# johncai117/Meta-Fine-Tuning

Measured on AMD Instinct MI355X. Metric: episodes/sec at 5-way N-shot (ResNet10+GNN) per GPU and 1/2/4/8-GPU node, higher is better.
Workload: dtype f32

## Files before the change

### include/mft_hip.h

```cpp
#ifndef MFT_HIP_H
#define MFT_HIP_H

#ifdef __cplusplus
extern "C" {
#endif

#define MFT_EINVAL (-22)

enum { MFT_ACT_NONE = 0, MFT_ACT_RELU = 1, MFT_ACT_LRELU = 2 };
enum { MFT_BN_AFFINE_FMA = 0x100 };

int mft_version(void);
int mft_device_info(int* cu_count, int* gcn_arch_is_gfx950);

int mft_stream_create_cumask(const unsigned* mask_words, int n_words, void** stream_out);
int mft_stream_create_priority(int priority, void** stream_out, int* range_out);
int mft_stream_destroy(void* stream);
int mft_stream_probe(float* w, float* m, float* v, long long n, void* stream);
int mft_event_create(void** event_out);
int mft_event_record(void* event, void* stream);
int mft_event_elapsed_ms(void* start, void* stop, float* ms_out);
int mft_event_destroy(void* event);
int mft_probe_placement(unsigned* out, int n_blocks, int spin_cycles, void* stream);

int mft_augment_views(const unsigned char* src, int n_img, int Hs, int Ws, const float* params, int n_views, float* out,
                      long long view_stride, long long img_stride, int size, const float* mean3, const float* std3,
                      void* stream);

int mft_nchw_to_nhwc(const float* src, float* dst, int n_img, int C, int H, int W, void* stream);

long long mft_conv2d_wgrad_adam_dgrad_ws_floats(int n_img, int H, int W, int Cin);
int mft_conv2d_wgrad_adam_dgrad_nhwc(const float* x, int ldx, const float* dy, int ldy, float* w, float* m, float* v,
                                     float* dx_partials, int n_img, int H, int W, int Cin, int Cout, int imgs_per_group,
                                     long long group_stride, int step, float lr, float beta1, float beta2, float eps, void* stream);
int mft_conv2d_wgrad_adam_dgrad_nhwc_dev(const float* x, int ldx, const float* dy, int ldy, float* w, float* m, float* v,
                                         float* dx_partials, int n_img, int H, int W, int Cin, int Cout, int imgs_per_group,
                                         long long group_stride, const float* hyper, float beta1, float beta2, float eps,
                                         void* stream);
int mft_col2im_bn_backward_small(const float* dx_partials, const float* x_raw, const float* relu_out, float* dx, int n_img, int H,
                                 int W, int C, int imgs_per_group, const float* mean, const float* rstd, const float* gamma,
                                 long long gb_group_stride, float* dgamma, float* dbeta, void* stream);

int mft_ce_pool_bn_backward2(const float* feat, const int* labels, int imgs_per_group, int n_groups, int C, int hw,
                             const float* out, const float* xa, const float* xb, float* dxa, float* dxb, const float* mean_a,
                             const float* rstd_a, const float* gamma_a, const float* mean_b, const float* rstd_b,
                             const float* gamma_b, long long gb_group_stride, float* dgamma_a, float* dbeta_a, float* dgamma_b,
                             float* dbeta_b, float* loss, void* stream);

int mft_stem_cache_fill(const float* in, const float* w, int w_ld, int n_img, int H, int W, float* pmax, float* pmin,
                        float* mean_img, float* m2_img, void* stream);
int mft_pool_window_minmax(const float* x, float* ymax, float* ymin, long long n_img, int H, int W, int C, void* stream);
int mft_bn_relu_pooled_gather(const float* pmax, const float* pmin, const int* src_idx, float* y, int n_img, int OH, int OW, int C,
                              int imgs_per_group, const float* mean, const float* rstd, const float* gamma, const float* beta,
                              void* stream);

int mft_ingest_episode_views(const float* const* views, int n_views, int double_first, int n_way, int per_class, int n_support,
                             int C, int H, int W, float* support_store, float* all_store, void* stream);
int mft_pack_oihw(const float* w_oihw, float* w_pk, int Cout, int Cin, int KH, int KW, int k_pad, void* stream);
int mft_pack_oihw_multi(const void* jobs, int n_jobs, long long total_elements, void* stream);
int mft_unpack_oihw(const float* w_pk, float* w_oihw, int Cout, int Cin, int KH, int KW, int k_pad, void* stream);
int mft_pack_dgrad(const float* w_pk, float* wt_pk, int Cout, int Cin, int KH, int KW,
                   int groups, long long w_stride, long long wt_stride, void* stream);

int mft_conv2d_nhwc(const float* in, int ldi, const float* w, const float* bias, float* out, int ldo,
                    int n_img, int H, int W, int Cin, int Cout, int KH, int KW, int stride, int pad,
                    int imgs_per_group, long long w_group_stride, void* stream);

int mft_split_bf16x3(const float* w, unsigned short* planes, long long n, void* stream);
int mft_split_bf16x3_multi(const void* jobs, int n_jobs, long long total_elements, void* stream);
int mft_conv2d_nhwc_x3(const float* in, int ldi, const unsigned short* w3, long long plane_elems, float* out, int ldo,
                       int n_img, int H, int W, int Cin, int Cout, int KH, int KW, int stride, int pad, void* stream);
long long mft_conv2d_x3_stats_ws_floats(int n_img, int H, int W, int Cout, int KH, int KW, int stride, int pad);
int mft_conv2d_nhwc_x3_bnstats(const float* in, int ldi, const unsigned short* w3, long long plane_elems, float* out, int ldo,
                               int n_img, int H, int W, int Cin, int Cout, int KH, int KW, int stride, int pad,
                               int imgs_per_group, float eps, float* stats_ws, float* mean, float* rstd, void* stream);
int mft_conv2d_nhwc_x3_bnin_bnstats(const float* in, int ldi, const float* in_ws, const float* in_gamma, const float* in_beta,
                                    const unsigned short* w3, long long plane_elems, float* out, int ldo, int n_img, int H, int W,
                                    int Cin, int Cout, int imgs_per_group, float eps, float* stats_ws, float* mean, float* rstd,
                                    void* stream);
int mft_split_f16x2(const float* w, unsigned short* planes, long long n, void* stream);
int mft_conv2d_nhwc_h2(const float* in, int ldi, const unsigned short* w2, long long plane_elems, float* out, int ldo,
                       int n_img, int H, int W, int Cin, int Cout, int KH, int KW, int stride, int pad, void* stream);
int mft_conv2d_nhwc_h2_bnstats(const float* in, int ldi, const unsigned short* w2, long long plane_elems, float* out, int ldo,
                               int n_img, int H, int W, int Cin, int Cout, int KH, int KW, int stride, int pad,
                               int imgs_per_group, float eps, float* stats_ws, float* mean, float* rstd, void* stream);
int mft_conv2d_nhwc_h2_bnin_bnstats(const float* in, int ldi, const float* in_ws, const float* in_gamma, const float* in_beta,
                                    const unsigned short* w2, long long plane_elems, float* out, int ldo, int n_img, int H, int W,
                                    int Cin, int Cout, int imgs_per_group, float eps, float* stats_ws, float* mean, float* rstd,
                                    void* stream);
int mft_bn_apply_x3ws(const float* x, int ldx, float* y, int ldy, int C, int rows_per_group, int n_groups, const float* ws,
                      const float* gamma, const float* beta, const float* res, int ldr, const float* res_ws,
                      const float* res_gamma, const float* res_beta, int act, float slope, float eps, float* mean, float* rstd,
                      float* res_mean, float* res_rstd, void* stream);
int mft_bn_running_ema(const float* mean_a, const float* rstd_a, int rows_a, const float* mean_b, const float* rstd_b, int rows_b,
                       const int* order, int n_steps, int C, float eps, float momentum, float* running_mean, float* running_var,
                       void* stream);
int mft_bn_apply_x3ws_fits(int C, int rows_per_group, int with_res_bn);
int mft_bn_relu_pooled_gather_moments(const float* pmax, const float* pmin, const int* src_idx, float* y, int n_img, int OH, int OW,
                                      int C, int imgs_per_group, const float* mean_img, const float* m2_img, int rows_per_img,
                                      float eps, const float* gamma, const float* beta, float* mean, float* rstd, void* stream);

int mft_has_experiments(void);

int mft_conv2d_dgrad_nhwc(const float* dy, int ldy, const float* w, float* dx, int ldx,
                          int n_img, int H, int W, int Cin, int Cout, int KH, int KW, int stride, int pad,
                          int imgs_per_group, long long w_group_stride, void* stream);

long long mft_conv_ksplit_ws_floats(long long rows, int cols, int K);
long long mft_conv_ksplit_grouped_ws_floats(long long rows_per_group, int cols, int K, int groups);
int mft_conv2d_nhwc_ksplit_grouped(const float* in, int ldi, const float* w, float* out, int ldo, int n_img, int H, int W, int Cin,
                                   int Cout, int KH, int KW, int stride, int pad, int imgs_per_group, long long w_group_stride,
                                   float* ws, void* stream);
int mft_conv2d_dgrad_nhwc_ksplit_grouped(const float* dy, int ldy, const float* w, float* dx, int ldx, int n_img, int H, int W, int Cin,
                                         int Cout, int KH, int KW, int stride, int pad, int imgs_per_group, long long w_group_stride,
                                         float* ws, void* stream);
int mft_conv2d_nhwc_ksplit(const float* in, int ldi, const float* w, const float* bias, float* out, int ldo, int n_img, int H, int W,
                           int Cin, int Cout, int KH, int KW, int stride, int pad, float* ws, void* stream);
int mft_conv2d_dgrad_nhwc_ksplit(const float* dy, int ldy, const float* w, float* dx, int ldx, int n_img, int H, int W, int Cin,
                                 int Cout, int KH, int KW, int stride, int pad, float* ws, void* stream);
long long mft_conv2d_wgrad_ws_floats(int n_img, int H, int W, int Cin, int Cout, int KH, int KW, int stride, int pad,
                                     int imgs_per_group);
int mft_conv2d_wgrad_nhwc(const float* in, int ldi, const float* dy, int ldy, float* dw,
                          int n_img, int H, int W, int Cin, int Cout, int KH, int KW, int stride, int pad,
                          int imgs_per_group, long long dw_group_stride, float* ws, void* stream);

long long mft_conv2d_wgrad_oihw_ws_floats(int n_img, int H, int W, int Cin, int Cout, int KH, int KW, int stride, int pad);
int mft_conv2d_wgrad_oihw(const float* in, int ldi, const float* dy, int ldy, float* dw_oihw, int n_img, int H, int W, int Cin,
                          int Cout, int KH, int KW, int stride, int pad, int cin_valid, int cout_valid, float* ws, void* stream);

typedef struct MftWgradJob {
    const float* in; const float* dy; float* dw_oihw; float* ws;
    int ldi, ldy, n_img, H, W, Cin, Cout, KH, KW, stride, pad, cin_valid, cout_valid, reserved;
} MftWgradJob;
int mft_conv2d_wgrad_oihw_multi(const MftWgradJob* jobs, int n_jobs, void* stream);

int mft_conv2d_wgrad_adam_nhwc(const float* in, int ldi, const float* dy, int ldy, float* w, float* m, float* v,
                               float* dw_or_null, int n_img, int H, int W, int Cin, int Cout, int KH, int KW,
                               int stride, int pad, int imgs_per_group, long long group_stride,
                               int step, float lr, float beta1, float beta2, float eps, void* stream);

int mft_wgrad_adam_next_forward(const float* x, int ldx, const float* dy, int ldy, float* w, float* m, float* v,
                                float* dw_or_null, int n_img, int H, int W, int Cin, int Cout, int KH, int KW, int stride,
                                int pad, int imgs_per_group, long long group_stride, int step, const float* hyper, float lr,
                                float beta1, float beta2, float eps, const float* x_next, int mode, float* raw, float* act,
                                const float* gamma, const float* beta, long long gb_group_stride, float* mean, float* rstd,
                                const float* sc_raw, const float* gamma_s, const float* beta_s, float* mean_s, float* rstd_s,
                                float* pooled, float bn_eps, void* stream);


long long mft_bn_stats_ws_floats(int C, int rows_per_group, int n_groups);
int mft_bn_stats(const float* x, int ldx, int C, int rows_per_group, int n_groups, float eps,
                 float* mean, float* rstd, float* ws,
                 float* running_mean, float* running_var, float momentum, long long* num_batches_tracked, void* stream);
typedef struct MftBnStatsJob {
    const float* x; float* mean; float* rstd; float* ws; float* running_mean; float* running_var; long long* num_batches_tracked;
    int ldx, C, rows_per_group, n_groups; float eps, momentum;
} MftBnStatsJob;
int mft_bn_stats_multi(const MftBnStatsJob* jobs, int n_jobs, void* stream);
typedef struct MftBnFwdJob {
    const float* x; float* y; const float* gamma; const float* beta; float* mean; float* rstd;
    float* running_mean; float* running_var; long long* num_batches_tracked;
    const float* res; const float* res_gamma; const float* res_beta; float* res_mean; float* res_rstd;
    float* res_running_mean; float* res_running_var; long long* res_num_batches_tracked;
    int ldx, ldy, ldr, C, rows_per_group, n_groups, act; float eps, momentum, slope;
} MftBnFwdJob;
int mft_bn_forward_small(const MftBnFwdJob* job, void* stream);
int mft_bn_forward_small_max_rows(void);
typedef struct MftBnApplyJob {
    const float* x; float* y; const float* mean; const float* rstd; const float* gamma; const float* beta;
    int ldx, ldy, C, rows_per_group, n_groups, act; float slope; int reserved;
} MftBnApplyJob;
int mft_bn_apply_multi(const MftBnApplyJob* jobs, int n_jobs, void* stream);
int mft_bn_apply(const float* x, int ldx, float* y, int ldy, int C, int rows_per_group, int n_groups,
                 const float* mean, const float* rstd, const float* gamma, const float* beta,
                 long long gb_group_stride,
                 const float* res, int ldr, const float* res_mean, const float* res_rstd,
                 const float* res_gamma, const float* res_beta,
                 int act, float slope, void* stream);
int mft_var_to_rstd(const float* var, float* rstd, int n, float eps, void* stream);
int mft_bn_relu_maxpool(const float* x, float* y, int n_img, int H, int W, int C, int imgs_per_group,
                        const float* mean, const float* rstd, const float* gamma, const float* beta,
                        void* stream);

int mft_bn_image_moments(const float* x, int ldx, int C, int rows_per_img, long long n_img, float* mean_img, float* m2_img,
                         void* stream);
int mft_bn_combine_moments(const float* mean_img, const float* m2_img, const int* idx, int C, int rows_per_img,
                           int imgs_per_group, int n_groups, float eps, float* mean, float* rstd, void* stream);
int mft_bn_relu_maxpool_gather(const float* x, const int* src_idx, float* y, int n_img, int H, int W, int C,
                               int imgs_per_group, const float* mean, const float* rstd, const float* gamma,
                               const float* beta, void* stream);
int mft_global_avgpool(const float* x, float* y, int n_img, int HW, int C, void* stream);

int mft_bn_backward(const float* x, int ldx, const float* dy, int lddy, const float* relu_out, int ldro,
                    float* dx, int lddx, int C, int rows_per_group, int n_groups,
                    const float* mean, const float* rstd, const float* gamma, long long gb_group_stride,
                    float* dgamma, float* dbeta, void* stream);
int mft_bn_small_forward(const float* x1, int ld1, const float* x2, int ld2, const float* res, int ldr, float* y, int ldy, int C,
                         int rows_per_group, int n_groups, const float* gamma1, const float* beta1, const float* gamma2,
                         const float* beta2, long long gb_group_stride, float* mean1, float* rstd1, float* mean2, float* rstd2,
                         int act, float slope, float eps, float* pooled, int hw, void* stream);
int mft_bn_backward2(const float* xa, const float* xb, int ldx, const float* dy, int lddy, float* dxa, float* dxb, int lddx, int C,
                     int rows_per_group, int n_groups, const float* mean_a, const float* rstd_a, const float* gamma_a,
                     const float* mean_b, const float* rstd_b, const float* gamma_b, long long gb_group_stride, float* dgamma_a,
                     float* dbeta_a, float* dgamma_b, float* dbeta_b, void* stream);
int mft_ce_pool_backward(const float* feat, const int* labels, int rows_per_group, int n_groups, int C, int hw, const float* out,
                         float* d_out, float* loss, void* stream);

int mft_avgpool_relu_backward(const float* dfeat, const float* out, float* dout, int n_img, int HW, int C, void* stream);

int mft_cross_entropy(const float* logits, int ld, const int* labels, int C, int rows_per_group, int n_groups,
                      float* loss, float* dlogits, void* stream);
int mft_cross_entropy_mean(const float* logits, int ld, const void* labels, int labels_i64, int C, int rows, float* loss,
                           double* loss_sum, void* stream);
int mft_cross_entropy_mean_backward(const float* logits, int ld, const void* labels, int labels_i64, int C, int rows,
                                    const float* grad_loss, float* dlogits, int ldd, void* stream);
int mft_softmax_rows(const float* x, int ldx, float* y, int ldy, int C, int rows, void* stream);

int mft_proto_scores(const float* feats, int ld, int episodes, int n_way, int n_support, int n_query, int D, float* scores,
                     int softmax, void* stream);
int mft_proto_backward(const float* feats, int ld, int episodes, int n_way, int n_support, int n_query, int D,
                       const float* dscores, int ldg, float* dfeats, int ldd, void* stream);

int mft_mn_gemm(int transa, int transb, int M, int N, int batch, const float* a1, int lda1, long long a1_bs, const float* b1,
                const float* b1_alt, int ldb1, long long b1_bs, int K1, const float* a2, int lda2, long long a2_bs, const float* b2,
                int ldb2, long long b2_bs, int K2, const float* c_in, int ldci, long long ci_bs, const float* bias1,
                const float* bias2, float* c, int ldc, long long c_bs, void* stream);
int mft_lstm_step_forward(float* gates, int ld_g, long long bs_g, const float* c_prev, int ld_cp, long long bs_cp,
                          const float* f_add, int ld_f, float* c_out, float* h_out, int ld_o, long long bs_o, int rows, int D,
                          int batch, void* stream);
int mft_lstm_step_backward(float* gates, int ld_g, long long bs_g, const float* c_prev, int ld_cp, long long bs_cp,
                           const float* c_new, int ld_cn, long long bs_cn, const float* dh1, int ld_d1, long long bs_d1,
                           const float* dh2, int ld_d2, long long bs_d2, const float* dc_in, float* dc_out, int ld_dc,
                           long long bs_dc, float* dh_sum, float* dgate_sum, int accumulate, int rows, int D, int batch,
                           void* stream);
int mft_mn_gather(const float* feats, int ld, int episodes, int n_way, int n_support, int n_query, int D, float* zS, float* zQ,
                  float* h0, void* stream);
int mft_mn_scatter_backward(const float* dzS, const float* dq1, const float* dq2, int episodes, int n_way, int n_support,
                            int n_query, int D, float* dfeats, int ldd, void* stream);
int mft_mn_encode_combine(const float* zS, const float* hf, const float* hr, int episodes, int S, int D, float* G, float* gnorm,
                          void* stream);
int mft_mn_colsum(const float* x, int ldx, int C, long long rows, float* out, void* stream);
int mft_mn_attention_forward(const float* h, const float* G, int episodes, int Q, int S, int D, float* a, float* r, void* stream);
// ... 178 lines not shown
```

### meta-fine-tuning_amd/_lib.py

```python
import ctypes
import os

PKG = os.path.dirname(os.path.abspath(__file__))
LIB_PATH = os.path.join(PKG, "libmft_hip.so")

_P = ctypes.c_void_p
_I = ctypes.c_int
_L = ctypes.c_longlong
_F = ctypes.c_float

SIGNATURES = {
    "mft_version": [],
    "mft_device_info": [_P, _P],
    "mft_stream_create_cumask": [_P, _I, _P],
    "mft_stream_destroy": [_P],
    "mft_stream_probe": [_P, _P, _P, _L, _P],
    "mft_probe_placement": [_P, _I, _I, _P],
    "mft_event_create": [_P],
    "mft_event_record": [_P, _P],
    "mft_event_elapsed_ms": [_P, _P, _P],
    "mft_event_destroy": [_P],
    "mft_augment_views": [_P, _I, _I, _I, _P, _I, _P, _L, _L, _I, _P, _P, _P],
    "mft_nchw_to_nhwc": [_P, _P, _I, _I, _I, _I, _P],
    "mft_pack_oihw": [_P, _P, _I, _I, _I, _I, _I, _P],
    "mft_unpack_oihw": [_P, _P, _I, _I, _I, _I, _I, _P],
    "mft_pack_dgrad": [_P, _P, _I, _I, _I, _I, _I, _L, _L, _P],
    "mft_conv2d_nhwc": [_P, _I, _P, _P, _P, _I, _I, _I, _I, _I, _I, _I, _I, _I, _I, _I, _L, _P],
    "mft_has_experiments": [],
    "mft_split_bf16x3": [_P, _P, _L, _P],
    "mft_split_bf16x3_multi": [_P, _I, _L, _P],
    "mft_conv2d_nhwc_x3": [_P, _I, _P, _L, _P, _I, _I, _I, _I, _I, _I, _I, _I, _I, _I, _P],
    "mft_conv2d_x3_stats_ws_floats": [_I, _I, _I, _I, _I, _I, _I, _I],
    "mft_conv2d_nhwc_x3_bnstats": [_P, _I, _P, _L, _P, _I, _I, _I, _I, _I, _I, _I, _I, _I, _I, _I, _F, _P, _P, _P, _P],
    "mft_conv2d_dgrad_nhwc": [_P, _I, _P, _P, _I, _I, _I, _I, _I, _I, _I, _I, _I, _I, _I, _L, _P],
    "mft_conv_ksplit_ws_floats": [_L, _I, _I],
    "mft_conv_ksplit_grouped_ws_floats": [_L, _I, _I, _I],
    "mft_conv2d_nhwc_ksplit_grouped": [_P, _I, _P, _P, _I, _I, _I, _I, _I, _I, _I, _I, _I, _I, _I, _L, _P, _P],
    "mft_conv2d_dgrad_nhwc_ksplit_grouped": [_P, _I, _P, _P, _I, _I, _I, _I, _I, _I, _I, _I, _I, _I, _I, _L, _P, _P],
    "mft_conv2d_nhwc_ksplit": [_P, _I, _P, _P, _P, _I, _I, _I, _I, _I, _I, _I, _I, _I, _I, _P, _P],
    "mft_conv2d_dgrad_nhwc_ksplit": [_P, _I, _P, _P, _I, _I, _I, _I, _I, _I, _I, _I, _I, _I, _P, _P],
    "mft_conv2d_wgrad_oihw_ws_floats": [_I, _I, _I, _I, _I, _I, _I, _I, _I],
    "mft_conv2d_wgrad_oihw": [_P, _I, _P, _I, _P, _I, _I, _I, _I, _I, _I, _I, _I, _I, _I, _I, _P, _P],
    "mft_conv2d_wgrad_oihw_multi": [_P, _I, _P],
    "mft_conv2d_wgrad_ws_floats": [_I, _I, _I, _I, _I, _I, _I, _I, _I, _I],
    "mft_conv2d_wgrad_nhwc": [_P, _I, _P, _I, _P, _I, _I, _I, _I, _I, _I, _I, _I, _I, _I, _L, _P, _P],
    "mft_conv2d_wgrad_adam_nhwc": [_P, _I, _P, _I, _P, _P, _P, _P, _I, _I, _I, _I, _I, _I, _I, _I, _I, _I, _L, _I, _F, _F, _F,
                                   _F, _P],
    "mft_pair_softmax_ut_backward": [_P, _P, _P, _P, _P, _I, _I, _I, _P, _P],
    "mft_pair_bwd_stats_ws_floats": [_L, _I],
    "mft_pair_bn_act_backward": [_P, _I, _P, _I, _P, _P, _P, _P, _P, _P, _I, _L, _I, _L, _F, _P, _P, _P, _P, _P, _P],
    "mft_pair_absdiff_ut": [_P, _I, _P, _P, _I, _I, _I, _L, _L, _P],
    "mft_pair_dx_gather": [_P, _I, _P, _I, _P, _I, _I, _I, _I, _L, _L, _P],
    "mft_pack_oihw_multi": [_P, _I, _L, _P],
    "mft_wgrad_adam_next_forward": [_P, _I, _P, _I, _P, _P, _P, _P, _I, _I, _I, _I, _I, _I, _I, _I, _I, _I, _L, _I, _P, _F, _F, _F,
                                    _F, _P, _I, _P, _P, _P, _P, _L, _P, _P, _P, _P, _P, _P, _P, _P, _F, _P],
    "mft_bn_stats_ws_floats": [_I, _I, _I],
    "mft_bn_stats": [_P, _I, _I, _I, _I, _F, _P, _P, _P, _P, _P, _F, _P, _P],
    "mft_bn_apply": [_P, _I, _P, _I, _I, _I, _I, _P, _P, _P, _P, _L, _P, _I, _P, _P, _P, _P, _I, _F, _P],
    "mft_bn_apply_multi": [_P, _I, _P],
    "mft_bn_stats_multi": [_P, _I, _P],
    "mft_bn_relu_maxpool": [_P, _P, _I, _I, _I, _I, _I, _P, _P, _P, _P, _P],
    "mft_bn_relu_maxpool_gather": [_P, _P, _P, _I, _I, _I, _I, _I, _P, _P, _P, _P, _P],
    "mft_bn_image_moments": [_P, _I, _I, _I, _L, _P, _P, _P],
    "mft_bn_combine_moments": [_P, _P, _P, _I, _I, _I, _I, _F, _P, _P, _P],
    "mft_global_avgpool": [_P, _P, _I, _I, _I, _P],
    "mft_bn_small_forward": [_P, _I, _P, _I, _P, _I, _P, _I, _I, _I, _I, _P, _P, _P, _P, _L, _P, _P, _P, _P, _I, _F, _F, _P, _I, _P],
    "mft_bn_backward2": [_P, _P, _I, _P, _I, _P, _P, _I, _I, _I, _I, _P, _P, _P, _P, _P, _P, _L, _P, _P, _P, _P, _P],
    "mft_ce_pool_backward": [_P, _P, _I, _I, _I, _I, _P, _P, _P, _P],
    "mft_bn_backward": [_P, _I, _P, _I, _P, _I, _P, _I, _I, _I, _I, _P, _P, _P, _L, _P, _P, _P],
    "mft_avgpool_relu_backward": [_P, _P, _P, _I, _I, _I, _P],
    "mft_cross_entropy": [_P, _I, _P, _I, _I, _I, _P, _P, _P],
    "mft_softmax_rows": [_P, _I, _P, _I, _I, _I, _P],
    "mft_proto_scores": [_P, _I, _I, _I, _I, _I, _I, _P, _I, _P],
    "mft_proto_backward": [_P, _I, _I, _I, _I, _I, _I, _P, _I, _P, _I, _P],
    "mft_mn_gemm": [_I, _I, _I, _I, _I, _P, _I, _L, _P, _P, _I, _L, _I, _P, _I, _L, _P, _I, _L, _I, _P, _I, _L, _P, _P, _P, _I, _L, _P],
    "mft_lstm_step_forward": [_P, _I, _L, _P, _I, _L, _P, _I, _P, _P, _I, _L, _I, _I, _I, _P],
    "mft_lstm_step_backward": [_P, _I, _L, _P, _I, _L, _P, _I, _L, _P, _I, _L, _P, _I, _L, _P, _P, _I, _L, _P, _P, _I, _I, _I, _I, _P],
    "mft_mn_gather": [_P, _I, _I, _I, _I, _I, _I, _P, _P, _P, _P],
    "mft_mn_scatter_backward": [_P, _P, _P, _I, _I, _I, _I, _I, _P, _I, _P],
    "mft_mn_encode_combine": [_P, _P, _P, _I, _I, _I, _P, _P, _P],
    "mft_mn_colsum": [_P, _I, _I, _L, _P, _P],
    "mft_mn_attention_forward": [_P, _P, _I, _I, _I, _I, _P, _P, _P],
    "mft_mn_attention_backward": [_P, _P, _P, _P, _I, _I, _I, _I, _P, _P, _P],
    "mft_mn_readout_forward": [_P, _P, _P, _I, _I, _I, _I, _I, _P, _P, _P, _P, _P, _P],
    "mft_mn_readout_backward": [_P, _I, _P, _P, _P, _P, _P, _P, _P, _I, _I, _I, _I, _I, _P, _P, _P, _P],
    "mft_nll_mean": [_P, _I, _P, _I, _I, _I, _P, _P, _P],
    "mft_nll_mean_backward": [_P, _I, _I, _I, _P, _P, _I, _P],
    "mft_ridge_gram": [_P, _I, _I, _I, _I, _I, _I, _F, _P, _P],
    "mft_ridge_factor_solve": [_P, _I, _I, _I, _I, _I, _I, _P, _P, _P, _P],
    "mft_ridge_scores": [_P, _I, _I, _I, _I, _I, _I, _P, _P, _P, _I, _P],
    "mft_ridge_backward_query": [_P, _I, _I, _I, _I, _I, _I, _P, _P, _P, _I, _P, _I, _P, _P, _P],
    "mft_ridge_backward_support": [_P, _I, _I, _I, _I, _I, _I, _P, _P, _P, _P, _P, _P, _I, _P, _P],
    "mft_dist_linear_forward": [_P, _I, _I, _I, _P, _P, _I, _I, _F, _P, _I, _P],
    "mft_dist_linear_backward": [_P, _I, _I, _P, _P, _I, _I, _F, _P, _I, _P, _I, _P, _P, _P],
    "mft_dist_head_sgd_run": [_P, _P, _P, _I, _I, _I, _I, _I, _I, _P, _P, _F, _F, _F, _F, _F, _P],
    "mft_dist_head_step": [_P, _I, _P, _I, _I, _I, _I, _F, _P, _P, _P, _P, _P, _P, _P, _I, _P, _I, _F, _F, _F, _F, _F, _P],
    "mft_cross_entropy_mean": [_P, _I, _P, _I, _I, _I, _P, _P, _P],
    "mft_cross_entropy_mean_backward": [_P, _I, _P, _I, _I, _I, _P, _P, _I, _P],
    "mft_adam_step": [_P, _P, _P, _P, _L, _I, _F, _F, _F, _F, _F, _P],
    "mft_sgd_step": [_P, _P, _P, _L, _I, _F, _F, _F, _F, _P],
    "mft_maml_delta": [_P, _P, _P, _L, _P],
    "mft_conv2d_wgrad_adam_dgrad_ws_floats": [_I, _I, _I, _I],
    "mft_conv2d_wgrad_adam_dgrad_nhwc": [_P, _I, _P, _I, _P, _P, _P, _P, _I, _I, _I, _I, _I, _I, _L, _I, _F, _F, _F, _F, _P],
    "mft_conv2d_wgrad_adam_dgrad_nhwc_dev": [_P, _I, _P, _I, _P, _P, _P, _P, _I, _I, _I, _I, _I, _I, _L, _P, _F, _F, _F, _P],
    "mft_col2im_bn_backward_small": [_P, _P, _P, _P, _I, _I, _I, _I, _I, _P, _P, _P, _L, _P, _P, _P],
    "mft_stream_create_priority": [_I, _P, _P],
    "mft_ce_pool_bn_backward2": [_P, _P, _I, _I, _I, _I, _P, _P, _P, _P, _P, _P, _P, _P, _P, _P, _P, _L, _P, _P, _P, _P, _P, _P],
    "mft_pool_window_minmax": [_P, _P, _P, _L, _I, _I, _I, _P],
    "mft_stem_cache_fill": [_P, _P, _I, _I, _I, _I, _P, _P, _P, _P, _P],
    "mft_conv2d_nhwc_x3_bnin_bnstats": [_P, _I, _P, _P, _P, _P, _L, _P, _I, _I, _I, _I, _I, _I, _I, _F, _P, _P, _P, _P],
    "mft_split_f16x2": [_P, _P, _L, _P],
    "mft_conv2d_nhwc_h2": [_P, _I, _P, _L, _P, _I, _I, _I, _I, _I, _I, _I, _I, _I, _I, _P],
    "mft_conv2d_nhwc_h2_bnstats": [_P, _I, _P, _L, _P, _I, _I, _I, _I, _I, _I, _I, _I, _I, _I, _I, _F, _P, _P, _P, _P],
    "mft_conv2d_nhwc_h2_bnin_bnstats": [_P, _I, _P, _P, _P, _P, _L, _P, _I, _I, _I, _I, _I, _I, _I, _F, _P, _P, _P, _P],
    "mft_bn_apply_x3ws": [_P, _I, _P, _I, _I, _I, _I, _P, _P, _P, _P, _I, _P, _P, _P, _I, _F, _F, _P, _P, _P, _P, _P],
    "mft_bn_apply_x3ws_fits": [_I, _I, _I],
    "mft_bn_running_ema": [_P, _P, _I, _P, _P, _I, _P, _I, _I, _F, _F, _P, _P, _P],
    "mft_bn_relu_pooled_gather_moments": [_P, _P, _P, _P, _I, _I, _I, _I, _I, _P, _P, _I, _F, _P, _P, _P, _P, _P],
    "mft_bn_relu_pooled_gather": [_P, _P, _P, _P, _I, _I, _I, _I, _I, _P, _P, _P, _P, _P],
    "mft_ingest_episode_views": [_P, _I, _I, _I, _I, _I, _I, _I, _I, _P, _P, _P],
    "mft_block_entry_small_forward": [_P, _I, _P, _L, _P, _L, _P, _P, _P, _I, _I, _I, _I, _I, _I, _I, _P, _P, _L, _P, _P, _F, _P],
    "mft_block_exit_small_forward": [_P, _P, _L, _P, _P, _P, _P, _I, _I, _I, _I, _I, _P, _P, _P, _P, _L, _P, _P, _P, _P, _F, _P],
    "mft_conv2d_dgrad_bn_backward_small": [_P, _I, _P, _P, _I, _I, _I, _I, _I, _I, _I, _I, _I, _I, _L, _P, _P, _P, _P, _P, _L,
                                           _P, _P, _P],
    "mft_linear_head_sgd_run": [_P, _P, _P, _I, _I, _I, _I, _I, _I, _P, _P, _F, _F, _F, _F, _P],
    "mft_linear_head_adam_run": [_P, _P, _P, _I, _I, _I, _I, _I, _I, _P, _P, _F, _F, _F, _F, _F, _P],
    "mft_adam_multi": [_P, _I, _I, _F, _F, _F, _F, _F, _F, _P],
    "mft_adam_hyper_advance": [_P, _P, _F, _F, _F, _P],
    "mft_adam_step_dev": [_P, _P, _P, _P, _L, _P, _F, _F, _F, _F, _P],
    "mft_conv2d_wgrad_adam_nhwc_dev": [_P, _I, _P, _I, _P, _P, _P, _P, _I, _I, _I, _I, _I, _I, _I, _I, _I, _I, _L, _P, _F, _F,
                                       _F, _P],
    "mft_linear_head_step": [_P, _I, _P, _I, _I, _I, _I, _P, _P, _P, _P, _P, _P, _P, _I, _P, _I, _F, _F, _F, _F, _F, _P],
    "mft_linear_head_scores": [_P, _I, _I, _I, _I, _I, _P, _P, _P, _P],
    "mft_pair_absdiff": [_P, _I, _P, _I, _I, _I, _I, _P],
    "mft_masked_softmax": [_P, _I, _P, _I, _I, _P],
    "mft_pair_mlp_tiles_m": [_I, _I],
    "mft_pair_mlp_layer": [_P, _I, _I, _P, _P, _P, _P, _I, _I, _P, _P, _I, _I, _I, _I, _F, _P, _P, _P, _I, _P],
    "mft_bn_forward_small": [_P, _P],
    "mft_bn_forward_small_max_rows": [],
    "mft_gemm_rk": [_P, _I, _P, _I, _I, _P, _P, _I, _I, _I, _P],
    "mft_pair_mlp_tiles_m_rk": [_I, _I],
    "mft_pair_mlp_layer_rk": [_P, _I, _I, _P, _P, _P, _P, _I, _I, _P, _P, _I, _I, _I, _I, _F, _P, _P, _P, _P],
    "mft_pair_mlp_stats_finalize_rk": [_P, _P, _P, _I, _I, _I, _P, _P, _F, _P, _P, _P, _P, _P],
    "mft_pair_mlp_stats_finalize": [_P, _P, _P, _I, _I, _I, _P, _P, _F, _P, _P, _P, _P, _P],
    "mft_pair_mlp_score": [_P, _I, _P, _P, _P, _P, _F, _P, _I, _I, _I, _P],
    "mft_masked_softmax_ut": [_P, _P, _I, _I, _P],
    "mft_graph_aggregate": [_P, _P, _I, _P, _I, _I, _I, _I, _P],
    "mft_copy_cols": [_P, _I, _P, _I, _I, _I, _I, _I, _F, _P],
    "mft_build_graph_nodes": [_P, _I, _P, _I, _I, _I, _I, _I, _I, _P],
    "mft_gather_query_scores": [_P, _I, _P, _I, _I, _I, _I, _P],
    "mft_gather_rows": [_P, _P, _P, _I, _L, _P],
    "mft_var_to_rstd": [_P, _P, _I, _F, _P],
    "mft_bn_backward_ws_floats": [_I, _I, _I],
    "mft_bn_backward_act": [_P, _I, _P, _I, _P, _I, _P, _I, _I, _I, _I, _P, _P, _P, _L, _P, _P, _I, _F, _P, _P, _P, _P, _P],
    "mft_bn_backward_act_multi": [_P, _I, _P],
    "mft_act_backward": [_P, _I, _P, _I, _P, _I, _I, _L, _I, _F, _I, _P],
    "mft_colsum": [_P, _I, _I, _L, _P, _P, _P],
    "mft_bn_relu_maxpool_arg": [_P, _P, _P, _I, _I, _I, _I, _I, _P, _P, _P, _P, _P],
    "mft_maxpool_relu_backward": [_P, _P, _P, _P, _I, _I, _I, _I, _P],
    "mft_masked_softmax_backward": [_P, _P, _P, _I, _I, _I, _P],
    "mft_pair_absdiff_backward": [_P, _I, _P, _I, _P, _I, _I, _I, _I, _P],
    "mft_graph_aggregate_backward": [_P, _P, _I, _P, _I, _P, _I, _P, _I, _I, _I, _I, _P],
    "mft_build_graph_nodes_backward": [_P, _I, _P, _I, _I, _I, _I, _I, _I, _P],
    "mft_gather_query_scores_backward": [_P, _P, _I, _I, _I, _I, _I, _P, _P],
    "mft_fwt_draw_fold": [_P, _I, _I, _I, ctypes.c_ulonglong, _P, _P, _P, _P, _P],
    "mft_fwt_unfold": [_P, _I, _I, _I, _P, _P],
}
TESTING_SIGNATURES = {
    "mft_debug_set_conv_tile": [_I],
    "mft_debug_set_x3_tile": [_I],
    "mft_debug_reset": [],
    "mft_wgrad_fwd_set_exact": [_I],
    "mft_wgrad_fwd_set_xcd": [_I],
}
_RESTYPE = {"mft_conv2d_x3_stats_ws_floats": _L, "mft_bn_stats_ws_floats": _L, "mft_conv2d_wgrad_ws_floats": _L, "mft_bn_backward_ws_floats": _L,
            "mft_conv2d_wgrad_adam_dgrad_ws_floats": _L, "mft_pair_bwd_stats_ws_floats": _L, "mft_conv_ksplit_ws_floats": _L, "mft_conv2d_wgrad_oihw_ws_floats": _L, "mft_conv_ksplit_grouped_ws_floats": _L}

_lib = None


def lib():
    global _lib
    if _lib is None:
        if not os.path.exists(LIB_PATH):
            raise RuntimeError(
                "libmft_hip.so not found at %s -- build it with `python -c 'import __graft_entry__ as g; g.build()'`; "
                "this package has no CPU or PyTorch fallback" % LIB_PATH)
        import torch
        if torch.cuda.is_available():
            torch.cuda.init()
            torch.empty(1, device="cuda")
        h = ctypes.CDLL(LIB_PATH)
        for name, argtypes in list(SIGNATURES.items()) + list(TESTING_SIGNATURES.items()):
            fn = getattr(h, name)
            fn.argtypes = argtypes
            fn.restype = _RESTYPE.get(name, _I)
        _lib = h
    return _lib


MFT_EINVAL = -22


def check(rc, what):
    if rc != 0:
        raise RuntimeError("%s failed with code %d (hipError_t / MFT_EINVAL=-22)" % (what, rc))


class LaunchTimer:

    _SKIP = ("mft_event_", "mft_stream_", "mft_debug_", "mft_version", "mft_device_info", "mft_has_experiments",
             "mft_wgrad_fwd_set_", "mft_probe_placement")

    def __init__(self, only=None, keep_args=False):
        self.only = only
        self.keep_args = keep_args
        self._pairs = []
        self._free = []
        self._real = None

    def _event(self):
        if self._free:
            return self._free.pop()
        e = ctypes.c_void_p()
        check(self._real.mft_event_create(ctypes.byref(e)), "mft_event_create")
        return e

    def __getattr__(self, name):
        real = self.__dict__["_real"]
        fn = getattr(real, name)
        sig = SIGNATURES.get(name)
        if (sig is None or not sig or sig[-1] is not _P or name.endswith("_ws_floats") or name.startswith(self._SKIP)
                or (self.only is not None and not self.only(name))):
            return fn

        def timed(*args):
            stream = args[-1]
            a, b = self._event(), self._event()
            real.mft_event_record(a, stream)
            rc = fn(*args)
            if rc != 0:
                self._free += [a, b]
                return rc
            real.mft_event_record(b, stream)
            self._pairs.append((name, a, b, args if self.keep_args else None))
            return rc
        return timed

    def __enter__(self):
        global _lib
        self._real = lib()
        assert not isinstance(self._real, LaunchTimer), "LaunchTimer blocks do not nest"
        _lib = self
        return self

    def __exit__(self, *exc):
        global _lib
        _lib = self._real
        if exc and exc[0] is not None:
            for _, a, b, _ in self._pairs:
                self._free += [a, b]
            self._pairs = []
            self.close()
        return False

    def collect(self, calls=False):
        out, flat = {}, []
# ... 14 lines not shown
```

### meta-fine-tuning_amd/csrc/conv_x3.hip

```cpp
#include "mft_common.h"
#include "bn_fold.h"

namespace {

typedef __bf16 bf16x8 __attribute__((ext_vector_type(8)));
typedef __bf16 bf16x2 __attribute__((ext_vector_type(2)));
typedef _Float16 f16x8 __attribute__((ext_vector_type(8)));
typedef _Float16 f16x4 __attribute__((ext_vector_type(4)));
typedef float f32x2 __attribute__((ext_vector_type(2)));
typedef unsigned u32x2 __attribute__((ext_vector_type(2)));
typedef unsigned u32x4 __attribute__((ext_vector_type(4)));

struct X3Args {
    const float* in;
    const unsigned short* w3;
    long long plane;
    float* out;
    int ldi, ldo;
    int H, W, Cin, OH, OW, Cout, KH, KW, stride, pad;
    int Kpad;
    int M;
    int tiles_n;
    unsigned in_bytes, w_bytes;
    int xcd_swizzle;
    int row_swz;
    float* stats_ws;
    int rows_per_group;
    int s1_rows;
    const float* bn_ws; const float* bn_gamma; const float* bn_beta;
    float bn_eps;
    int bn_max_tiles;
};

constexpr int X3_RS = 40;

__device__ __forceinline__ unsigned pk_bf16(float a, float b) {
    f32x2 v = {a, b};
    return __builtin_bit_cast(unsigned, __builtin_convertvector(v, bf16x2));
}

__device__ __forceinline__ void split4(const f32x4 x, u32x2& p1, u32x2& p2, u32x2& p3) {
    f32x4 r;
    p1[0] = pk_bf16(x[0], x[1]);
    p1[1] = pk_bf16(x[2], x[3]);
    r[0] = x[0] - __builtin_bit_cast(float, p1[0] << 16);
    r[1] = x[1] - __builtin_bit_cast(float, p1[0] & 0xffff0000u);
    r[2] = x[2] - __builtin_bit_cast(float, p1[1] << 16);
    r[3] = x[3] - __builtin_bit_cast(float, p1[1] & 0xffff0000u);
    p2[0] = pk_bf16(r[0], r[1]);
    p2[1] = pk_bf16(r[2], r[3]);
    r[0] -= __builtin_bit_cast(float, p2[0] << 16);
    r[1] -= __builtin_bit_cast(float, p2[0] & 0xffff0000u);
    r[2] -= __builtin_bit_cast(float, p2[1] << 16);
    r[3] -= __builtin_bit_cast(float, p2[1] & 0xffff0000u);
    p3[0] = pk_bf16(r[0], r[1]);
    p3[1] = pk_bf16(r[2], r[3]);
}

__device__ __forceinline__ void split4_h2(const f32x4 x, u32x2& p1, u32x2& p2) {
    const f16x4 hi = __builtin_convertvector(x, f16x4);
    const f32x4 r = (x - __builtin_convertvector(hi, f32x4)) * 2048.f;
    const f16x4 lo = __builtin_convertvector(r, f16x4);
    p1 = __builtin_bit_cast(u32x2, hi);
    p2 = __builtin_bit_cast(u32x2, lo);
}
constexpr float X3_H2_LO_SCALE = 1.0f / 2048.f;

template <int BM, int BN, bool DB, int HOIST = 0, int DBG = 0, bool XS = false, int NP = 3>
__global__ __launch_bounds__(256) __attribute__((amdgpu_waves_per_eu(NP == 2 ? 3 : 1))) void conv_x3_kernel(X3Args p) {
    static_assert(NP == 3 || (NP == 2 && !DB && HOIST == 0 && DBG == 0 && !XS), "f16x2: the plain single-buffer form only");
    constexpr int NACC = NP == 3 ? 1 : 2;
    constexpr int TM = BM / 64;
    constexpr int TN = BN / 64;
    constexpr int PA = BM / 32;
    constexpr int PB = BN / 64;
    constexpr int RS = XS ? 32 : X3_RS;
    constexpr int A_PLANE = BM * RS;
    constexpr int B_PLANE = BN * RS;
    auto lo = [](int row, int c) -> int {
        if constexpr (XS) return row * 32 + ((((c >> 3) ^ (row >> 2)) & 3) << 3) + (c & 7);
        else return row * X3_RS + c;
    };
    extern __shared__ __attribute__((aligned(16))) unsigned short smem[];
    unsigned short* As = smem;
    unsigned short* Bs = smem + NP * A_PLANE;
    constexpr int BUF = NP * (A_PLANE + B_PLANE);

    const int tid = threadIdx.x;
    const int lane = tid & 63, wave = tid >> 6;
    const int wm = wave >> 1, wn = wave & 1;
    const int r = lane & 31, h = lane >> 5;
    const bool g_swz = !XS && p.row_swz != 0;
    int tile_id = blockIdx.x;
    if (p.xcd_swizzle) {
        const int nwg = gridDim.x, q = nwg >> 3, rmd = nwg & 7;
        const int xcd = tile_id & 7, slot = tile_id >> 3;
        tile_id = xcd * q + (xcd < rmd ? xcd : rmd) + slot;
    }
    const int nt = tile_id % p.tiles_n;
    const int mt = tile_id / p.tiles_n;
    const int m0 = mt * BM, n0 = nt * BN;

    const int g_id = tid >> 5;
    const int g_rr = (tid >> 3) & 3;
    const int lrow = g_swz ? g_rr * 4 + (g_id & 3) + 16 * (g_id >> 2) : tid >> 3;
    const int c4 = (tid & 7) * 4;
    const int ohw = p.OH * p.OW;
    const __amdgpu_buffer_rsrc_t rA = __builtin_amdgcn_make_buffer_rsrc((void*)p.in, 0, p.in_bytes, 0x00020000);
    const __amdgpu_buffer_rsrc_t rB = __builtin_amdgcn_make_buffer_rsrc((void*)p.w3, 0, p.w_bytes, 0x00020000);
    int a_off[PA];
    int a_ih0[PA], a_iw0[PA];
    bool a_ok[PA];
#pragma unroll
    for (int j = 0; j < PA; ++j) {
        const int m = m0 + lrow + 32 * j;
        a_ok[j] = m < p.M;
        const int mm = a_ok[j] ? m : 0;
        const int img = mm / ohw;
        const int rem = mm - img * ohw;
        const int oh = rem / p.OW, ow = rem - oh * p.OW;
        a_ih0[j] = oh * p.stride - p.pad;
        a_iw0[j] = ow * p.stride - p.pad;
        a_off[j] = (((img * p.H + a_ih0[j]) * p.W + a_iw0[j]) * p.ldi + c4) * 4;
    }
    const int bseg = tid & 3;
    const int brow = g_swz ? ((tid >> 2) & 3) * 4 + ((tid >> 4) & 3) + 16 * (tid >> 6) : tid >> 2;
    int b_off[PB];
#pragma unroll
    for (int j = 0; j < PB; ++j) b_off[j] = ((n0 + brow + 64 * j) * p.Kpad + bseg * 8) * 2;
    const int plane_bytes = (int)(p.plane * 2);

    f32x16 accs[NACC][TM][TN];
#pragma unroll
    for (int q = 0; q < NACC; ++q)
#pragma unroll
        for (int i = 0; i < TM; ++i)
#pragma unroll
            for (int j = 0; j < TN; ++j)
#pragma unroll
                for (int e = 0; e < 16; ++e) accs[q][i][j][e] = 0.f;
    auto& acc = accs[0];
    auto val = [&](int i, int j, int e) -> float {
        if constexpr (NP == 3) return accs[0][i][j][e];
        else return __builtin_fmaf(accs[NACC - 1][i][j][e], X3_H2_LO_SCALE, accs[0][i][j][e]);
    };

    struct Stage {
        f32x4 ra[PA];
        u32x4 rb[PB][NP];
    };
    Stage st0;
    const int nk = p.Kpad / 32;

    int t_kt = 0, t_ci0 = 0, t_kh = 0, t_kw = 0;
    auto load_tile = [&](int kt, Stage& S) {
        const int k0 = kt * 32;
        while (t_kt < kt) {
            ++t_kt;
            t_ci0 += 32;
            if (t_ci0 == p.Cin) { t_ci0 = 0; if (++t_kw == p.KW) { t_kw = 0; ++t_kh; } }
        }
        const int ci0 = t_ci0, kh = t_kh, kw = t_kw;
        const int tap_off = ((kh * p.W + kw) * p.ldi + ci0) * 4;
#pragma unroll
        for (int j = 0; j < PA; ++j) {
            const bool ok = a_ok[j] && (unsigned)(a_ih0[j] + kh) < (unsigned)p.H && (unsigned)(a_iw0[j] + kw) < (unsigned)p.W;
            const unsigned voff = ok ? (unsigned)(a_off[j] + tap_off) : 0x80000000u;
            S.ra[j] = __builtin_bit_cast(f32x4, __builtin_amdgcn_raw_buffer_load_b128(rA, voff, 0, 0));
        }
#pragma unroll
        for (int j = 0; j < PB; ++j)
#pragma unroll
            for (int pl = 0; pl < NP; ++pl)
                S.rb[j][pl] = __builtin_amdgcn_raw_buffer_load_b128(rB, b_off[j] + pl * plane_bytes, k0 * 2, 0);
    };
    auto store_tile = [&](const Stage& S, int buf) {
        unsigned short* As = smem + buf * BUF;
        unsigned short* Bs = As + NP * A_PLANE;
#pragma unroll
        for (int j = 0; j < PA; ++j) {
            const int off = lo(lrow + 32 * j, c4);
            if constexpr (NP == 2) {
                u32x2 p1, p2;
                split4_h2(S.ra[j], p1, p2);
                *(u32x2*)(As + off) = p1;
                *(u32x2*)(As + A_PLANE + off) = p2;
            } else {
                u32x2 p1, p2, p3;
                if constexpr (DBG & 1) {
                    const u32x4 raw = __builtin_bit_cast(u32x4, S.ra[j]);
                    p1[0] = raw[0]; p1[1] = raw[1]; p2[0] = raw[2]; p2[1] = raw[3]; p3 = p1;
                } else {
                    split4(S.ra[j], p1, p2, p3);
                }
                *(u32x2*)(As + off) = p1;
                *(u32x2*)(As + A_PLANE + off) = p2;
                *(u32x2*)(As + 2 * A_PLANE + off) = p3;
            }
        }
#pragma unroll
        for (int j = 0; j < PB; ++j)
#pragma unroll
            for (int pl = 0; pl < NP; ++pl)
                *(u32x4*)(Bs + pl * B_PLANE + lo(brow + 64 * j, bseg * 8)) = S.rb[j][pl];
    };

    auto compute = [&](int buf) {
        const unsigned short* As = smem + buf * BUF;
        const unsigned short* Bs = As + NP * A_PLANE;
        if constexpr (NP == 2) {
#pragma unroll
            for (int kk = 0; kk < 2; ++kk) {
                f16x8 a[TM][2], b[TN][2];
#pragma unroll
                for (int i = 0; i < TM; ++i)
#pragma unroll
                    for (int pl = 0; pl < 2; ++pl)
                        a[i][pl] = *(const f16x8*)(As + pl * A_PLANE + lo(wm * (BM / 2) + i * 32 + r, kk * 16 + h * 8));
#pragma unroll
                for (int j = 0; j < TN; ++j)
#pragma unroll
                    for (int pl = 0; pl < 2; ++pl)
                        b[j][pl] = *(const f16x8*)(Bs + pl * B_PLANE + lo(wn * (BN / 2) + j * 32 + r, kk * 16 + h * 8));
                constexpr int TA[3] = {0, 1, 0};
                constexpr int TB[3] = {1, 0, 0};
                constexpr int TQ[3] = {1, 1, 0};
#pragma unroll
                for (int t = 0; t < 3; ++t)
#pragma unroll
                    for (int i = 0; i < TM; ++i)
#pragma unroll
                        for (int j = 0; j < TN; ++j)
                            accs[TQ[t] ? NACC - 1 : 0][i][j] =
                                __builtin_amdgcn_mfma_f32_32x32x16_f16(a[i][TA[t]], b[j][TB[t]], accs[TQ[t] ? NACC - 1 : 0][i][j], 0, 0, 0);
            }
            return;
        }
        if constexpr (HOIST == 0) {
#pragma unroll
            for (int kk = 0; kk < 2; ++kk) {
                bf16x8 a[TM][3], b[TN][3];
#pragma unroll
                for (int i = 0; i < TM; ++i)
#pragma unroll
                    for (int pl = 0; pl < 3; ++pl)
                        a[i][pl] = *(const bf16x8*)(As + pl * A_PLANE + lo(wm * (BM / 2) + i * 32 + r, kk * 16 + h * 8));
#pragma unroll
                for (int j = 0; j < TN; ++j)
// ... 14 lines not shown
#pragma unroll
                    for (int t = 0; t < 6; ++t)
#pragma unroll
                        for (int i = 0; i < TM; ++i)
#pragma unroll
                            for (int j = 0; j < TN; ++j)
                                acc[i][j] = __builtin_amdgcn_mfma_f32_32x32x16_bf16(a[i][TA[t]], b[j][TB[t]], acc[i][j], 0, 0, 0);
                }
            }
            return;
        }
        bf16x8 a[2][TM][3], b[2][TN][3];
        if constexpr (HOIST == 1) {
#pragma unroll
            for (int kk = 0; kk < 2; ++kk) {
#pragma unroll
                for (int pl = 0; pl < 3; ++pl) {
#pragma unroll
                    for (int i = 0; i < TM; ++i)
                        a[kk][i][pl] = *(const bf16x8*)(As + pl * A_PLANE + lo(wm * (BM / 2) + i * 32 + r, kk * 16 + h * 8));
#pragma unroll
                    for (int j = 0; j < TN; ++j)
                        b[kk][j][pl] = *(const bf16x8*)(Bs + pl * B_PLANE + lo(wn * (BN / 2) + j * 32 + r, kk * 16 + h * 8));
                }
            }
            __builtin_amdgcn_sched_barrier(0);
            constexpr int TA[6] = {0, 0, 1, 1, 0, 2};
            constexpr int TB[6] = {0, 1, 0, 1, 2, 0};
#pragma unroll
            for (int kk = 0; kk < 2; ++kk)
#pragma unroll
                for (int t = 0; t < 6; ++t)
#pragma unroll
                    for (int i = 0; i < TM; ++i)
#pragma unroll
                        for (int j = 0; j < TN; ++j)
                            acc[i][j] = __builtin_amdgcn_mfma_f32_32x32x16_bf16(a[kk][i][TA[t]], b[kk][j][TB[t]], acc[i][j], 0, 0, 0);
            __builtin_amdgcn_sched_barrier(0);
        } else {
            auto rd = [&](int kk) {
#pragma unroll
                for (int pl = 0; pl < 3; ++pl) {
#pragma unroll
                    for (int i = 0; i < TM; ++i)
                        a[kk][i][pl] = *(const bf16x8*)(As + pl * A_PLANE + lo(wm * (BM / 2) + i * 32 + r, kk * 16 + h * 8));
#pragma unroll
                    for (int j = 0; j < TN; ++j)
                        b[kk][j][pl] = *(const bf16x8*)(Bs + pl * B_PLANE + lo(wn * (BN / 2) + j * 32 + r, kk * 16 + h * 8));
                }
            };
            constexpr int TA[6] = {0, 0, 1, 1, 0, 2};
            constexpr int TB[6] = {0, 1, 0, 1, 2, 0};
            auto mm = [&](int kk) {
#pragma unroll
                for (int t = 0; t < 6; ++t)
#pragma unroll
                    for (int i = 0; i < TM; ++i)
#pragma unroll
                        for (int j = 0; j < TN; ++j)
                            acc[i][j] = __builtin_amdgcn_mfma_f32_32x32x16_bf16(a[kk][i][TA[t]], b[kk][j][TB[t]], acc[i][j], 0, 0, 0);
            };
            rd(0);
            __builtin_amdgcn_sched_barrier(0);
            rd(1);
            mm(0);
            for (int q = 0; q < 6 * TM * TN; ++q) {
                __builtin_amdgcn_sched_group_barrier(0x8, 1, 0);
                __builtin_amdgcn_sched_group_barrier(0x100, (3 * (TM + TN) + 6 * TM * TN - 1) / (6 * TM * TN), 0);
            }
            __builtin_amdgcn_sched_barrier(0);
            mm(1);
            __builtin_amdgcn_sched_barrier(0);
        }
    };
    if constexpr (DB) {
        load_tile(0, st0);
        store_tile(st0, 0);
        __syncthreads();
        load_tile(nk > 1 ? 1 : 0, st0);
        for (int kt = 0; kt + 1 < nk; ++kt) {
            compute(kt & 1);
            store_tile(st0, (kt + 1) & 1);
            load_tile(kt + 2 < nk ? kt + 2 : nk - 1, st0);
            __syncthreads();
        }
        compute((nk - 1) & 1);
    } else {
        load_tile(0, st0);
        store_tile(st0, 0);
        __syncthreads();
        for (int kt = 0; kt < nk; ++kt) {
            if constexpr (!(DBG & 4)) { if (kt + 1 < nk) load_tile(kt + 1, st0); }
            if constexpr (!(DBG & 16)) compute(0);
            if constexpr (!(DBG & 32)) __syncthreads();
            if constexpr (!(DBG & 8)) { if (kt + 1 < nk) store_tile(st0, 0); }
            if constexpr (!(DBG & 32)) __syncthreads();
        }
    }

#pragma unroll
    for (int i = 0; i < TM; ++i)
#pragma unroll
        for (int j = 0; j < TN; ++j) {
            const int n = n0 + wn * (BN / 2) + j * 32 + r;
#pragma unroll
            for (int e = 0; e < 16; ++e) {
                const int row = (e & 3) + 8 * (e >> 2) + 4 * h;
                const int m = m0 + wm * (BM / 2) + i * 32 + row;
                if (m < p.M) p.out[(long long)m * p.ldo + n] = val(i, j, e);
            }
        }
    if (p.stats_ws != nullptr) {
        static_assert(TN == 1 || TN == 2, "stats epilogue");
        const int split = (m0 / p.rows_per_group + 1) * p.rows_per_group;
        float* sred = reinterpret_cast<float*>(smem);
        __syncthreads();
#pragma unroll
        for (int j = 0; j < TN; ++j) {
            float a1 = 0.f, a2 = 0.f, b1 = 0.f, b2 = 0.f;
#pragma unroll
            for (int i = 0; i < TM; ++i)
#pragma unroll
                for (int e = 0; e < 16; ++e) {
                    const int m = m0 + wm * (BM / 2) + i * 32 + (e & 3) + 8 * (e >> 2) + 4 * h;
                    const float v = val(i, j, e);
                    if (m < p.M) {
                        if (m < split) { a1 += v; a2 += v * v; }
                        else { b1 += v; b2 += v * v; }
                    }
                }
            a1 += __shfl_xor(a1, 32, 64); a2 += __shfl_xor(a2, 32, 64);
            b1 += __shfl_xor(b1, 32, 64); b2 += __shfl_xor(b2, 32, 64);
            if (h == 0) {
                float* o = sred + ((((wm * 2 + wn) * TN + j) * 32 + r) << 2);
                o[0] = a1; o[1] = a2; o[2] = b1; o[3] = b2;
            }
        }
        __syncthreads();
        if (wm == 0 && h == 0) {
#pragma unroll
            for (int j = 0; j < TN; ++j) {
                const float* o0 = sred + ((((0 * 2 + wn) * TN + j) * 32 + r) << 2);
                const float* o1 = sred + ((((1 * 2 + wn) * TN + j) * 32 + r) << 2);
                const int n = n0 + wn * (BN / 2) + j * 32 + r;
                float* w0 = p.stats_ws + (((long long)mt * 2 + 0) * p.Cout + n) * 2;
                float* w1 = p.stats_ws + (((long long)mt * 2 + 1) * p.Cout + n) * 2;
                w0[0] = o0[0] + o1[0]; w0[1] = o0[1] + o1[1];
                w1[0] = o0[2] + o1[2]; w1[1] = o0[3] + o1[3];
            }
        }
    }
}

#ifdef MFT_EXPERIMENTS
#include "../../tools/experiments/conv_x3_pingpong.inc"
#endif

template <int BM, int BN, bool BNIN, int NP = 3, bool BDB = true>
__device__ __forceinline__ void conv_x3_s1_body(const X3Args& p) {
    static_assert(NP == 3 || NP == 2, "3 bf16 pieces (six products) or 2 fp16 pieces (three products)");
    constexpr int NACC = NP == 3 ? 1 : 2;
    constexpr int TM = BM / 64, TN = BN / 64;
    constexpr int PA = BM / 32, PB = BN / 64;
    constexpr int RS = X3_RS;
    constexpr int B_PLANE = BN * RS;
    const int A_PLANE = p.s1_rows * RS;
    extern __shared__ __attribute__((aligned(16))) unsigned short smem[];
    constexpr int NBB = (NP == 2 && BDB) ? 2 : 1;
    unsigned short* As = smem;
    unsigned short* Bs = smem + NP * A_PLANE;
    float* bn_tab = reinterpret_cast<float*>(Bs + NBB * NP * B_PLANE);

    const int tid = threadIdx.x;
    const int lane = tid & 63, wave = tid >> 6;
    const int wm = wave >> 1, wn = wave & 1;
    const int r = lane & 31, h = lane >> 5;
    int tile_id = blockIdx.x;
    if (p.xcd_swizzle) {
        const int nwg = gridDim.x, q = nwg >> 3, rmd = nwg & 7;
        const int xcd = tile_id & 7, slot = tile_id >> 3;
        tile_id = xcd * q + (xcd < rmd ? xcd : rmd) + slot;
    }
    const int nt = tile_id % p.tiles_n;
    const int mt = tile_id / p.tiles_n;
    const int m0 = mt * BM, n0 = nt * BN;
    const int W = p.W, H = p.H;
    const int fr0 = m0 / W;
    const int g0 = BNIN ? m0 / p.rows_per_group : 0;
    const bool bn_two = BNIN && (m0 + (BM < p.M - m0 ? BM : p.M - m0) - 1) / p.rows_per_group > g0;
    if constexpr (BNIN) {
        char* stage = reinterpret_cast<char*>(smem);
        const size_t gstride = mft_x3_stage_bytes(p.bn_max_tiles, p.Cin);
        const bool two = bn_two;
        mft_x3_stats_stage(p.bn_ws, p.Cin, g0, p.M, p.rows_per_group, BM, p.bn_max_tiles, stage, tid, 256);
        if (two) mft_x3_stats_stage(p.bn_ws, p.Cin, g0 + 1, p.M, p.rows_per_group, BM, p.bn_max_tiles, stage + gstride, tid, 256);
        __syncthreads();
        for (int i = tid; i < 2 * p.Cin; i += 256) {
            const int gi = i >= p.Cin ? 1 : 0, c = i - gi * p.Cin;
            if (gi == 0 || two) {
                float mu, rs, sc, sh;
                mft_x3_stats_staged(stage + gi * gstride, p.bn_max_tiles, p.Cin, c, g0 + gi, p.M, p.rows_per_group, BM, p.bn_eps, mu, rs);
                mft_bn_fold(mu, rs, p.bn_gamma[c], p.bn_beta[c], sc, sh);
                bn_tab[(gi * 2 + 0) * p.Cin + c] = sc;
                bn_tab[(gi * 2 + 1) * p.Cin + c] = sh;
            }
        }
        __syncthreads();
    }
    const int g_id = tid >> 5, g_rr = (tid >> 3) & 3;
    const int lrow = p.row_swz ? g_rr * 4 + (g_id & 3) + 16 * (g_id >> 2) : tid >> 3;
    const int c4 = (tid & 7) * 4;
    const __amdgpu_buffer_rsrc_t rA = __builtin_amdgcn_make_buffer_rsrc((void*)p.in, 0, p.in_bytes, 0x00020000);
    const __amdgpu_buffer_rsrc_t rB = __builtin_amdgcn_make_buffer_rsrc((void*)p.w3, 0, p.w_bytes, 0x00020000);
    int a_off[PA], a_oh[PA], a_lds[PA], a_tab[PA];
    bool a_ok[PA];
#pragma unroll
    for (int j = 0; j < PA; ++j) {
        const int t = lrow + 32 * j, m = m0 + t;
        const int fr = m / W;
        a_ok[j] = m < p.M;
        a_oh[j] = fr - (fr / H) * H;
        a_off[j] = ((a_ok[j] ? m : 0) * p.ldi + c4) * 4;
        a_lds[j] = (t + 1) * RS + c4;
        a_tab[j] = BNIN ? ((a_ok[j] ? m / p.rows_per_group - g0 : 0) * 2 * p.Cin + c4) : 0;
    }
    const int hside = (tid >> 3) & 1;
    const int mh = hside ? m0 + BM : m0 - 1;
    const int frh = (mh > 0 ? mh : 0) / W;
    const bool h_ok = tid < 16 && (hside ? (mh < p.M && mh - frh * W != 0) : (m0 > 0 && m0 - fr0 * W != 0));
    const int h_oh = frh - (frh / H) * H;
    const int h_off = ((h_ok ? mh : 0) * p.ldi + c4) * 4;
    const int h_lds = (hside ? BM + 1 : 0) * RS + c4;
    const int h_tab = BNIN ? (((hside && h_ok) ? (m0 + BM - 1) / p.rows_per_group - g0 : 0) * 2 * p.Cin + c4) : 0;

    const int bseg = tid & 3;
    const int brow = p.row_swz ? ((tid >> 2) & 3) * 4 + ((tid >> 4) & 3) + 16 * (tid >> 6) : tid >> 2;
    int b_off[PB];
#pragma unroll
    for (int j = 0; j < PB; ++j) b_off[j] = ((n0 + brow + 64 * j) * p.Kpad + bseg * 8) * 2;
    const int plane_bytes = (int)(p.plane * 2);

    int fa[TM], fl[TM], fr_[TM];
    constexpr int Z0 = BM + 2;
#pragma unroll
    for (int i = 0; i < TM; ++i) {
        const int t = wm * (BM / 2) + i * 32 + r;
        const int ow = (m0 + t) - ((m0 + t) / W) * W;
        fa[i] = (t + 1) * RS;
        fl[i] = ow == 0 ? (Z0 + ((t - Z0) & 15)) * RS : fa[i] - RS;
        fr_[i] = ow == W - 1 ? (Z0 + ((t + 2 - Z0) & 15)) * RS : fa[i] + RS;
    }

    f32x16 acc[NACC][TM][TN];
#pragma unroll
    for (int q = 0; q < NACC; ++q)
#pragma unroll
        for (int i = 0; i < TM; ++i)
#pragma unroll
            for (int j = 0; j < TN; ++j)
#pragma unroll
                for (int e = 0; e < 16; ++e) acc[q][i][j][e] = 0.f;
    auto val = [&](int i, int j, int e) -> float {
        if constexpr (NP == 3) return acc[0][i][j][e];
        else return __builtin_fmaf(acc[1][i][j][e], X3_H2_LO_SCALE, acc[0][i][j][e]);
    };

    struct Stage {
        f32x4 ra[PA];
        f32x4 rh;
        u32x4 rb[PB][NP];
    };
    Stage st;
    const int n_ci = p.Cin / 32;
    const int n_ms = 3 * n_ci;
    auto load_a = [&](int ms, Stage& S) {
        const int kh = ms / n_ci, ci0 = (ms - kh * n_ci) * 32;
        const int shift = ((kh - 1) * W * p.ldi + ci0) * 4;
#pragma unroll
        for (int j = 0; j < PA; ++j) {
            const bool ok = a_ok[j] && (unsigned)(a_oh[j] + kh - 1) < (unsigned)H;
            S.ra[j] = __builtin_bit_cast(f32x4, __builtin_amdgcn_raw_buffer_load_b128(rA, ok ? (unsigned)(a_off[j] + shift) : 0x80000000u, 0, 0));
        }
        const bool okh = h_ok && (unsigned)(h_oh + kh - 1) < (unsigned)H;
        S.rh = __builtin_bit_cast(f32x4, __builtin_amdgcn_raw_buffer_load_b128(rA, okh ? (unsigned)(h_off + shift) : 0x80000000u, 0, 0));
    };
    auto load_b = [&](int ms, int kw, Stage& S) {
        const int kh = ms / n_ci, ci0 = (ms - kh * n_ci) * 32;
        const int k0 = (kh * 3 + kw) * p.Cin + ci0;
#pragma unroll
        for (int j = 0; j < PB; ++j)
#pragma unroll
            for (int pl = 0; pl < NP; ++pl)
                S.rb[j][pl] = __builtin_amdgcn_raw_buffer_load_b128(rB, b_off[j] + pl * plane_bytes, k0 * 2, 0);
    };
    auto put_a = [&](const f32x4 v, int off) {
        if constexpr (NP == 3) {
            u32x2 p1, p2, p3;
            split4(v, p1, p2, p3);
            *(u32x2*)(As + off) = p1;
            *(u32x2*)(As + A_PLANE + off) = p2;
            *(u32x2*)(As + 2 * A_PLANE + off) = p3;
        } else {
            u32x2 p1, p2;
            split4_h2(v, p1, p2);
            *(u32x2*)(As + off) = p1;
            *(u32x2*)(As + A_PLANE + off) = p2;
        }
    };
    auto bn_relu = [&](const f32x4 v, const f32x4 sc, const f32x4 sh, bool ok) {
        f32x4 o = mft_bn_affine4(v, sc, sh);
#pragma unroll
        for (int e = 0; e < 4; ++e) o[e] = ok ? fmaxf(o[e], 0.f) : 0.f;
        return o;
    };
    auto store_a = [&](const Stage& S, int ms) {
        if constexpr (BNIN) {
            const int kh = ms / n_ci, ci0 = (ms - kh * n_ci) * 32;
            const bool okh = h_ok && (unsigned)(h_oh + kh - 1) < (unsigned)H;
            if (!bn_two) {
                const f32x4 sc = *(const f32x4*)(bn_tab + ci0 + c4), sh = *(const f32x4*)(bn_tab + p.Cin + ci0 + c4);
#pragma unroll
                for (int j = 0; j < PA; ++j)
                    put_a(bn_relu(S.ra[j], sc, sh, a_ok[j] && (unsigned)(a_oh[j] + kh - 1) < (unsigned)H), a_lds[j]);
                if (tid < 16) put_a(bn_relu(S.rh, sc, sh, okh), h_lds);
            } else {
#pragma unroll
                for (int j = 0; j < PA; ++j)
                    put_a(bn_relu(S.ra[j], *(const f32x4*)(bn_tab + a_tab[j] + ci0), *(const f32x4*)(bn_tab + a_tab[j] + p.Cin + ci0),
                                  a_ok[j] && (unsigned)(a_oh[j] + kh - 1) < (unsigned)H), a_lds[j]);
                if (tid < 16)
                    put_a(bn_relu(S.rh, *(const f32x4*)(bn_tab + h_tab + ci0), *(const f32x4*)(bn_tab + h_tab + p.Cin + ci0), okh), h_lds);
            }
        } else {
#pragma unroll
            for (int j = 0; j < PA; ++j) put_a(S.ra[j], a_lds[j]);
            if (tid < 16) put_a(S.rh, h_lds);
        }
    };
    auto store_b = [&](const Stage& S, int bb = 0) {
#pragma unroll
        for (int j = 0; j < PB; ++j)
#pragma unroll
            for (int pl = 0; pl < NP; ++pl)
                *(u32x4*)(Bs + (bb * NP + pl) * B_PLANE + (brow + 64 * j) * RS + bseg * 8) = S.rb[j][pl];
    };
    auto compute = [&](int kw, int bb = 0) {
        const unsigned short* const Bc = Bs + bb * NP * B_PLANE;
#pragma unroll
        for (int kk = 0; kk < 2; ++kk) {
            if constexpr (NP == 3) {
                bf16x8 a[TM][3], b[TN][3];
#pragma unroll
                for (int i = 0; i < TM; ++i)
#pragma unroll
                    for (int pl = 0; pl < 3; ++pl)
                        a[i][pl] = *(const bf16x8*)(As + pl * A_PLANE + (kw == 0 ? fl[i] : (kw == 1 ? fa[i] : fr_[i])) + kk * 16 + h * 8);
#pragma unroll
                for (int j = 0; j < TN; ++j)
#pragma unroll
                    for (int pl = 0; pl < 3; ++pl)
                        b[j][pl] = *(const bf16x8*)(Bc + pl * B_PLANE + (wn * (BN / 2) + j * 32 + r) * RS + kk * 16 + h * 8);
                constexpr int TA[6] = {2, 0, 1, 1, 0, 0};
                constexpr int TB[6] = {0, 2, 1, 0, 1, 0};
#pragma unroll
                for (int t = 0; t < 6; ++t)
#pragma unroll
                    for (int i = 0; i < TM; ++i)
#pragma unroll
                        for (int j = 0; j < TN; ++j)
                            acc[0][i][j] = __builtin_amdgcn_mfma_f32_32x32x16_bf16(a[i][TA[t]], b[j][TB[t]], acc[0][i][j], 0, 0, 0);
            } else {
                f16x8 a[TM][2], b[TN][2];
#pragma unroll
                for (int i = 0; i < TM; ++i)
#pragma unroll
                    for (int pl = 0; pl < 2; ++pl)
                        a[i][pl] = *(const f16x8*)(As + pl * A_PLANE + (kw == 0 ? fl[i] : (kw == 1 ? fa[i] : fr_[i])) + kk * 16 + h * 8);
#pragma unroll
                for (int j = 0; j < TN; ++j)
#pragma unroll
                    for (int pl = 0; pl < 2; ++pl)
                        b[j][pl] = *(const f16x8*)(Bc + pl * B_PLANE + (wn * (BN / 2) + j * 32 + r) * RS + kk * 16 + h * 8);
                constexpr int TA[3] = {0, 1, 0};
                constexpr int TB[3] = {1, 0, 0};
                constexpr int TQ[3] = {1, 1, 0};
#pragma unroll
                for (int t = 0; t < 3; ++t)
#pragma unroll
                    for (int i = 0; i < TM; ++i)
#pragma unroll
                        for (int j = 0; j < TN; ++j)
                            acc[TQ[t]][i][j] = __builtin_amdgcn_mfma_f32_32x32x16_f16(a[i][TA[t]], b[j][TB[t]], acc[TQ[t]][i][j], 0, 0, 0);
            }
        }
    };

    for (int i = tid; i < NP * A_PLANE / 8; i += 256) ((u32x4*)As)[i] = (u32x4){0u, 0u, 0u, 0u};
    load_a(0, st);
    load_b(0, 0, st);
    __syncthreads();
    store_a(st, 0);
    store_b(st);
    __syncthreads();
    if constexpr (NBB == 2) {
        int cur = 0;
        for (int ms = 0; ms < n_ms; ++ms) {
            const int msn = ms + 1 < n_ms ? ms + 1 : ms;
            load_b(ms, 1, st);
            compute(0, cur);
            store_b(st, cur ^ 1);
            __syncthreads();
            load_b(ms, 2, st);
            compute(1, cur ^ 1);
            store_b(st, cur);
            __syncthreads();
            load_a(msn, st);
            load_b(msn, 0, st);
            compute(2, cur);
            store_b(st, cur ^ 1);
            __syncthreads();
            store_a(st, msn);
            __syncthreads();
            cur ^= 1;
        }
    } else {
        for (int ms = 0; ms < n_ms; ++ms) {
            const int msn = ms + 1 < n_ms ? ms + 1 : ms;
            load_b(ms, 1, st);
            compute(0);
            __syncthreads();
            store_b(st);
            __syncthreads();
            load_b(ms, 2, st);
            compute(1);
            __syncthreads();
            store_b(st);
            __syncthreads();
            load_a(msn, st);
            load_b(msn, 0, st);
            compute(2);
            __syncthreads();
            store_a(st, msn);
            store_b(st);
            __syncthreads();
        }
    }

#pragma unroll
    for (int i = 0; i < TM; ++i)
#pragma unroll
        for (int j = 0; j < TN; ++j) {
            const int n = n0 + wn * (BN / 2) + j * 32 + r;
#pragma unroll
            for (int e = 0; e < 16; ++e) {
                const int row = (e & 3) + 8 * (e >> 2) + 4 * h;
                const int m = m0 + wm * (BM / 2) + i * 32 + row;
                if (m < p.M) p.out[(long long)m * p.ldo + n] = val(i, j, e);
            }
        }
    if (p.stats_ws != nullptr) {
        static_assert(TN == 1 || TN == 2, "stats epilogue");
        const int split = (m0 / p.rows_per_group + 1) * p.rows_per_group;
        float* sred = reinterpret_cast<float*>(smem);
        __syncthreads();
#pragma unroll
        for (int j = 0; j < TN; ++j) {
            float a1 = 0.f, a2 = 0.f, b1 = 0.f, b2 = 0.f;
#pragma unroll
            for (int i = 0; i < TM; ++i)
#pragma unroll
                for (int e = 0; e < 16; ++e) {
                    const int m = m0 + wm * (BM / 2) + i * 32 + (e & 3) + 8 * (e >> 2) + 4 * h;
                    const float v = val(i, j, e);
                    if (m < p.M) {
                        if (m < split) { a1 += v; a2 += v * v; }
                        else { b1 += v; b2 += v * v; }
                    }
                }
            a1 += __shfl_xor(a1, 32, 64); a2 += __shfl_xor(a2, 32, 64);
            b1 += __shfl_xor(b1, 32, 64); b2 += __shfl_xor(b2, 32, 64);
            if (h == 0) {
                float* o = sred + ((((wm * 2 + wn) * TN + j) * 32 + r) << 2);
                o[0] = a1; o[1] = a2; o[2] = b1; o[3] = b2;
            }
        }
        __syncthreads();
        if (wm == 0 && h == 0) {
#pragma unroll
            for (int j = 0; j < TN; ++j) {
                const float* o0 = sred + ((((0 * 2 + wn) * TN + j) * 32 + r) << 2);
                const float* o1 = sred + ((((1 * 2 + wn) * TN + j) * 32 + r) << 2);
                const int n = n0 + wn * (BN / 2) + j * 32 + r;
                float* w0 = p.stats_ws + (((long long)mt * 2 + 0) * p.Cout + n) * 2;
                float* w1 = p.stats_ws + (((long long)mt * 2 + 1) * p.Cout + n) * 2;
                w0[0] = o0[0] + o1[0]; w0[1] = o0[1] + o1[1];
                w1[0] = o0[2] + o1[2]; w1[1] = o0[3] + o1[3];
            }
        }
    }
}

template <int BM, int BN, int NP = 3, bool BDB = true>
__global__ __launch_bounds__(256) __attribute__((amdgpu_waves_per_eu(NP == 2 ? 3 : 1))) void conv_x3_s1_kernel(X3Args p) {
    conv_x3_s1_body<BM, BN, false, NP, BDB>(p);
}

template <int BM, int BN, int NP = 3, bool BDB = true>
__global__ __launch_bounds__(256) __attribute__((amdgpu_waves_per_eu(3, 3))) void conv_x3_s1_bnin_kernel(X3Args p) {
    conv_x3_s1_body<BM, BN, true, NP, BDB>(p);
}

__global__ void x3_stats_finalize_kernel(const float* __restrict__ ws, int C, int M, int R, int BM, float eps,
                                         float* __restrict__ mean, float* __restrict__ rstd) {
    const int c = blockIdx.x * blockDim.x + threadIdx.x;
    const int g = blockIdx.y;
    if (c >= C) return;
    float mu, rs;
    mft_x3_stats_merge(ws, C, c, g, M, R, BM, eps, mu, rs);
    mean[(long long)g * C + c] = mu;
    rstd[(long long)g * C + c] = rs;
}

__global__ __launch_bounds__(256) void split_bf16x3_kernel(const float* __restrict__ w, unsigned short* __restrict__ out,
                                                           long long n) {
    for (long long i = (long long)blockIdx.x * blockDim.x + threadIdx.x; i < n; i += (long long)gridDim.x * blockDim.x) {
        const float x = w[i];
        const unsigned q1 = pk_bf16(x, 0.f) & 0xffffu;
        const float r1 = x - __builtin_bit_cast(float, q1 << 16);
        const unsigned q2 = pk_bf16(r1, 0.f) & 0xffffu;
        const float r2 = r1 - __builtin_bit_cast(float, q2 << 16);
        const unsigned q3 = pk_bf16(r2, 0.f) & 0xffffu;
        out[i] = (unsigned short)q1;
        out[n + i] = (unsigned short)q2;
        out[2 * n + i] = (unsigned short)q3;
    }
}

struct SplitJob { const float* src; unsigned short* dst; long long n, Cout, Cin, taps, transposed, start; };

__global__ __launch_bounds__(256) void split_bf16x3_multi_kernel(const SplitJob* __restrict__ jobs, int n_jobs, long long total) {
    for (long long i = (long long)blockIdx.x * blockDim.x + threadIdx.x; i < total; i += (long long)gridDim.x * blockDim.x) {
        int lo = 0, hi = n_jobs - 1;
        while (lo < hi) {
            const int mid = (lo + hi + 1) >> 1;
            if (jobs[mid].start <= i) lo = mid; else hi = mid - 1;
        }
        const SplitJob j = jobs[lo];
        const long long l = i - j.start;
        long long src = l;
        if (j.transposed) {
            const long long co = l % j.Cout, t = l / j.Cout;
            const long long tp = t % j.taps, ci = t / j.taps;
            src = (co * j.taps + (j.taps - 1 - tp)) * j.Cin + ci;
        }
        const float x = j.src[src];
        const unsigned q1 = pk_bf16(x, 0.f) & 0xffffu;
        const float r1 = x - __builtin_bit_cast(float, q1 << 16);
        const unsigned q2 = pk_bf16(r1, 0.f) & 0xffffu;
        const float r2 = r1 - __builtin_bit_cast(float, q2 << 16);
        const unsigned q3 = pk_bf16(r2, 0.f) & 0xffffu;
        j.dst[l] = (unsigned short)q1;
        j.dst[j.n + l] = (unsigned short)q2;
        j.dst[2 * j.n + l] = (unsigned short)q3;
    }
}

__global__ __launch_bounds__(256) void split_f16x2_kernel(const float* __restrict__ w, unsigned short* __restrict__ out, long long n) {
    for (long long i = (long long)blockIdx.x * blockDim.x + threadIdx.x; i < n; i += (long long)gridDim.x * blockDim.x) {
        const float x = w[i];
        const _Float16 hi = (_Float16)x;
        const _Float16 lo = (_Float16)((x - (float)hi) * 2048.f);
        out[i] = __builtin_bit_cast(unsigned short, hi);
        out[n + i] = __builtin_bit_cast(unsigned short, lo);
    }
}

int g_x3_db = 0;
int g_x3_dbg = 0;
int g_x3_hoist = 0;
int g_x3_row_swz = 1;
int g_x3_xcd = 1;
int g_x3_min_lds_kb = 0;

template <int BM, int BN, bool DB>
int launch_x3(X3Args p, hipStream_t s, int np = 3) {
    const int tiles_m = (p.M + BM - 1) / BM;
    p.tiles_n = p.Cout / BN;
    p.xcd_swizzle = g_x3_xcd;
    p.row_swz = g_x3_row_swz;
    if (np == 2) {
        if constexpr (!DB) {
            p.row_swz = g_x3_row_swz != 0;
            const size_t lds2 = (size_t)2 * (BM + BN) * X3_RS * sizeof(unsigned short);
            hipLaunchKernelGGL((conv_x3_kernel<BM, BN, false, 0, 0, false, 2>), dim3((unsigned)(tiles_m * p.tiles_n)), dim3(256), lds2, s, p);
            return mft_launch_status();
        }
        return MFT_EINVAL;
    }
#ifdef MFT_EXPERIMENTS
    const bool xs = g_x3_row_swz == 2 && !DB && g_x3_hoist == 0 && g_x3_dbg == 0;
#else
    constexpr bool xs = false;
#endif
    size_t lds = (size_t)(DB ? 2 : 1) * 3 * (BM + BN) * (xs ? 32 : X3_RS) * sizeof(unsigned short);
#ifdef MFT_EXPERIMENTS
    if ((size_t)g_x3_min_lds_kb * 1024 > lds) lds = (size_t)g_x3_min_lds_kb * 1024;
    if (xs) {
        if constexpr (!DB) {
            hipLaunchKernelGGL((conv_x3_kernel<BM, BN, false, 0, 0, true>), dim3((unsigned)(tiles_m * (p.Cout / BN))), dim3(256), lds, s,
                               ([&] { X3Args q = p; q.tiles_n = p.Cout / BN; q.xcd_swizzle = g_x3_xcd; q.row_swz = 0; return q; })());
            return mft_launch_status();
        }
    }
    auto kern = g_x3_hoist == 1 ? conv_x3_kernel<BM, BN, DB, 1> : (g_x3_hoist == 2 ? conv_x3_kernel<BM, BN, DB, 2> : conv_x3_kernel<BM, BN, DB, 0>);
    if (g_x3_dbg && !DB) {
        switch (g_x3_dbg) {
            case 1: kern = conv_x3_kernel<BM, BN, DB, 0, 1>; break;
            case 2: kern = conv_x3_kernel<BM, BN, DB, 0, 2>; break;
            case 4: kern = conv_x3_kernel<BM, BN, DB, 0, 4>; break;
            case 8: kern = conv_x3_kernel<BM, BN, DB, 0, 8>; break;
            case 12: kern = conv_x3_kernel<BM, BN, DB, 0, 12>; break;
            case 13: kern = conv_x3_kernel<BM, BN, DB, 0, 13>; break;
            case 16: kern = conv_x3_kernel<BM, BN, DB, 0, 16>; break;
            case 28: kern = conv_x3_kernel<BM, BN, DB, 0, 28>; break;
            case 32: kern = conv_x3_kernel<BM, BN, DB, 0, 32>; break;
            case 34: kern = conv_x3_kernel<BM, BN, DB, 0, 34>; break;
            case 36: kern = conv_x3_kernel<BM, BN, DB, 0, 36>; break;
            case 33: kern = conv_x3_kernel<BM, BN, DB, 0, 33>; break;
            default: break;
        }
    }
#else
    auto kern = conv_x3_kernel<BM, BN, DB, 0>;
#endif
    if (lds > 64 * 1024) {
        hipError_t e = hipFuncSetAttribute((const void*)kern, hipFuncAttributeMaxDynamicSharedMemorySize, 160 * 1024);
        if (e != hipSuccess) return (int)e;
    }
    hipLaunchKernelGGL(kern, dim3((unsigned)(tiles_m * p.tiles_n)), dim3(256), lds, s, p);
    return mft_launch_status();
}

int g_x3_s1 = 1;

constexpr size_t X3_S1_LDS_3PER_CU = 160 * 1024 / 3;

int g_x3_bdb = 1;

inline size_t x3_s1_lds(int BM, int BN, int W, int bn_cin, int np = 3) {
    (void)W;
    return (size_t)np * (BM + 18 + ((np == 2 && g_x3_bdb) ? 2 : 1) * BN) * X3_RS * sizeof(unsigned short) + (size_t)4 * bn_cin * sizeof(float);
}

template <int BM, int BN>
int launch_x3_s1(X3Args p, hipStream_t s, int np = 3) {
    const int tiles_m = (p.M + BM - 1) / BM;
    p.tiles_n = p.Cout / BN;
    p.xcd_swizzle = g_x3_xcd;
    p.row_swz = g_x3_row_swz != 0;
    p.s1_rows = BM + 18;
    const size_t lds = x3_s1_lds(BM, BN, p.W, p.bn_ws ? p.Cin : 0, np);
    const dim3 grid((unsigned)(tiles_m * p.tiles_n));
    if (np == 2 && g_x3_bdb) {
        if (p.bn_ws) hipLaunchKernelGGL((conv_x3_s1_bnin_kernel<BM, BN, 2, true>), grid, dim3(256), lds, s, p);
        else hipLaunchKernelGGL((conv_x3_s1_kernel<BM, BN, 2, true>), grid, dim3(256), lds, s, p);
    } else if (np == 2) {
        if (p.bn_ws) hipLaunchKernelGGL((conv_x3_s1_bnin_kernel<BM, BN, 2, false>), grid, dim3(256), lds, s, p);
        else hipLaunchKernelGGL((conv_x3_s1_kernel<BM, BN, 2, false>), grid, dim3(256), lds, s, p);
    } else if (p.bn_ws) {
        hipLaunchKernelGGL((conv_x3_s1_bnin_kernel<BM, BN>), grid, dim3(256), lds, s, p);
    } else {
        hipLaunchKernelGGL((conv_x3_s1_kernel<BM, BN>), grid, dim3(256), lds, s, p);
    }
    return mft_launch_status();
}

int g_x3_pp = 0;
#ifdef MFT_EXPERIMENTS

template <int BM, int BN>
int launch_x3_pp(X3Args p, hipStream_t s) {
    const int tiles_m = (p.M + BM - 1) / BM;
    p.tiles_n = p.Cout / BN;
    p.xcd_swizzle = g_x3_xcd;
    p.row_swz = 1;
    const size_t lds = (size_t)2 * 3 * (BM + BN) * X3_RS * sizeof(unsigned short);
    static MftPerDeviceOnce attr_once;
    if (attr_once.need()) {
        hipError_t e = hipFuncSetAttribute((const void*)conv_x3_pp_kernel<BM, BN>, hipFuncAttributeMaxDynamicSharedMemorySize, 160 * 1024);
        if (e != hipSuccess) return (int)e;
        attr_once.mark();
    }
    hipLaunchKernelGGL((conv_x3_pp_kernel<BM, BN>), dim3((unsigned)(tiles_m * p.tiles_n)), dim3(512), lds, s, p);
    return mft_launch_status();
}

#endif

#ifdef MFT_EXPERIMENTS
#include "../../tools/experiments/conv3x3_patch_x3.inc"
#endif
int g_x3_patch = 0;
int g_x3_tile = 0;

}

extern "C" int mft_split_bf16x3(const float* w, unsigned short* planes, long long n, void* stream) {
    if (n <= 0) return MFT_EINVAL;
    long long blocks = (n + 255) / 256;
    if (blocks > 4096) blocks = 4096;
    hipLaunchKernelGGL(split_bf16x3_kernel, dim3((unsigned)blocks), dim3(256), 0, (hipStream_t)stream, w, planes, n);
    return mft_launch_status();
}

extern "C" int mft_split_bf16x3_multi(const void* jobs, int n_jobs, long long total_elements, void* stream) {
    if (n_jobs < 1 || total_elements < 1) return MFT_EINVAL;
    long long blocks = (total_elements + 255) / 256;
    if (blocks > 4096) blocks = 4096;
    hipLaunchKernelGGL(split_bf16x3_multi_kernel, dim3((unsigned)blocks), dim3(256), 0, (hipStream_t)stream, (const SplitJob*)jobs, n_jobs,
                       total_elements);
    return mft_launch_status();
}

extern "C" int mft_debug_set_x3_tile(int t) {
#ifndef MFT_EXPERIMENTS
    const bool off = (t == 10 || t == 60 || t == 70 || t == 80 || t == 100 || t == 200);
    if (!off && ((t >= 10 && t < 20) || t == 42 || (t >= 60 && t < 90) || t >= 100)) return MFT_EINVAL;
#endif
    if (t >= 200) g_x3_dbg = t - 200;
    else if (t >= 100) g_x3_min_lds_kb = t - 100;
    else if (t >= 90) g_x3_s1 = t - 90;
    else if (t >= 80) g_x3_hoist = t - 80;
    else if (t >= 70) g_x3_pp = t - 70;
    else if (t >= 60) g_x3_db = t - 60;
    else if (t >= 40) g_x3_row_swz = t - 40;
    else if (t >= 30) g_x3_bdb = t - 30;
    else if (t >= 20) g_x3_xcd = t - 20;
    else if (t >= 10) g_x3_patch = t - 10;
    else g_x3_tile = t;
    return 0;
}

static int x3_dispatch(const float* in, int ldi, const unsigned short* w3, long long plane_elems, float* out, int ldo,
                       int n_img, int H, int W, int Cin, int Cout, int KH, int KW, int stride, int pad, float* stats_ws,
                       int rows_per_group, void* stream,
                       const float* bn_ws = nullptr, const float* bn_gamma = nullptr, const float* bn_beta = nullptr,
                       float bn_eps = 0.f, int np = 3) {
    if (n_img <= 0 || Cin % 32 != 0 || Cout % 64 != 0 || ldi % 4 != 0 || (np != 3 && np != 2)) return MFT_EINVAL;
    if (np == 2 && (g_x3_tile > 1 || g_x3_db || g_x3_pp || g_x3_dbg || g_x3_hoist || g_x3_row_swz == 2 || g_x3_min_lds_kb ||
                    g_x3_patch))
        return MFT_EINVAL;
    X3Args p;
    p.bn_ws = bn_ws; p.bn_gamma = bn_gamma; p.bn_beta = bn_beta; p.bn_eps = bn_eps;
    p.bn_max_tiles = bn_ws ? mft_x3_max_group_tiles(rows_per_group, 128) : 0;
    if (bn_ws != nullptr && (!bn_gamma || !bn_beta || rows_per_group < 128 || KH != 3 || KW != 3 || stride != 1 ||
                             pad != 1 || x3_s1_lds(128, 64, W, Cin, np) > X3_S1_LDS_3PER_CU ||
                             2 * mft_x3_stage_bytes_host(p.bn_max_tiles, Cin) >
                                 (size_t)np * (128 + 18) * X3_RS * sizeof(unsigned short)))
        return MFT_EINVAL;
    p.stats_ws = stats_ws;
    p.rows_per_group = rows_per_group;
    p.in = in; p.w3 = w3; p.plane = plane_elems; p.out = out; p.ldi = ldi; p.ldo = ldo;
    p.H = H; p.W = W; p.Cin = Cin; p.Cout = Cout; p.KH = KH; p.KW = KW; p.stride = stride; p.pad = pad;
    p.OH = (H + 2 * pad - KH) / stride + 1;
    p.OW = (W + 2 * pad - KW) / stride + 1;
    p.Kpad = KH * KW * Cin;
    const long long M = (long long)n_img * p.OH * p.OW;
    if (M > 0x7fffffffLL) return MFT_EINVAL;
    p.M = (int)M;
    p.tiles_n = 0;
    hipStream_t s = (hipStream_t)stream;
    int G = 0, R = 0;
    double eff = 0.0;
#ifdef MFT_EXPERIMENTS
    if (stats_ws == nullptr && g_x3_patch && KH == 3 && KW == 3 && stride == 1 && pad == 1 && ldi == Cin && ldo == Cout &&
        patch_geometry(H, W, &G, &R, &eff) && (g_x3_patch >= 2 || eff >= 0.9)) {
        P3Args q;
        q.in = in; q.w3 = w3; q.plane = plane_elems; q.out = out;
        q.n_img = n_img; q.H = H; q.W = W; q.Cin = Cin; q.Cout = Cout; q.G = G; q.R = R;
        q.row_blocks = (H + R - 1) / R;
        q.tiles_n = Cout / 64;
        const int img_groups = (n_img + G - 1) / G;
        const size_t lds = (size_t)3 * G * (R + 2) * (W + 2) * X3_RS * sizeof(unsigned short);
        static MftPerDeviceOnce attr_once;
        if (attr_once.need()) {
            hipError_t e = hipFuncSetAttribute((const void*)conv3x3_patch_x3_kernel, hipFuncAttributeMaxDynamicSharedMemorySize,
                                               64 * 1024);
            if (e != hipSuccess) return (int)e;
            attr_once.mark();
        }
        if (lds <= 64 * 1024) {
            hipLaunchKernelGGL(conv3x3_patch_x3_kernel, dim3((unsigned)(img_groups * q.row_blocks * q.tiles_n)), dim3(256), lds, s, q);
            return mft_launch_status();
        }
    }
#else
    (void)G; (void)R; (void)eff;
#endif
    int tile = g_x3_tile;
    if (tile == 0) tile = 1;
    p.w_bytes = (unsigned)(np * plane_elems * 2);
    const long long img_bytes = (long long)H * W * ldi * 4;
    const long long max_imgs = 0x7fff0000LL / img_bytes;
    if (max_imgs < 1 || 3 * plane_elems * 2 >= 0x7fff0000LL) return MFT_EINVAL;
    if ((stats_ws != nullptr || bn_ws != nullptr) && (max_imgs < n_img || rows_per_group < 128)) return MFT_EINVAL;
    if (stats_ws != nullptr && tile != 3) tile = 1;
    if (stats_ws != nullptr && tile == 3 && rows_per_group < 64) return MFT_EINVAL;
    for (long long i0 = 0; i0 < n_img; i0 += max_imgs) {
        const long long ni = (n_img - i0 < max_imgs) ? (n_img - i0) : max_imgs;
        X3Args q = p;
        q.in = in + i0 * H * W * ldi;
        q.out = out + i0 * p.OH * p.OW * ldo;
        q.M = (int)(ni * p.OH * p.OW);
        q.in_bytes = (unsigned)(ni * img_bytes);
        const bool s1 = g_x3_s1 && tile == 1 && KH == 3 && KW == 3 && stride == 1 && pad == 1 && !g_x3_db && !g_x3_pp && !g_x3_dbg &&
                        g_x3_hoist == 0 && g_x3_row_swz != 2 && g_x3_min_lds_kb == 0 &&
                        x3_s1_lds(128, 64, W, 0, np) <= 64 * 1024;
        if (bn_ws != nullptr && !s1) return MFT_EINVAL;
        const int rc = s1 ? launch_x3_s1<128, 64>(q, s, np)
                       : np == 2 ? launch_x3<128, 64, false>(q, s, 2)
                       : (tile == 2 && Cout % 128 == 0) ? launch_x3<128, 128, false>(q, s)
                       : (tile == 3)                  ? launch_x3<64, 64, false>(q, s)
#ifdef MFT_EXPERIMENTS
                       : g_x3_db                      ? launch_x3<128, 64, true>(q, s)
                       : (g_x3_pp && !g_x3_dbg)       ? launch_x3_pp<128, 64>(q, s)
#endif
                                                      : launch_x3<128, 64, false>(q, s);
        if (rc != 0) return rc;
    }
    return 0;
}

extern "C" int mft_conv2d_nhwc_x3(const float* in, int ldi, const unsigned short* w3, long long plane_elems, float* out,
                                  int ldo, int n_img, int H, int W, int Cin, int Cout, int KH, int KW, int stride,
                                  int pad, void* stream) {
    return x3_dispatch(in, ldi, w3, plane_elems, out, ldo, n_img, H, W, Cin, Cout, KH, KW, stride, pad, nullptr, 0, stream);
}

extern "C" int mft_split_f16x2(const float* w, unsigned short* planes, long long n, void* stream) {
    if (n <= 0) return MFT_EINVAL;
    long long blocks = (n + 255) / 256;
    if (blocks > 4096) blocks = 4096;
    hipLaunchKernelGGL(split_f16x2_kernel, dim3((unsigned)blocks), dim3(256), 0, (hipStream_t)stream, w, planes, n);
    return mft_launch_status();
}

extern "C" int mft_conv2d_nhwc_h2(const float* in, int ldi, const unsigned short* w2, long long plane_elems, float* out,
                                  int ldo, int n_img, int H, int W, int Cin, int Cout, int KH, int KW, int stride,
                                  int pad, void* stream) {
    return x3_dispatch(in, ldi, w2, plane_elems, out, ldo, n_img, H, W, Cin, Cout, KH, KW, stride, pad, nullptr, 0, stream,
                       nullptr, nullptr, nullptr, 0.f, 2);
}

extern "C" long long mft_conv2d_x3_stats_ws_floats(int n_img, int H, int W, int Cout, int KH, int KW, int stride, int pad) {
    const long long OH = (H + 2 * pad - KH) / stride + 1, OW = (W + 2 * pad - KW) / stride + 1;
    return ((long long)n_img * OH * OW + 63) / 64 * 2 * Cout * 2;
}

static int x3_bnstats(int np, const float* in, int ldi, const unsigned short* w3, long long plane_elems,
                      float* out, int ldo, int n_img, int H, int W, int Cin, int Cout, int KH, int KW,
                      int stride, int pad, int imgs_per_group, float eps, float* stats_ws,
                      float* mean, float* rstd, void* stream) {
    if (imgs_per_group <= 0 || n_img % imgs_per_group != 0 || stats_ws == nullptr) return MFT_EINVAL;
    const int OH = (H + 2 * pad - KH) / stride + 1, OW = (W + 2 * pad - KW) / stride + 1;
    const int R = imgs_per_group * OH * OW;
    const int rc = x3_dispatch(in, ldi, w3, plane_elems, out, ldo, n_img, H, W, Cin, Cout, KH, KW, stride, pad, stats_ws, R,
                               stream, nullptr, nullptr, nullptr, 0.f, np);
    if (rc != 0) return rc;
    if (mean == nullptr && rstd == nullptr) return g_x3_tile == 3 ? MFT_EINVAL : 0;
    const int groups = n_img / imgs_per_group;
    hipLaunchKernelGGL(x3_stats_finalize_kernel, dim3((Cout + 63) / 64, groups), dim3(64), 0, (hipStream_t)stream,
                       (const float*)stats_ws, Cout, n_img * OH * OW, R, g_x3_tile == 3 ? 64 : 128, eps, mean, rstd);
    return mft_launch_status();
}

extern "C" int mft_conv2d_nhwc_x3_bnstats(const float* in, int ldi, const unsigned short* w3, long long plane_elems,
                                          float* out, int ldo, int n_img, int H, int W, int Cin, int Cout, int KH, int KW,
                                          int stride, int pad, int imgs_per_group, float eps, float* stats_ws,
                                          float* mean, float* rstd, void* stream) {
    return x3_bnstats(3, in, ldi, w3, plane_elems, out, ldo, n_img, H, W, Cin, Cout, KH, KW, stride, pad, imgs_per_group, eps, stats_ws, mean,
                      rstd, stream);
}

extern "C" int mft_conv2d_nhwc_h2_bnstats(const float* in, int ldi, const unsigned short* w2, long long plane_elems,
                                          float* out, int ldo, int n_img, int H, int W, int Cin, int Cout, int KH, int KW,
                                          int stride, int pad, int imgs_per_group, float eps, float* stats_ws,
                                          float* mean, float* rstd, void* stream) {
    return x3_bnstats(2, in, ldi, w2, plane_elems, out, ldo, n_img, H, W, Cin, Cout, KH, KW, stride, pad, imgs_per_group, eps, stats_ws, mean,
                      rstd, stream);
}

static int x3_bnin_bnstats(int np, const float* in, int ldi, const float* in_ws, const float* in_gamma,
                           const float* in_beta, const unsigned short* w3, long long plane_elems, float* out,
                           int ldo, int n_img, int H, int W, int Cin, int Cout, int imgs_per_group, float eps,
                           float* stats_ws, float* mean, float* rstd, void* stream) {
    if (imgs_per_group <= 0 || n_img % imgs_per_group != 0 || stats_ws == nullptr || in_ws == nullptr ||
        (mean == nullptr) != (rstd == nullptr) || g_x3_tile == 3)
        return MFT_EINVAL;
    const int R = imgs_per_group * H * W;
    const int rc = x3_dispatch(in, ldi, w3, plane_elems, out, ldo, n_img, H, W, Cin, Cout, 3, 3, 1, 1, stats_ws, R, stream,
                               in_ws, in_gamma, in_beta, eps, np);
    if (rc != 0 || mean == nullptr) return rc;
    hipLaunchKernelGGL(x3_stats_finalize_kernel, dim3((Cout + 63) / 64, n_img / imgs_per_group), dim3(64), 0, (hipStream_t)stream,
                       (const float*)stats_ws, Cout, n_img * H * W, R, 128, eps, mean, rstd);
    return mft_launch_status();
}

extern "C" int mft_conv2d_nhwc_x3_bnin_bnstats(const float* in, int ldi, const float* in_ws, const float* in_gamma,
                                               const float* in_beta, const unsigned short* w3, long long plane_elems, float* out,
                                               int ldo, int n_img, int H, int W, int Cin, int Cout, int imgs_per_group, float eps,
                                               float* stats_ws, float* mean, float* rstd, void* stream) {
    return x3_bnin_bnstats(3, in, ldi, in_ws, in_gamma, in_beta, w3, plane_elems, out, ldo, n_img, H, W, Cin, Cout, imgs_per_group, eps,
                           stats_ws, mean, rstd, stream);
}

extern "C" int mft_conv2d_nhwc_h2_bnin_bnstats(const float* in, int ldi, const float* in_ws, const float* in_gamma,
                                               const float* in_beta, const unsigned short* w2, long long plane_elems, float* out,
                                               int ldo, int n_img, int H, int W, int Cin, int Cout, int imgs_per_group, float eps,
                                               float* stats_ws, float* mean, float* rstd, void* stream) {
    return x3_bnin_bnstats(2, in, ldi, in_ws, in_gamma, in_beta, w2, plane_elems, out, ldo, n_img, H, W, Cin, Cout, imgs_per_group, eps,
                           stats_ws, mean, rstd, stream);
}
```

### meta-fine-tuning_amd/functional.py

```python
import os

import numpy as np

import torch

from . import ops
from . import settings

FUSED_DGRAD = settings.current().fused_dgrad
FUSED_LAST_BLOCK = settings.current().fused_last_block
X3_FUSED_STATS = settings.current().x3_fused_stats
X3_FOLD_BN = settings.current().x3_fold_bn
TRUNK_F16X2 = settings.current().trunk_f16x2
TRAIN_X3 = settings.current().train_x3
TRAIN_X3_MIN_ROWS = settings.current().train_x3_min_rows
F16X2_BOUND = 3.0e4
F16X2_FLOOR = 2.0 ** -10
F16X2_MAX_ROWS = 1 << 20


def stem_rows_bound(ipg, image_size):
    oh = (image_size + 6 - 7) // 2 + 1
    ph = (oh + 2 - 3) // 2 + 1
    h6 = (ph + 2 - 3) // 2 + 1
    side = max(oh, 2 * ph, 4 * h6)
    return int(ipg) * side * side


def f16x2_safe(sd, prefix="", max_rows=None):
    import math
    max_rows = F16X2_MAX_ROWS if max_rows is None else int(max_rows)

    def arr(key):
        return np.abs(sd[prefix + key].detach().float().cpu().numpy())

    def g(name):
        w, b = arr(name + ".weight"), arr(name + ".bias")
        if not float(np.median(w)) >= F16X2_FLOOR:
            return float("inf")
        return float(w.max()) * math.sqrt(max_rows) + float(b.max())

    try:
        x_in = g("trunk.1")
        for idx, (cin, cout, _s) in STAGES.items():
            if idx == 7:
                break
            p = "trunk.%d" % idx
            for cname in (".C1", ".C2") + ((".shortcut",) if cin != cout else ()):
                w = arr(p + cname + ".weight")
                if not (float(w.max()) < F16X2_BOUND and float(np.sqrt(np.mean(np.square(w, dtype=np.float64)))) >= F16X2_FLOOR):
                    return False
            r1 = g(p + ".BN1")
            x_out = g(p + ".BN2") + (g(p + ".BNshortcut") if cin != cout else x_in)
            if not (x_in < F16X2_BOUND and r1 < F16X2_BOUND):
                return False
            x_in = x_out
        return True
    except KeyError:
        return False

STAGES = {4: (64, 64, 1), 5: (64, 128, 2), 6: (128, 256, 2), 7: (256, 512, 2)}

ADAPT_KEYS = [
    "trunk.7.C1.weight", "trunk.7.BN1.weight", "trunk.7.BN1.bias",
    "trunk.7.C2.weight", "trunk.7.BN2.weight", "trunk.7.BN2.bias",
    "trunk.7.shortcut.weight", "trunk.7.BNshortcut.weight", "trunk.7.BNshortcut.bias",
]
ADAPT_SHAPES = {
    "trunk.7.C1.weight": (512, 256, 3, 3), "trunk.7.C2.weight": (512, 512, 3, 3),
    "trunk.7.shortcut.weight": (512, 256, 1, 1),
    "trunk.7.BN1.weight": (512,), "trunk.7.BN1.bias": (512,), "trunk.7.BN2.weight": (512,),
    "trunk.7.BN2.bias": (512,), "trunk.7.BNshortcut.weight": (512,), "trunk.7.BNshortcut.bias": (512,),
}
ADAPT_NUMEL = sum(int(torch.Size(s).numel()) for s in ADAPT_SHAPES.values())


class Arena:

    def __init__(self, device):
        self.device = device
        self.bufs = {}

    def get(self, name, shape, dtype=torch.float32):
        key = (name, tuple(shape), dtype)
        t = self.bufs.get(key)
        if t is None:
            t = torch.empty(tuple(shape), device=self.device, dtype=dtype)
            self.bufs[key] = t
        return t

    def existing(self, name, shape, dtype=torch.float32):
        key = (name, tuple(shape), dtype)
        if key not in self.bufs:
            near = sorted(str(k) for k in self.bufs if k[0] == name)
            raise KeyError("arena has no buffer %r with shape %s%s" % (name, tuple(shape), "; same name, other shapes: " + ", ".join(near) if near else ""))
        return self.bufs[key]

    def nbytes(self):
        return sum(t.numel() * t.element_size() for t in self.bufs.values())


class ResNet10Weights:

    def __init__(self, sd, device, prefix="", x3=False, f16x2=None, max_rows=None):
        self.device = device
        self.conv = {}
        self.conv3 = {}
        self.f16x2_rows = F16X2_MAX_ROWS if max_rows is None else max(int(max_rows), 1)
        if f16x2 is None:
            f16x2 = bool(x3) and TRUNK_F16X2 and f16x2_safe(sd, prefix, self.f16x2_rows)
        self.f16x2 = bool(f16x2)
        split = ops.split_weight_h2 if self.f16x2 else ops.split_weight_x3
        self.bn = {}
        self.plan = ops.PackPlan()
        self.train3 = {}
        self.tplan = ops.SplitPlan()

        def dev(t):
            return t.detach().to(device=device, dtype=torch.float32).contiguous()

        def conv(name):
            src = sd[prefix + name + ".weight"]
            w = dev(src)
            self.conv[name] = ops.pack_conv_weight(w)
            if w.data_ptr() == src.data_ptr():
                self.plan.add(w, self.conv[name])
            if x3 and name.startswith(("trunk.4", "trunk.5", "trunk.6")):
                self.conv3[name] = split(self.conv[name])

        def bn(name):
            self.bn[name] = (dev(sd[prefix + name + ".weight"]), dev(sd[prefix + name + ".bias"]))

        conv("trunk.0")
        bn("trunk.1")
        for idx, (cin, cout, s) in STAGES.items():
            p = "trunk.%d" % idx
            conv(p + ".C1"); bn(p + ".BN1"); conv(p + ".C2"); bn(p + ".BN2")
            if cin != cout:
                conv(p + ".shortcut"); bn(p + ".BNshortcut")

    _STEM_SCALE = {"trunk.4": 2, "trunk.5": 2, "trunk.6": 4}

    def planes(self, p, ipg, H, fixed=None, running=None):
        if not self.conv3 or not self.f16x2:
            return self.conv3
        if fixed is not None or running is not None:
            return {}
        side = self._STEM_SCALE.get(p, 8) * H
        return self.conv3 if ipg * side * side <= self.f16x2_rows else {}

    def repack(self):
        assert self.can_repack()
        self.plan.run()
        self.tplan.run()

    def train_planes(self, name, cin, cout, k, stride, rows_out, transposed=False):
        if not TRAIN_X3 or k != 3 or rows_out < TRAIN_X3_MIN_ROWS:
            return None
        ci, co = (cout, cin) if transposed else (cin, cout)
        if ci % 32 != 0 or co % 64 != 0 or (transposed and stride != 1):
            return None
        key = (name, transposed)
        pl = self.train3.get(key)
        if pl is None:
            if not self.can_repack():
                return None
            pl = self.train3[key] = self.tplan.add(self.conv[name], cout, cin, k * k, transposed)
        return pl

    def can_repack(self):
        return len(self.plan.jobs) == len(self.conv) and not self.conv3


class LastBlockSlab:

    ORDER = [("c1w", 512 * 2304), ("c2w", 512 * 4608), ("scw", 512 * 256),
             ("bn1g", 512), ("bn1b", 512), ("bn2g", 512), ("bn2b", 512), ("bnsg", 512), ("bnsb", 512)]
    KEY = {"c1w": "trunk.7.C1.weight", "c2w": "trunk.7.C2.weight", "scw": "trunk.7.shortcut.weight",
           "bn1g": "trunk.7.BN1.weight", "bn1b": "trunk.7.BN1.bias", "bn2g": "trunk.7.BN2.weight",
           "bn2b": "trunk.7.BN2.bias", "bnsg": "trunk.7.BNshortcut.weight", "bnsb": "trunk.7.BNshortcut.bias"}

    def __init__(self, E, device, zero=True, flat=None):
        self.E = E
        total = E * ADAPT_NUMEL
        if flat is not None:
            assert flat.numel() == total and flat.dtype == torch.float32 and flat.is_contiguous()
            self.flat = flat.zero_() if zero else flat
        else:
            self.flat = torch.zeros(total, device=device) if zero else torch.empty(total, device=device)
        off = 0
        for name, n in self.ORDER:
            v = self.flat[off:off + E * n]
            if name.endswith("w"):
                cout = 512
                v = v.view(E, cout, n // cout)
            else:
                v = v.view(E, n)
            setattr(self, name, v)
            off += E * n
        assert off == total

    def load_shared(self, W):
        self.c1w.copy_(W.conv["trunk.7.C1"].unsqueeze(0).expand_as(self.c1w))
        self.c2w.copy_(W.conv["trunk.7.C2"].unsqueeze(0).expand_as(self.c2w))
        self.scw.copy_(W.conv["trunk.7.shortcut"].unsqueeze(0).expand_as(self.scw))
        for nm, bnname in (("bn1", "trunk.7.BN1"), ("bn2", "trunk.7.BN2"), ("bns", "trunk.7.BNshortcut")):
            g, b = W.bn[bnname]
            getattr(self, nm + "g").copy_(g.unsqueeze(0).expand(self.E, -1))
            getattr(self, nm + "b").copy_(b.unsqueeze(0).expand(self.E, -1))

    def export(self, e):
        out = {}
        for name, _ in self.ORDER:
            key = self.KEY[name]
            t = getattr(self, name)[e]
            if name.endswith("w"):
                out[key] = ops.unpack_conv_weight(t.contiguous(), ADAPT_SHAPES[key])
            else:
                out[key] = t.clone()
        return out


def _bn_stats4(arena, tag, x, ipg, groups, running=None, fixed=None):
    if fixed is not None:
        return fixed
    n, H, W, C = x.shape
    mean = arena.get(tag + ".mean", (groups, C))
    rstd = arena.get(tag + ".rstd", (groups, C))
    rows = ipg * H * W
    nws = max(int(ops._lib.lib().mft_bn_stats_ws_floats(C, rows, groups)), 1)
    ws = arena.get("bn.ws", (max(nws, 1 << 16),)) if nws <= (1 << 16) else arena.get(tag + ".ws", (nws,))
    rm = rv = nbt = None
    if running is not None:
        rm, rv, nbt = running if len(running) == 3 else (running + (None,))
    rc = ops._lib.lib().mft_bn_stats(ops._p(x), C, C, rows, groups, ops.BN_EPS, ops._p(mean), ops._p(rstd), ops._p(ws),
                                     ops._p(rm), ops._p(rv), 0.1, ops._p(nbt), ops._stream())
    ops._lib.check(rc, "mft_bn_stats")
    return mean, rstd


class StemCache:

# ... 113 lines not shown
    return a


def _bn_small(arena, tag, x1, g1, b1, rows, groups, C, gbs, out, x2=None, g2=None, b2=None, res=None, pooled=None, hw=0, stats=None,
              stats2=None):
    m1, s1 = stats if stats is not None else (arena.get(tag + ".mean", (groups, C)), arena.get(tag + ".rstd", (groups, C)))
    m2 = s2 = None
    if x2 is not None:
        m2, s2 = stats2 if stats2 is not None else (arena.get(tag + ".mean2", (groups, C)), arena.get(tag + ".rstd2", (groups, C)))
    rc = ops._lib.lib().mft_bn_small_forward(ops._p(x1), C, ops._p(x2), C, ops._p(res), C, ops._p(out), C, C, rows, groups,
                                             ops._p(g1), ops._p(b1), ops._p(g2), ops._p(b2), gbs, ops._p(m1), ops._p(s1),
                                             ops._p(m2), ops._p(s2), ops.ACT_RELU, 0.0, ops.BN_EPS, ops._p(pooled), hw,
                                             ops._stream())
    ops._lib.check(rc, "mft_bn_small_forward")
    return m1, s1, m2, s2


def simple_block(W, p, x, arena, ipg, cin, cout, stride, running=None, tag="b", slab=None, tape=None, pooled=None, fixed=None,
                 stats_out=None):
    n, H, Wd, _ = x.shape
    groups = n // ipg
    OH = (H + 2 - 3) // stride + 1

    def run(name):
        return None if running is None else running.get(name)

    def fix(name):
        return None if fixed is None else fixed[name]

    if slab is None:
        c1w, c2w = W.conv[p + ".C1"], W.conv[p + ".C2"]
        (g1, b1), (g2, b2) = W.bn[p + ".BN1"], W.bn[p + ".BN2"]
        scw = W.conv.get(p + ".shortcut")
        gs, bs = W.bn.get(p + ".BNshortcut", (None, None))
        gbs = 0
    else:
        c1w, c2w, scw = slab.c1w, slab.c2w, slab.scw
        g1, b1, g2, b2, gs, bs = slab.bn1g, slab.bn1b, slab.bn2g, slab.bn2b, slab.bnsg, slab.bnsb
        gbs = cout
    wipg = ipg if slab is not None else 0
    w3 = W.planes(p, ipg, H, fixed, running) if slab is None else {}

    def conv(name, inp, wpk, k, s, pd, out):
        if (p + name) in w3:
            return ops.conv2d_x3(inp, w3[p + name], cout, k, k, s, pd, out=out)
        return ops.conv2d(inp, wpk, cout, k, k, s, pd, imgs_per_group=wipg, out=out)

    rows = ipg * OH * OH
    if slab is not None and rows <= 64 and cout % 64 == 0 and cin != cout and running is None:
        so = stats_out or {}
        c1 = arena.get(tag + ".c1", (n, OH, OH, cout))
        r1 = arena.get(tag + ".r1", (n * OH * OH, cout))
        sc = arena.get(tag + ".sc", (n, OH, OH, cout))
        rc = ops._lib.MFT_EINVAL
        if FUSED_LAST_BLOCK and c1w.dim() == 3 and scw.dim() == 3 and groups > ops.SMALL_GROUPS and not so:
            m1 = arena.get(tag + ".bn1.mean", (groups, cout))
            s1 = arena.get(tag + ".bn1.rstd", (groups, cout))
            rc = ops._lib.lib().mft_block_entry_small_forward(
                ops._p(x), x.shape[-1], ops._p(c1w), c1w.shape[1] * c1w.shape[2], ops._p(scw), scw.shape[1] * scw.shape[2],
                ops._p(c1), ops._p(r1), ops._p(sc), n, H, Wd, cin, cout, stride, ipg, ops._p(g1), ops._p(b1), gbs, ops._p(m1),
                ops._p(s1), ops.BN_EPS, ops._stream())
            if rc != ops._lib.MFT_EINVAL:
                ops._lib.check(rc, "mft_block_entry_small_forward")
        if rc == ops._lib.MFT_EINVAL:
            conv(".C1", x, c1w, 3, stride, 1, c1)
            m1, s1, _, _ = _bn_small(arena, tag + ".bn1", c1, g1, b1, rows, groups, cout, gbs, r1, stats=so.get("bn1"))
            conv(".shortcut", x, scw, 1, stride, 0, sc)
        r1 = r1.view(n, OH, OH, cout)
        c2 = arena.get(tag + ".c2", (n, OH, OH, cout))
        out = arena.get(tag + ".out", (n * OH * OH, cout))
        rc = ops._lib.MFT_EINVAL
        if FUSED_LAST_BLOCK and pooled is not None and c2w.dim() == 3 and groups > ops.SMALL_GROUPS and not so:
            m2, s2, ms, ss = (arena.get(tag + ".bn2." + k, (groups, cout)) for k in ("mean", "rstd", "mean2", "rstd2"))
            rc = ops._lib.lib().mft_block_exit_small_forward(
                ops._p(r1), ops._p(c2w), c2w.shape[1] * c2w.shape[2], ops._p(sc), ops._p(c2), ops._p(out), ops._p(pooled), n, OH,
                OH, cout, ipg, ops._p(g2), ops._p(b2), ops._p(gs), ops._p(bs), gbs, ops._p(m2), ops._p(s2), ops._p(ms),
                ops._p(ss), ops.BN_EPS, ops._stream())
            if rc != ops._lib.MFT_EINVAL:
                ops._lib.check(rc, "mft_block_exit_small_forward")
        if rc == ops._lib.MFT_EINVAL:
            conv(".C2", r1, c2w, 3, 1, 1, c2)
            m2, s2, ms, ss = _bn_small(arena, tag + ".bn2", c2, g2, b2, rows, groups, cout, gbs, out, x2=sc, g2=gs, b2=bs,
                                       pooled=pooled, hw=OH * OH, stats=so.get("bn2"), stats2=so.get("bns"))
        out = out.view(n, OH, OH, cout)
        if tape is not None:
            tape.update(x=x, c1=c1, m1=m1, s1=s1, r1=r1, c2=c2, m2=m2, s2=s2, sc=sc, ms=ms, ss=ss, out=out,
                        pooled=pooled is not None)
        return out
    fuse_stats = (slab is None and running is None and fixed is None and rows >= 128 and X3_FUSED_STATS)

    def conv_bn(name, bnname, inp, wpk, k, s, pd, obuf, stag):
        if fuse_stats and (p + name) in w3:
            H_in = inp.shape[1]
            nws = int(ops._lib.lib().mft_conv2d_x3_stats_ws_floats(n, H_in, H_in, cout, k, k, s, pd))
            ws = arena.get("x3.statws", (max(nws, 1 << 20),)) if nws <= (1 << 20) else arena.get(stag + ".statws", (nws,))
            mean = arena.get(stag + ".mean", (groups, cout))
            rstd = arena.get(stag + ".rstd", (groups, cout))
            r = ops.conv2d_x3_bnstats(inp, w3[p + name], cout, k, k, s, pd, ipg, obuf, ws, mean, rstd)
            if r is not None:
                return r
        o = conv(name, inp, wpk, k, s, pd, obuf)
        mm, ss_ = _bn_stats4(arena, stag, o, ipg, groups, run(p + bnname), fix(p + bnname))
        return o, mm, ss_

    if (X3_FOLD_BN and fuse_stats and tape is None
            and all((p + nm) in w3 for nm in ((".C1", ".C2", ".shortcut") if cin != cout else (".C1", ".C2")))):
        r = _frozen_block_folded(W, p, x, arena, ipg, cin, cout, stride, tag)
        if r is not None:
            return r

    c1, m1, s1 = conv_bn(".C1", ".BN1", x, c1w, 3, stride, 1, arena.get(tag + ".c1", (n, OH, OH, cout)), tag + ".bn1")
    r1 = ops.bn_apply(c1.view(-1, cout), cout, rows, groups, m1, s1, g1, b1, act=ops.ACT_RELU, fma_affine=fuse_stats,
                      out=arena.get(tag + ".r1", (n * OH * OH, cout)), gb_group_stride=gbs).view(n, OH, OH, cout)
    c2, m2, s2 = conv_bn(".C2", ".BN2", r1, c2w, 3, 1, 1, arena.get(tag + ".c2", (n, OH, OH, cout)), tag + ".bn2")
    out = arena.get(tag + ".out", (n * OH * OH, cout))
    sc = ms = ss = None
    if cin != cout:
        sc, ms, ss = conv_bn(".shortcut", ".BNshortcut", x, scw, 1, stride, 0, arena.get(tag + ".sc", (n, OH, OH, cout)),
                             tag + ".bns")
        ops.bn_apply(c2.view(-1, cout), cout, rows, groups, m2, s2, g2, b2, act=ops.ACT_RELU, fma_affine=fuse_stats, res=sc.view(-1, cout),
                     res_bn=(ms, ss, gs, bs), out=out, gb_group_stride=gbs)
    else:
        ops.bn_apply(c2.view(-1, cout), cout, rows, groups, m2, s2, g2, b2, act=ops.ACT_RELU, fma_affine=fuse_stats, res=x.view(-1, cin),
                     out=out, gb_group_stride=gbs)
    out = out.view(n, OH, OH, cout)
    if tape is not None:
        tape.update(x=x, c1=c1, m1=m1, s1=s1, r1=r1, c2=c2, m2=m2, s2=s2, sc=sc, ms=ms, ss=ss, out=out)
    return out


_X3WS_FITS = {}


def _frozen_block_folded(W, p, x, arena, ipg, cin, cout, stride, tag):
    n, H, _, _ = x.shape
    groups = n // ipg
    OH = (H + 2 - 3) // stride + 1
    rows = ipg * OH * OH
    lib = ops._lib.lib()
    fits = _X3WS_FITS.get((cout, rows))
    if fits is None:
        fits = _X3WS_FITS[(cout, rows)] = bool(lib.mft_bn_apply_x3ws_fits(cout, rows, 1))
    if not fits:
        return None
    (g1, b1), (g2, b2) = W.bn[p + ".BN1"], W.bn[p + ".BN2"]
    w3 = W.conv3

    def partials(name, inp, k, s, pd, obuf, stag):
        ws = arena.get(stag + ".statws", (int(lib.mft_conv2d_x3_stats_ws_floats(n, inp.shape[1], inp.shape[1], cout, k, k, s, pd)),))
        r = ops.conv2d_x3_bnstats(inp, w3[p + name], cout, k, k, s, pd, ipg, obuf, ws, None, None)
        return None if r is None else ws

    c1 = arena.get(tag + ".c1", (n, OH, OH, cout))
    ws1 = partials(".C1", x, 3, stride, 1, c1, tag + ".bn1")
    if ws1 is None:
        return None
    c2 = arena.get(tag + ".c2", (n, OH, OH, cout))
    ws2 = arena.get(tag + ".bn2.statws", (int(lib.mft_conv2d_x3_stats_ws_floats(n, OH, OH, cout, 3, 3, 1, 1)),))
    if ops.conv2d_x3_bnin_bnstats(c1, ws1, g1, b1, w3[p + ".C2"], cout, ipg, c2, ws2) is None:
        r1 = ops.bn_apply_x3ws(c1.view(-1, cout), cout, rows, groups, ws1, g1, b1, arena.get(tag + ".r1", (n * OH * OH, cout)),
                               act=ops.ACT_RELU).view(n, OH, OH, cout)
        if ops.conv2d_x3_bnstats(r1, w3[p + ".C2"], cout, 3, 3, 1, 1, ipg, c2, ws2, None, None) is None:
            raise RuntimeError("frozen block %s: C2 outside the bf16x3 domain after C1 was inside it" % p)
    out = arena.get(tag + ".out", (n * OH * OH, cout))
    if cin != cout:
        gs, bs = W.bn[p + ".BNshortcut"]
        sc = arena.get(tag + ".sc", (n, OH, OH, cout))
        wss = partials(".shortcut", x, 1, stride, 0, sc, tag + ".bns")
        if wss is None:
            raise RuntimeError("frozen block %s: shortcut outside the bf16x3 domain after C1 was inside it" % p)
        ops.bn_apply_x3ws(c2.view(-1, cout), cout, rows, groups, ws2, g2, b2, out, act=ops.ACT_RELU, res=sc.view(-1, cout),
                          res_ws=wss, res_gamma=gs, res_beta=bs)
    else:
        ops.bn_apply_x3ws(c2.view(-1, cout), cout, rows, groups, ws2, g2, b2, out, act=ops.ACT_RELU, res=x.view(-1, cin))
    return out.view(n, OH, OH, cout)


def last_block_forward(W, a, arena, ipg, slab=None, tape=None, running=None, tag="f", fixed=None, stats_out=None):
    n = a.shape[0]
    feat = arena.get(tag + ".feat", (n, 512))
    info = tape if tape is not None else {}
    out = simple_block(W, "trunk.7", a, arena, ipg, 256, 512, 2, running, tag + ".trunk.7", slab=slab, tape=info, pooled=feat,
                       fixed=fixed, stats_out=stats_out)
    if not info.get("pooled", False):
        ops._lib.check(ops._lib.lib().mft_global_avgpool(ops._p(out), ops._p(feat), n, out.shape[1] * out.shape[2], 512,
                                                         ops._stream()), "mft_global_avgpool")
    return feat


def resnet10_forward(W, x, arena, ipg=0, slab=None, tape=None, running=None, tag="f", fixed=None):
    n = x.shape[0]
    if ipg <= 0 or fixed is not None:
        ipg = n
    a = resnet10_trunk(W, x, arena, ipg, upto=7, running=running, tag=tag, fixed=fixed)
    return last_block_forward(W, a, arena, ipg, slab=slab, tape=tape, running=running, tag=tag, fixed=fixed)


def _dgrad_c2_bn1(lib, tape, params, grads, arena, tag, dc2, c1, r1, n, oh, ow, C, ipg, bn_bwd):
    rc = ops._lib.MFT_EINVAL
    if FUSED_LAST_BLOCK and n // ipg > ops.SMALL_GROUPS:
        dc1 = arena.get(tag + ".dc1", tuple(c1.shape))
        w2 = params.c2w
        rc = lib.mft_conv2d_dgrad_bn_backward_small(ops._p(dc2), C, ops._p(w2), ops._p(dc1), C, n, oh, ow, C, C, 3, 3, 1, ipg,
                                                    w2.shape[1] * w2.shape[2], ops._p(c1), ops._p(r1), ops._p(tape["m1"]),
                                                    ops._p(tape["s1"]), ops._p(params.bn1g), C, ops._p(grads.bn1g),
                                                    ops._p(grads.bn1b), ops._stream())
        if rc != ops._lib.MFT_EINVAL:
            ops._lib.check(rc, "mft_conv2d_dgrad_bn_backward_small")
    if rc == ops._lib.MFT_EINVAL:
        dr1 = ops.conv2d_dgrad(dc2, params.c2w, 512, 3, 3, 1, imgs_per_group=ipg, out=arena.get(tag + ".dr1", (n, oh, ow, C)))
        dc1 = bn_bwd(c1, dr1, tape["m1"], tape["s1"], params.bn1g, grads.bn1g, grads.bn1b, r1, "dc1")
    return dc1


def next_step_tape(arena, tag, n, oh, ow, C, groups):
    rows = n * oh * ow
    t = {k: arena.get(tag + "." + k, (n, oh, ow, C)) for k in ("c1", "r1", "c2", "sc", "out")}
    for k in ("m1", "s1", "m2", "s2", "ms", "ss"):
        t[k] = arena.get(tag + "." + k, (groups, C))
    t["feat"] = arena.get(tag + ".feat", (n, C))
    t["pooled"] = True
    assert t["c1"].numel() == rows * C
    return t


def last_block_backward(tape, dfeat, params, grads, arena, ipg, tag="bw", adam=None, ce=None, nxt=None, before_next_read=None):
    x, c1, r1, c2, sc, out = tape["x"], tape["c1"], tape["r1"], tape["c2"], tape["sc"], tape["out"]
    n, oh, ow, C = out.shape
    groups = n // ipg
    rows = ipg * oh * ow
    lib = ops._lib.lib()
    fused_ce = FUSED_LAST_BLOCK and ce is not None and C % 64 == 0 and ipg <= 16
    d_out = None
    if fused_ce:
        pass
    elif ce is not None:
        d_out = arena.get(tag + ".dout", (n, oh, ow, C))
        feat, labels, loss = ce
        ops._lib.check(lib.mft_ce_pool_backward(ops._p(feat), ops._p(labels), ipg, groups, C, oh * ow, ops._p(out), ops._p(d_out),
                                                ops._p(loss), ops._stream()), "mft_ce_pool_backward")
    else:
        d_out = arena.get(tag + ".dout", (n, oh, ow, C))
        ops._lib.check(lib.mft_avgpool_relu_backward(ops._p(dfeat), ops._p(out), ops._p(d_out), n, oh * ow, C,
                                                     ops._stream()), "mft_avgpool_relu_backward")

    def bn_bwd(xraw, dy, mean, rstd, gamma, dgamma, dbeta, relu_out, name, need_dx=True):
        dx = arena.get(tag + "." + name, tuple(xraw.shape)) if need_dx else None
        rc = lib.mft_bn_backward(ops._p(xraw), C, ops._p(dy), C, ops._p(relu_out), C, ops._p(dx), C, C, rows, groups,
                                 ops._p(mean), ops._p(rstd), ops._p(gamma), C, ops._p(dgamma), ops._p(dbeta),
                                 ops._stream())
        ops._lib.check(rc, "mft_bn_backward")
        return dx

    def wgrad(xin, dy, name, k, stride, pad):
        if adam is None:
            ops.conv2d_wgrad(xin, dy, 512, k, k, stride, pad, imgs_per_group=ipg, out=getattr(grads, name))
        else:
            m, v, step, lr = adam
            hyper = step if torch.is_tensor(step) else None
            ops.conv2d_wgrad_adam(xin, dy, getattr(params, name), getattr(m, name), getattr(v, name), 512, k, k,
                                  stride, pad, 1 if hyper is not None else step, imgs_per_group=ipg, lr=lr, hyper=hyper)

    if fused_ce:
        feat, labels, loss = ce
        dc2 = arena.get(tag + ".dc2", tuple(c2.shape))
        dsc = arena.get(tag + ".dsc", tuple(sc.shape))
        rc = lib.mft_ce_pool_bn_backward2(ops._p(feat), ops._p(labels), ipg, groups, C, oh * ow, ops._p(out), ops._p(c2), ops._p(sc),
                                          ops._p(dc2), ops._p(dsc), ops._p(tape["m2"]), ops._p(tape["s2"]), ops._p(params.bn2g),
                                          ops._p(tape["ms"]), ops._p(tape["ss"]), ops._p(params.bnsg), C, ops._p(grads.bn2g),
                                          ops._p(grads.bn2b), ops._p(grads.bnsg), ops._p(grads.bnsb), ops._p(loss), ops._stream())
        ops._lib.check(rc, "mft_ce_pool_bn_backward2")
    elif C % 64 == 0:
        dc2 = arena.get(tag + ".dc2", tuple(c2.shape))
        dsc = arena.get(tag + ".dsc", tuple(sc.shape))
        rc = lib.mft_bn_backward2(ops._p(c2), ops._p(sc), C, ops._p(d_out), C, ops._p(dc2), ops._p(dsc), C, C, rows, groups,
                                  ops._p(tape["m2"]), ops._p(tape["s2"]), ops._p(params.bn2g), ops._p(tape["ms"]),
                                  ops._p(tape["ss"]), ops._p(params.bnsg), C, ops._p(grads.bn2g), ops._p(grads.bn2b),
                                  ops._p(grads.bnsg), ops._p(grads.bnsb), ops._stream())
        ops._lib.check(rc, "mft_bn_backward2")
    else:
        dc2 = bn_bwd(c2, d_out, tape["m2"], tape["s2"], params.bn2g, grads.bn2g, grads.bn2b, None, "dc2")
        dsc = bn_bwd(sc, d_out, tape["ms"], tape["ss"], params.bnsg, grads.bnsg, grads.bnsb, None, "dsc")
    done_c2 = False
    if FUSED_DGRAD and FUSED_LAST_BLOCK and adam is not None and rows <= 64 and C % 64 == 0:
        m_, v_, step, lr = adam
        hyper = step if torch.is_tensor(step) else None
        w2 = params.c2w
        dxp = arena.get(tag + ".dxp", (groups, 9, rows, C))
        dc1 = arena.get(tag + ".dc1", tuple(c1.shape))
        if ops.conv2d_wgrad_adam_dgrad(r1, dc2, w2, m_.c2w, v_.c2w, dxp, 1 if hyper is not None else step, ipg, lr=lr,
                                       hyper=hyper):
            ops._lib.check(lib.mft_col2im_bn_backward_small(ops._p(dxp), ops._p(c1), ops._p(r1), ops._p(dc1), n, oh, ow, C, ipg,
                                                            ops._p(tape["m1"]), ops._p(tape["s1"]), ops._p(params.bn1g), C,
                                                            ops._p(grads.bn1g), ops._p(grads.bn1b), ops._stream()),
                           "mft_col2im_bn_backward_small")
            done_c2 = True
    def adam_tail():
        m, v, step, lr = adam
        nb = params.E * 6 * 512
        hyper = step if torch.is_tensor(step) else None
        ops.adam_step(params.flat[-nb:], grads.flat[-nb:], m.flat[-nb:], v.flat[-nb:], 1 if hyper is not None else step,
                      lr=lr, hyper=hyper)

    if before_next_read is not None and (nxt is None or nxt[0] is None):
        raise RuntimeError("before_next_read given, but this call never reads x_next")
    if nxt is not None:
        assert adam is not None and not done_c2
        x_next, tn = nxt[0], nxt[1]
        waited = [before_next_read is None]

        def wait_next_once():
            if not waited[0]:
                before_next_read()
                waited[0] = True
        m_, v_, step, lr = adam
        hyper = step if torch.is_tensor(step) else None
        st = 1 if hyper is not None else step
        dc1 = _dgrad_c2_bn1(lib, tape, params, grads, arena, tag, dc2, c1, r1, n, oh, ow, C, ipg, bn_bwd)
        adam_tail()
        kw = dict(lr=lr, hyper=hyper)
        fw = x_next is not None
        if fw:
            wait_next_once()
        ok = ops.wgrad_adam_next_forward(x, dsc, params.scw, m_.scw, v_.scw, 1, 1, 2, 0, st, ipg, x_next=x_next, mode=ops.WF_RAW,
                                         raw=tn["sc"] if fw else None, **kw)
        ok = ok and ops.wgrad_adam_next_forward(x, dc1, params.c1w, m_.c1w, v_.c1w, 3, 3, 2, 1, st, ipg, x_next=x_next,
                                                mode=ops.WF_ENTRY, raw=tn["c1"] if fw else None, act=tn["r1"] if fw else None,
# ... 219 lines not shown
```

### meta-fine-tuning_amd/ops.py

```python
import ctypes
import os

import torch

from . import _lib
from . import settings

ACT_NONE, ACT_RELU, ACT_LRELU = 0, 1, 2
BN_EPS = 1e-5
LRELU_SLOPE = 0.01


import threading

_tls = threading.local()


def _stream(t=None):
    dev = getattr(_tls, "dev", None)
    _tls.dev = None
    if t is not None:
        dev = t.device.index if torch.is_tensor(t) else (t.index if isinstance(t, torch.device) else int(t))
    return ctypes.c_void_p(torch.cuda.current_stream(dev).cuda_stream)

# ... 78 lines not shown
        if self.table is None:
            import numpy as np
            self.table = torch.from_numpy(np.asarray(self.jobs, dtype=np.int64)).to(self.keep[0][1].device)
        _lib.check(_lib.lib().mft_pack_oihw_multi(_p(self.table), len(self.jobs), self.total, _stream()), "mft_pack_oihw_multi")


class SplitPlan:

    def __init__(self):
        self.jobs, self.total, self.table, self.keep = [], 0, None, []
        self.retired = []

    def add(self, pk, Cout, Cin, taps, transposed=False):
        assert pk.is_cuda and pk.dtype == torch.float32 and pk.is_contiguous() and pk.shape == (Cout, taps * Cin) and (taps * Cin) % 32 == 0
        if torch.cuda.is_current_stream_capturing():
            raise RuntimeError("SplitPlan.add() under stream capture: run one eager step first (the planes of every layer are "
                               "registered by the first forward)")
        n = pk.numel()
        planes = torch.empty((3, Cin, taps * Cout) if transposed else (3, Cout, taps * Cin), device=pk.device, dtype=torch.int16)
        self.jobs.append((pk.data_ptr(), planes.data_ptr(), n, Cout, Cin, taps, 1 if transposed else 0, self.total))
        self.total += n
        self.keep.append((pk, planes))
        if self.table is not None:
            self.retired.append(self.table)
        self.table = None
        self._launch(len(self.jobs) - 1)
        return planes

    def _launch(self, only=None):
        import numpy as np
        if only is not None:
            j = list(self.jobs[only])
            j[7] = 0
            tab = torch.from_numpy(np.asarray([j], dtype=np.int64)).to(self.keep[only][0].device)
            _lib.check(_lib.lib().mft_split_bf16x3_multi(_p(tab), 1, j[2], _stream()), "mft_split_bf16x3_multi")
            return
        if self.table is None:
            self.table = torch.from_numpy(np.asarray(self.jobs, dtype=np.int64)).to(self.keep[0][0].device)
        _lib.check(_lib.lib().mft_split_bf16x3_multi(_p(self.table), len(self.jobs), self.total, _stream()), "mft_split_bf16x3_multi")

    def run(self):
        if self.jobs:
            self._launch()


def unpack_conv_weight(pk, shape):
    Cout, Cin, KH, KW = shape
    w = torch.empty(shape, device=pk.device, dtype=torch.float32)
    _lib.check(_lib.lib().mft_unpack_oihw(_p(pk), _p(w), Cout, Cin, KH, KW, pk.shape[-1], _stream()), "mft_unpack_oihw")
    return w


def pack_dgrad_weight(w_pk, Cout, Cin, KH, KW, groups=1):
    w_pk = _f32c(w_pk)
    K = KH * KW * Cin
    wt = torch.empty((groups, Cin, KH * KW * Cout), device=w_pk.device, dtype=torch.float32)
    _lib.check(_lib.lib().mft_pack_dgrad(_p(w_pk), _p(wt), Cout, Cin, KH, KW, groups, Cout * K, Cin * KH * KW * Cout,
                                         _stream()), "mft_pack_dgrad")
    return wt



def conv2d(x, w_pk, Cout, KH, KW, stride, pad, imgs_per_group=0, bias=None, out=None):
    _f32c(x)
    n, H, W, Cin = x.shape
    OH = (H + 2 * pad - KH) // stride + 1
    OW = (W + 2 * pad - KW) // stride + 1
    if out is None:
        out = torch.empty((n, OH, OW, Cout), device=x.device, dtype=torch.float32)
    wgs = 0
    if w_pk.dim() == 3:
        wgs = w_pk.shape[1] * w_pk.shape[2]
        if imgs_per_group <= 0 or n // imgs_per_group != w_pk.shape[0]:
            raise RuntimeError("per-group weights need imgs_per_group with n/imgs_per_group == groups")
    if ((wgs == 0 and imgs_per_group <= 0) or (w_pk.dim() == 3 and w_pk.shape[0] == 1)) and Cin != 3:
        nws = _ksplit_ws(n * OH * OW, Cout, w_pk.shape[-1])
        if nws:
            ws = torch.empty((nws,), device=x.device, dtype=torch.float32)
            rc = _lib.lib().mft_conv2d_nhwc_ksplit(_p(x), Cin, _p(w_pk), _p(bias), _p(out), Cout, n, H, W, Cin, Cout, KH, KW,
                                                   stride, pad, _p(ws), _stream())
            _lib.check(rc, "mft_conv2d_nhwc_ksplit")
            return out
    if w_pk.dim() == 3 and 1 < w_pk.shape[0] <= SMALL_GROUPS and bias is None and Cin != 3:
        G = w_pk.shape[0]
        nws = _ksplit_ws(imgs_per_group * OH * OW, Cout, w_pk.shape[-1], G)
        if nws:
            ws = torch.empty((nws,), device=x.device, dtype=torch.float32)
            rc = _lib.lib().mft_conv2d_nhwc_ksplit_grouped(_p(x), Cin, _p(w_pk), _p(out), Cout, n, H, W, Cin, Cout, KH, KW, stride, pad,
                                                           imgs_per_group, wgs, _p(ws), _stream())
            _lib.check(rc, "mft_conv2d_nhwc_ksplit_grouped")
            return out
    rc = _lib.lib().mft_conv2d_nhwc(_p(x), Cin, _p(w_pk), _p(bias), _p(out), Cout, n, H, W, Cin, Cout, KH, KW,
                                    stride, pad, imgs_per_group, wgs, _stream())
    _lib.check(rc, "mft_conv2d_nhwc")
    return out


SMALL_GROUPS = settings.current().small_groups
_KSPLIT_WS = {}


def _ksplit_ws(rows, cols, K, groups=1):
    key = (rows, cols, K, groups)
    v = _KSPLIT_WS.get(key)
    if v is None:
        v = _KSPLIT_WS[key] = int(_lib.lib().mft_conv_ksplit_ws_floats(rows, cols, K) if groups == 1 else
                                  _lib.lib().mft_conv_ksplit_grouped_ws_floats(rows, cols, K, groups))
    return v


def split_weight_x3(w_pk):
    _f32c(w_pk)
    planes = torch.empty((3,) + tuple(w_pk.shape), device=w_pk.device, dtype=torch.int16)
    _lib.check(_lib.lib().mft_split_bf16x3(_p(w_pk), _p(planes), w_pk.numel(), _stream()), "mft_split_bf16x3")
    return planes


def split_weight_h2(w_pk):
    _f32c(w_pk)
    planes = torch.empty((2,) + tuple(w_pk.shape), device=w_pk.device, dtype=torch.int16)
    _lib.check(_lib.lib().mft_split_f16x2(_p(w_pk), _p(planes), w_pk.numel(), _stream()), "mft_split_f16x2")
    return planes


def _x3_fn(w3, stem):
    kind = {3: "x3", 2: "h2"}[int(w3.shape[0])]
    name = "mft_conv2d_nhwc_%s%s" % (kind, stem)
    return getattr(_lib.lib(), name), name


def conv2d_x3(x, w3, Cout, KH, KW, stride, pad, out=None):
    _f32c(x)
    n, H, W, Cin = x.shape
    OH = (H + 2 * pad - KH) // stride + 1
    OW = (W + 2 * pad - KW) // stride + 1
    if out is None:
        out = torch.empty((n, OH, OW, Cout), device=x.device, dtype=torch.float32)
    fn, name = _x3_fn(w3, "")
    rc = fn(_p(x), Cin, _p(w3), w3.shape[1] * w3.shape[2], _p(out), Cout, n, H, W, Cin, Cout, KH, KW, stride, pad, _stream())
    _lib.check(rc, name)
    return out


def conv2d_x3_bnstats(x, w3, Cout, KH, KW, stride, pad, imgs_per_group, out, ws, mean, rstd, eps=BN_EPS):
    _f32c(x)
    n, H, W, Cin = x.shape
    fn, name = _x3_fn(w3, "_bnstats")
    rc = fn(_p(x), Cin, _p(w3), w3.shape[1] * w3.shape[2], _p(out), Cout, n, H, W, Cin, Cout, KH, KW, stride, pad, imgs_per_group, eps,
            _p(ws), _p(mean), _p(rstd), _stream())
    if rc == _lib.MFT_EINVAL:
        return None
    _lib.check(rc, name)
    return out, mean, rstd


def conv2d_x3_bnin_bnstats(c_raw, in_ws, in_gamma, in_beta, w3, Cout, imgs_per_group, out, ws, mean=None, rstd=None, eps=BN_EPS):
    _f32c(c_raw)
    n, H, W, Cin = c_raw.shape
    fn, name = _x3_fn(w3, "_bnin_bnstats")
    rc = fn(_p(c_raw), Cin, _p(in_ws), _p(in_gamma), _p(in_beta), _p(w3), w3.shape[1] * w3.shape[2], _p(out), Cout, n, H, W, Cin, Cout,
            imgs_per_group, eps, _p(ws), _p(mean), _p(rstd), _stream())
    if rc == _lib.MFT_EINVAL:
        return None
    _lib.check(rc, name)
    return out


def bn_apply_x3ws(x2d, C, rows_per_group, n_groups, ws, gamma, beta, out, act=ACT_NONE, res=None, res_ws=None, res_gamma=None,
                  res_beta=None, slope=LRELU_SLOPE, eps=BN_EPS, stats=None, res_stats=None):
    _f32c(x2d)
    m, r = stats if stats is not None else (None, None)
    rm, rr = res_stats if res_stats is not None else (None, None)
    rc = _lib.lib().mft_bn_apply_x3ws(_p(x2d), x2d.shape[-1], _p(out), out.shape[-1], C, rows_per_group, n_groups, _p(ws), _p(gamma),
                                      _p(beta), _p(res), 0 if res is None else res.shape[-1], _p(res_ws), _p(res_gamma),
                                      _p(res_beta), act, slope, eps, _p(m), _p(r), _p(rm), _p(rr), _stream())
    _lib.check(rc, "mft_bn_apply_x3ws")
    return out


def gemm(a, K, w_pk, N, bias=None, out=None, ldo=None, rows_per_group=0):
    _f32c(a)
    M, lda = a.shape
    if out is None:
        ldo = N if ldo is None else ldo
        out = torch.empty((M, ldo), device=a.device, dtype=torch.float32)
    else:
        ldo = out.shape[1]
    wgs = 0
    if w_pk.dim() == 3:
        wgs = w_pk.shape[1] * w_pk.shape[2]
    rc = _lib.lib().mft_conv2d_nhwc(_p(a), lda, _p(w_pk), _p(bias), _p(out), ldo, M, 1, 1, K, N, 1, 1, 1, 0,
                                    rows_per_group, wgs, _stream())
    _lib.check(rc, "mft_conv2d_nhwc(gemm)")
    return out


def gemm_rk(a, K, w_pk, N, bias=None, out=None, ldo=None):
    _f32c(a)
    M, lda = a.shape
    assert w_pk.dim() == 2 and w_pk.shape[1] == K and w_pk.shape[0] >= N and K % 16 == 0 and K <= 512, (tuple(w_pk.shape), K, N)
    if out is None:
        ldo = N if ldo is None else ldo
        out = torch.empty((M, ldo), device=a.device, dtype=torch.float32)
    else:
        ldo = out.shape[1]
    _lib.check(_lib.lib().mft_gemm_rk(_p(a), lda, _p(w_pk), w_pk.shape[0], K, _p(bias), _p(out), ldo, M, N, _stream()), "mft_gemm_rk")
    return out


def conv2d_dgrad(dy, w_pk, Cin, KH, KW, pad, imgs_per_group=0, out=None, stride=1, in_hw=None):
    _f32c(dy)
    n, OH, OW, Cout = dy.shape
    H, W = (OH, OW) if in_hw is None else in_hw
    if out is None:
        out = torch.empty((n, H, W, Cin), device=dy.device, dtype=torch.float32)
    wgs = w_pk.shape[1] * w_pk.shape[2] if w_pk.dim() == 3 else 0
    if ((wgs == 0 and imgs_per_group <= 0) or (w_pk.dim() == 3 and w_pk.shape[0] == 1)) and Cin % 64 == 0:
        nws = _ksplit_ws(n * H * W, Cin, KH * KW * Cout)
        if nws:
            ws = torch.empty((nws,), device=dy.device, dtype=torch.float32)
            rc = _lib.lib().mft_conv2d_dgrad_nhwc_ksplit(_p(dy), Cout, _p(w_pk), _p(out), Cin, n, H, W, Cin, Cout, KH, KW, stride, pad,
                                                         _p(ws), _stream())
            _lib.check(rc, "mft_conv2d_dgrad_nhwc_ksplit")
            return out
    if w_pk.dim() == 3 and 1 < w_pk.shape[0] <= SMALL_GROUPS and Cin % 64 == 0 and stride == 1 and imgs_per_group > 0:
        nws = _ksplit_ws(imgs_per_group * H * W, Cin, KH * KW * Cout, w_pk.shape[0])
        if nws:
            ws = torch.empty((nws,), device=dy.device, dtype=torch.float32)
            rc = _lib.lib().mft_conv2d_dgrad_nhwc_ksplit_grouped(_p(dy), Cout, _p(w_pk), _p(out), Cin, n, H, W, Cin, Cout, KH, KW, stride,
                                                                 pad, imgs_per_group, wgs, _p(ws), _stream())
            _lib.check(rc, "mft_conv2d_dgrad_nhwc_ksplit_grouped")
            return out
    rc = _lib.lib().mft_conv2d_dgrad_nhwc(_p(dy), Cout, _p(w_pk), _p(out), Cin, n, H, W, Cin, Cout, KH, KW, stride, pad,
                                          imgs_per_group, wgs, _stream())
    _lib.check(rc, "mft_conv2d_dgrad_nhwc")
    return out


def conv2d_wgrad(x, dy, Cout, KH, KW, stride, pad, imgs_per_group=0, out=None, ldy=None):
    _f32c(x)
    _f32c(dy)
    n, H, W, Cin = x.shape
    groups = 1 if imgs_per_group <= 0 else n // imgs_per_group
    K = round_up(KH * KW * Cin, 32)
    if out is None:
        out = torch.empty((groups, Cout, K), device=x.device, dtype=torch.float32)
    nws = int(_lib.lib().mft_conv2d_wgrad_ws_floats(n, H, W, Cin, Cout, KH, KW, stride, pad, imgs_per_group))
    ws = torch.empty((nws,), device=x.device, dtype=torch.float32) if nws > 0 else None
    rc = _lib.lib().mft_conv2d_wgrad_nhwc(_p(x), Cin, _p(dy), dy.shape[-1] if ldy is None else ldy, _p(out), n, H, W,
                                          Cin, Cout, KH, KW, stride, pad, imgs_per_group, Cout * K, _p(ws), _stream())
    _lib.check(rc, "mft_conv2d_wgrad_nhwc")
    return out


def conv2d_wgrad_oihw(x, dy, Cout, KH, KW, stride, pad, cin_valid=0, cout_valid=0, out=None):
    _f32c(x)
    _f32c(dy)
    n, H, W, Cin = x.shape
    if out is None:
        out = torch.empty((cout_valid or Cout, cin_valid or Cin, KH, KW), device=x.device, dtype=torch.float32)
    ws = torch.empty((int(_lib.lib().mft_conv2d_wgrad_oihw_ws_floats(n, H, W, Cin, Cout, KH, KW, stride, pad)),), device=x.device,
                     dtype=torch.float32)
    rc = _lib.lib().mft_conv2d_wgrad_oihw(_p(x), Cin, _p(dy), dy.shape[-1], _p(out), n, H, W, Cin, Cout, KH, KW, stride, pad,
                                          cin_valid, cout_valid, _p(ws), _stream())
    _lib.check(rc, "mft_conv2d_wgrad_oihw")
    return out


class _WgradJob(ctypes.Structure):
    _fields_ = [("inp", ctypes.c_void_p), ("dy", ctypes.c_void_p), ("dw", ctypes.c_void_p), ("ws", ctypes.c_void_p)] + \
               [(n, ctypes.c_int) for n in ("ldi", "ldy", "n_img", "H", "W", "Cin", "Cout", "KH", "KW", "stride", "pad", "cin_valid",
                                            "cout_valid", "reserved")]


class WgradBatch:

    def __init__(self, enabled=True):
        self.enabled = enabled
        self.jobs, self.keep, self.after = [], [], []

    def add(self, x, dy, Cout, KH, KW, stride, pad, cin_valid=0, cout_valid=0):
        if not self.enabled:
            return conv2d_wgrad_oihw(x, dy, Cout, KH, KW, stride, pad, cin_valid, cout_valid)
        _f32c(x)
        _f32c(dy)
        n, H, W, Cin = x.shape
        out = torch.empty((cout_valid or Cout, cin_valid or Cin, KH, KW), device=x.device, dtype=torch.float32)
        ws = torch.empty((int(_lib.lib().mft_conv2d_wgrad_oihw_ws_floats(n, H, W, Cin, Cout, KH, KW, stride, pad)),), device=x.device,
                         dtype=torch.float32)
        self.jobs.append((x.data_ptr(), dy.data_ptr(), out.data_ptr(), ws.data_ptr(), Cin, dy.shape[-1], n, H, W, Cin, Cout, KH, KW, stride,
                          pad, cin_valid, cout_valid, 0))
        self.keep.append((x, dy, out, ws))
        return out

    def then(self, fn):
        if not self.enabled:
            fn()
        else:
            self.after.append(fn)

    def flush(self):
        if self.jobs:
            arr = (_WgradJob * len(self.jobs))(*[_WgradJob(*j) for j in self.jobs])
            dev = self.keep[0][0].device
            _lib.check(_lib.lib().mft_conv2d_wgrad_oihw_multi(arr, len(self.jobs), _stream(dev)), "mft_conv2d_wgrad_oihw_multi")
        for fn in self.after:
# ... 798 lines not shown
```

### meta-fine-tuning_amd/settings.py

```python
import dataclasses
import os


def _flag(v):
    lv = v.strip().lower()
    if lv in ("1", "true", "yes", "on"):
        return True
    if lv in ("0", "false", "no", "off"):
        return False
    raise ValueError("expected 0 / 1 (or true / false), got %r" % (v,))


def _opt_int(v):
    return None if v in ("", "none", "None") else int(v)


def _fuse(v):
    if v not in ("auto", "0", "1"):
        raise ValueError("expected auto, 0 or 1, got %r" % (v,))
    return v


KNOBS = (
    ("fuse_next", "MFT_FUSE_NEXT", _fuse, "auto", "fused weight-gradient + Adam + next-step forward launches: auto = engine.fuse_next_policy | 1 | 0"),
    ("wf_xcd", "MFT_WF_XCD", _flag, True, "fused launch: all workgroups of an episode on one XCD (A/B hook; read once per process)"),
    ("slab_candidates", "MFT_SLAB_CANDIDATES", _opt_int, None, "candidate buffers of the w/m/v placement scan (None: engine default 12; 0: off)"),
    ("slab_ballast_gb", "MFT_SLAB_BALLAST_GB", float, 12.0, "throw-away allocation between groups of placement candidates, GB"),
    ("slab_hints", "MFT_SLAB_HINTS", _flag, True, "re-use an earlier scan's placement when one probe confirms it"),
    ("trunk_chunk", "MFT_TRUNK_CHUNK", _opt_int, None, "inner steps per frozen-trunk launch set (None: 32 at E = 1, else 1)"),
    ("trunk_priority", "MFT_TRUNK_PRIORITY", int, 1, "HIP priority of the frozen-trunk stream (1 = the device's least)"),
    ("last_priority", "MFT_LAST_PRIORITY", int, -1, "torch priority of the last-block stream"),
    ("debug_skip_trunk", "MFT_DEBUG_SKIP_TRUNK", _flag, False, "measurement aid: reuse one cached trunk output (results are WRONG)"),
    ("adapt_graph", "MFT_ADAPT_GRAPH", _flag, True, "adapt_last_block: replay the meta-fine-tuning inner loop from one hipGraph"),
    ("adapt_batched_trunk", "MFT_ADAPT_BATCHED_TRUNK", _flag, True, "adapt_last_block: frozen trunk of all steps as two grouped passes"),
    ("fused_dgrad", "MFT_FUSED_DGRAD", _flag, False, "one-pass trunk.7.C2 weight gradient + Adam + data gradient (measured slower in the step)"),
    ("x3_fused_stats", "MFT_X3_FUSED_STATS", _flag, True, "BatchNorm statistics from the split-precision convolution epilogue"),
    ("x3_fold_bn", "MFT_X3_FOLD_BN", _flag, True, "frozen blocks without helper launches (per-tile partials merged by the consumers)"),
    ("trunk_f16x2", "MFT_TRUNK_F16X2", _flag, True, "frozen trunk.4-6 on two fp16 pieces per operand (0: three bf16 pieces)"),
    ("stem_pooled", "MFT_STEM_POOLED", _flag, True, "stem cache keeps per-window (max, min) instead of the full-resolution output"),
    ("stem_fused_fill", "MFT_STEM_FUSED_FILL", _flag, True, "stem cache filled by ONE launch (convolution + moments + window min/max; 0: three launches through a full-resolution buffer)"),
    ("stem_chunk", "MFT_STEM_CHUNK", _opt_int, None, "images per stem-cache fill launch (None: StemCache's default)"),
    ("fused_last_block", "MFT_FUSED_LAST_BLOCK", _flag, True, "conv + BatchNorm fusions of the adapted block (csrc/skinny.hip)"),
    ("small_groups", "MFT_SMALL_GROUPS", int, 12, "up to this many per-episode weight sets take the K-sliced GEMM route"),
    ("fused_pair_mlp", "MFT_FUSED_PAIR_MLP", _flag, True, "Wcompute on the fused upper-triangle pair-MLP kernels"),
    ("pair_mlp_gb", "MFT_PAIR_MLP_GB", float, 6.0, "memory budget of the fused pair-MLP's hidden activations per chunk, GB"),
    ("train_graph", "MFT_TRAIN_GRAPH", _flag, True, "MetaTemplate episode loop: loss + backward replayed from one hipGraph"),
    ("train_x3", "MFT_TRAIN_X3", _flag, True, "meta-training: 3x3 layers with >= 8192 output rows on the bf16x3 kernels, forward and stride-1 data gradient (0: fp32 MFMA everywhere)"),
    ("train_x3_min_rows", "MFT_TRAIN_X3_MIN_ROWS", int, 6000, "meta-training: output rows from which a 3x3 layer takes the bf16x3 kernels (below: fp32 MFMA with K slices; measured at 3,780 / 945 rows in profiles/r06_q_train_x3_min_rows.txt)"),
    ("wgrad_batch", "MFT_WGRAD_BATCH", _flag, True, "meta-training backward: every layer's weight gradient deferred to the end of the pass and run in one multi-problem launch pair per 16 layers (0: one launch pair per layer, as round 5; bit-identical)"),
    ("pair_f16x2", "MFT_PAIR_F16X2", _flag, False, "GNN pair-MLP layers (Wcompute) as f16x2 products on the fp16 matrix cores (fp32-accurate; 0: fp32 MFMA)"),
    ("gemm_rk_rows", "MFT_GEMM_RK_ROWS", int, 4096, "meta-training: head linear layers (fc, Gconv.fc) of at most this many rows take the skinny register-K GEMM (0: the tile kernel always)"),
    ("pair_rk_rows", "MFT_PAIR_RK_ROWS", int, 16384, "meta-training: Wcompute layers over at most this many pair rows (all episodes of the step) take the register-K small-problem kernel, 32-row tiles, no LDS staging (0: the 128-row tile kernel always)"),
    ("train_source", "MFT_TRAIN_SOURCE", str, "pool", "train.main --dataset miniImageNet: 'pool' = resident uint8 class pool, 'synthetic' = host fp32 episodes"),
    ("standin_weights", "MFT_STANDIN_WEIGHTS", _flag, False, "allow synthetic stand-in weights when no checkpoint is found (explicit opt-in)"),
    ("image_size", "MFT_IMAGE_SIZE", int, 84, "image side the CLI evaluates at (84 = BASELINE; 224 = the reference's)"),
    ("episodes", "MFT_EPISODES", _opt_int, None, "override of the CLI's episode count (None: 600)"),
    ("episodes_per_batch", "MFT_EPISODES_PER_BATCH", _opt_int, None, "override of the CLI's lockstep batch (None: 128 / 96 / 64 by n_shot)"),
    ("timings", "MFT_TIMINGS", _flag, False, "print the drivers' phase timings to stderr"),
    ("pool_per_class", "MFT_POOL_PER_CLASS", _opt_int, None, "images per class of the dataset-shaped resident pool (None: the dataset's)"),
    ("synth_on_host", "MFT_SYNTH_ON_HOST", _flag, False, "generate synthetic test episodes with numpy on the host instead of on the device"),
    ("balance_batches", "MFT_BALANCE_BATCHES", _flag, True, "equalise the lockstep batch sizes of an evaluation"),
    ("force_collectives", "MFT_FORCE_COLLECTIVES", _flag, False, "run the N-rank collectives even with one rank (1-GPU RCCL tests)"),
    ("one_device", "MFT_ONE_DEVICE", _flag, False, "test hook: W ranks share device 0, gloo for the gathers"),
)


@dataclasses.dataclass(frozen=True)
class Settings:
    fuse_next: str = "auto"
    wf_xcd: bool = True
    slab_candidates: "int | None" = None
    slab_ballast_gb: float = 12.0
    slab_hints: bool = True
    trunk_chunk: "int | None" = None
    trunk_priority: int = 1
    last_priority: int = -1
    debug_skip_trunk: bool = False
    adapt_graph: bool = True
    adapt_batched_trunk: bool = True
    fused_dgrad: bool = False
    x3_fused_stats: bool = True
    x3_fold_bn: bool = True
    trunk_f16x2: bool = True
    stem_pooled: bool = True
    stem_fused_fill: bool = True
    stem_chunk: "int | None" = None
    fused_last_block: bool = True
    small_groups: int = 12
    fused_pair_mlp: bool = True
    pair_mlp_gb: float = 6.0
    train_graph: bool = True
    train_x3: bool = True
    train_x3_min_rows: int = 6000
    wgrad_batch: bool = True
    pair_f16x2: bool = False
    gemm_rk_rows: int = 4096
    pair_rk_rows: int = 16384
    train_source: str = "pool"
    standin_weights: bool = False
    image_size: int = 84
    episodes: "int | None" = None
    episodes_per_batch: "int | None" = None
    timings: bool = False
    pool_per_class: "int | None" = None
    synth_on_host: bool = False
    balance_batches: bool = True
    force_collectives: bool = False
    one_device: bool = False

    @classmethod
    def from_env(cls, env=None):
        env = os.environ if env is None else env
        kw = {}
        for field, var, parse, default, _ in KNOBS:
            raw = env.get(var)
            if raw is None:
                kw[field] = default
                continue
            try:
                kw[field] = parse(raw)
            except (TypeError, ValueError) as e:
                raise ValueError("%s=%r: %s" % (var, raw, e)) from None
        s = cls(**kw)
        if s.train_source not in ("pool", "synthetic"):
            raise ValueError("MFT_TRAIN_SOURCE=%r: expected pool or synthetic" % (s.train_source,))
        if s.image_size < 32:
            raise ValueError("MFT_IMAGE_SIZE out of range")
        return s


assert tuple(f.name for f in dataclasses.fields(Settings)) == tuple(k[0] for k in KNOBS), "KNOBS and Settings fields must match"
_VARS = tuple(k[1] for k in KNOBS)
_cache = (None, None)


def current():
    global _cache
    key = tuple(os.environ.get(v) for v in _VARS)
    if _cache[0] != key:
        _cache = (key, Settings.from_env())
    return _cache[1]


IMPORT_TIME = frozenset((
    "debug_skip_trunk", "adapt_graph", "adapt_batched_trunk", "fused_dgrad", "fused_last_block", "x3_fused_stats",
    "x3_fold_bn", "trunk_f16x2", "train_x3", "train_x3_min_rows", "fused_pair_mlp", "pair_f16x2", "pair_rk_rows", "gemm_rk_rows", "pair_mlp_gb", "wgrad_batch",
    "train_graph", "small_groups", "wf_xcd",
))
assert IMPORT_TIME <= set(k[0] for k in KNOBS), IMPORT_TIME - set(k[0] for k in KNOBS)


def describe():
    return "\n".join("%-26s %-22s %-7s default %-8r %s" % (var, field, "import" if field in IMPORT_TIME else "live", default, doc)
                     for field, var, _, default, doc in KNOBS)
```

Before: 86.87.

## Fuse shortcut conv into C1 grid and finish block exit inside C2 launch

In frozen ResNet blocks, the 1x1 strided shortcut convolution now runs as extra workgroups inside C1's launch through a paired kernel. C2 gains an exit variant in which the last workgroup per (group, N tile), tracked by atomic counters, finalises the BN stats and applies BN, residual and ReLU itself. Exit counters are zeroed by the C1 launch. This removes two launches per block and a separate bn_apply pass, at the cost of atomic stores, a serial tail in the last workgroup and extra LDS needs.

Measured after the change: 87.58, median of 6. Within noise of the previous version (+0.8%).

```diff
diff --git a/include/mft_hip.h b/include/mft_hip.h
--- a/include/mft_hip.h
+++ b/include/mft_hip.h
@@ -88,6 +88,30 @@
                                     const unsigned short* w2, long long plane_elems, float* out, int ldo, int n_img, int H, int W,
                                     int Cin, int Cout, int imgs_per_group, float eps, float* stats_ws, float* mean, float* rstd,
                                     void* stream);
+int mft_conv2d_nhwc_x3_pair_bnstats(const float* in, int ldi, int n_img, int H, int W, int Cin, int Cout, int stride,
+                                    int imgs_per_group, const unsigned short* w_c1, long long plane_c1, float* out_c1, int ldo_c1,
+                                    float* ws_c1, const unsigned short* w_sc, long long plane_sc, float* out_sc, int ldo_sc,
+                                    float* ws_sc, int* zero_cnt, int n_zero, void* stream);
+int mft_conv2d_nhwc_h2_pair_bnstats(const float* in, int ldi, int n_img, int H, int W, int Cin, int Cout, int stride,
+                                    int imgs_per_group, const unsigned short* w_c1, long long plane_c1, float* out_c1, int ldo_c1,
+                                    float* ws_c1, const unsigned short* w_sc, long long plane_sc, float* out_sc, int ldo_sc,
+                                    float* ws_sc, int* zero_cnt, int n_zero, void* stream);
+int mft_conv2d_nhwc_x3_bnstats_zero(const float* in, int ldi, const unsigned short* w3, long long plane_elems, float* out, int ldo,
+                                    int n_img, int H, int W, int Cin, int Cout, int KH, int KW, int stride, int pad,
+                                    int imgs_per_group, float* stats_ws, int* zero_cnt, int n_zero, void* stream);
+int mft_conv2d_nhwc_h2_bnstats_zero(const float* in, int ldi, const unsigned short* w2, long long plane_elems, float* out, int ldo,
+                                    int n_img, int H, int W, int Cin, int Cout, int KH, int KW, int stride, int pad,
+                                    int imgs_per_group, float* stats_ws, int* zero_cnt, int n_zero, void* stream);
+int mft_conv2d_nhwc_x3_bnin_bnstats_exit(const float* in, int ldi, const float* in_ws, const float* in_gamma, const float* in_beta,
+                                         const unsigned short* w3, long long plane_elems, float* out, int ldo, int n_img, int H, int W,
+                                         int Cin, int Cout, int imgs_per_group, float eps, float* stats_ws, const float* gamma,
+                                         const float* beta, const float* res, int ldr, const float* res_ws, const float* res_gamma,
+                                         const float* res_beta, float* y, int ldy, int* cnt, void* stream);
+int mft_conv2d_nhwc_h2_bnin_bnstats_exit(const float* in, int ldi, const float* in_ws, const float* in_gamma, const float* in_beta,
+                                         const unsigned short* w2, long long plane_elems, float* out, int ldo, int n_img, int H, int W,
+                                         int Cin, int Cout, int imgs_per_group, float eps, float* stats_ws, const float* gamma,
+                                         const float* beta, const float* res, int ldr, const float* res_ws, const float* res_gamma,
+                                         const float* res_beta, float* y, int ldy, int* cnt, void* stream);
 int mft_bn_apply_x3ws(const float* x, int ldx, float* y, int ldy, int C, int rows_per_group, int n_groups, const float* ws,
                       const float* gamma, const float* beta, const float* res, int ldr, const float* res_ws,
                       const float* res_gamma, const float* res_beta, int act, float slope, float eps, float* mean, float* rstd,
diff --git a/meta-fine-tuning_amd/_lib.py b/meta-fine-tuning_amd/_lib.py
--- a/meta-fine-tuning_amd/_lib.py
+++ b/meta-fine-tuning_amd/_lib.py
@@ -113,6 +113,12 @@
     "mft_conv2d_nhwc_h2": [_P, _I, _P, _L, _P, _I, _I, _I, _I, _I, _I, _I, _I, _I, _I, _P],
     "mft_conv2d_nhwc_h2_bnstats": [_P, _I, _P, _L, _P, _I, _I, _I, _I, _I, _I, _I, _I, _I, _I, _I, _F, _P, _P, _P, _P],
     "mft_conv2d_nhwc_h2_bnin_bnstats": [_P, _I, _P, _P, _P, _P, _L, _P, _I, _I, _I, _I, _I, _I, _I, _F, _P, _P, _P, _P],
+    "mft_conv2d_nhwc_x3_pair_bnstats": [_P, _I, _I, _I, _I, _I, _I, _I, _I, _P, _L, _P, _I, _P, _P, _L, _P, _I, _P, _P, _I, _P],
+    "mft_conv2d_nhwc_x3_bnstats_zero": [_P, _I, _P, _L, _P, _I, _I, _I, _I, _I, _I, _I, _I, _I, _I, _I, _P, _P, _I, _P],
+    "mft_conv2d_nhwc_x3_bnin_bnstats_exit": [_P, _I, _P, _P, _P, _P, _L, _P, _I, _I, _I, _I, _I, _I, _I, _F, _P, _P, _P, _P, _I, _P, _P, _P, _P, _I, _P, _P],
+    "mft_conv2d_nhwc_h2_pair_bnstats": [_P, _I, _I, _I, _I, _I, _I, _I, _I, _P, _L, _P, _I, _P, _P, _L, _P, _I, _P, _P, _I, _P],
+    "mft_conv2d_nhwc_h2_bnstats_zero": [_P, _I, _P, _L, _P, _I, _I, _I, _I, _I, _I, _I, _I, _I, _I, _I, _P, _P, _I, _P],
+    "mft_conv2d_nhwc_h2_bnin_bnstats_exit": [_P, _I, _P, _P, _P, _P, _L, _P, _I, _I, _I, _I, _I, _I, _I, _F, _P, _P, _P, _P, _I, _P, _P, _P, _P, _I, _P, _P],
     "mft_bn_apply_x3ws": [_P, _I, _P, _I, _I, _I, _I, _P, _P, _P, _P, _I, _P, _P, _P, _I, _F, _F, _P, _P, _P, _P, _P],
     "mft_bn_apply_x3ws_fits": [_I, _I, _I],
     "mft_bn_running_ema": [_P, _P, _I, _P, _P, _I, _P, _I, _I, _F, _F, _P, _P, _P],
diff --git a/meta-fine-tuning_amd/csrc/conv_x3.hip b/meta-fine-tuning_amd/csrc/conv_x3.hip
--- a/meta-fine-tuning_amd/csrc/conv_x3.hip
+++ b/meta-fine-tuning_amd/csrc/conv_x3.hip
@@ -30,6 +30,12 @@
     const float* bn_ws; const float* bn_gamma; const float* bn_beta;
     float bn_eps;
     int bn_max_tiles;
+    int* exit_cnt;
+    float* exit_out; int exit_ldo;
+    const float* exit_gamma; const float* exit_beta;
+    const float* exit_res; int exit_ldr;
+    const float* exit_rws; const float* exit_rgamma; const float* exit_rbeta;
+    int* zero_cnt; int n_zero;
 };
 
 constexpr int X3_RS = 40;
@@ -67,7 +73,7 @@
 constexpr float X3_H2_LO_SCALE = 1.0f / 2048.f;
 
 template <int BM, int BN, bool DB, int HOIST = 0, int DBG = 0, bool XS = false, int NP = 3>
-__global__ __launch_bounds__(256) __attribute__((amdgpu_waves_per_eu(NP == 2 ? 3 : 1))) void conv_x3_kernel(X3Args p) {
+__device__ __forceinline__ void conv_x3_body(const X3Args& p, const int wg, const int nwg) {
     static_assert(NP == 3 || (NP == 2 && !DB && HOIST == 0 && DBG == 0 && !XS), "f16x2: the plain single-buffer form only");
     constexpr int NACC = NP == 3 ? 1 : 2;
     constexpr int TM = BM / 64;
@@ -91,9 +97,11 @@
     const int wm = wave >> 1, wn = wave & 1;
     const int r = lane & 31, h = lane >> 5;
     const bool g_swz = !XS && p.row_swz != 0;
-    int tile_id = blockIdx.x;
+    if (p.zero_cnt != nullptr && wg == 0)
+        for (int i = tid; i < p.n_zero; i += 256) p.zero_cnt[i] = 0;
+    int tile_id = wg;
     if (p.xcd_swizzle) {
-        const int nwg = gridDim.x, q = nwg >> 3, rmd = nwg & 7;
+        const int q = nwg >> 3, rmd = nwg & 7;
         const int xcd = tile_id & 7, slot = tile_id >> 3;
         tile_id = xcd * q + (xcd < rmd ? xcd : rmd) + slot;
     }
@@ -414,12 +422,28 @@
     }
 }
 
+template <int BM, int BN, bool DB, int HOIST = 0, int DBG = 0, bool XS = false, int NP = 3>
+__global__ __launch_bounds__(256) __attribute__((amdgpu_waves_per_eu(NP == 2 ? 3 : 1))) void conv_x3_kernel(X3Args p) {
+    conv_x3_body<BM, BN, DB, HOIST, DBG, XS, NP>(p, blockIdx.x, gridDim.x);
+}
+
+struct X3PairArgs { X3Args q[2]; int split; };
+
+template <int BM, int BN, int NP>
+__global__ __launch_bounds__(256) __attribute__((amdgpu_waves_per_eu(NP == 2 ? 3 : 1))) void conv_x3_pair_kernel(X3PairArgs a) {
+    const int second = (int)blockIdx.x >= a.split;
+    const X3Args& p = a.q[second];
+    conv_x3_body<BM, BN, false, 0, 0, false, NP>(p, second ? (int)blockIdx.x - a.split : (int)blockIdx.x,
+                                                 second ? (int)gridDim.x - a.split : a.split);
+}
+
 #ifdef MFT_EXPERIMENTS
 #include "../../tools/experiments/conv_x3_pingpong.inc"
 #endif
 
-template <int BM, int BN, bool BNIN, int NP = 3, bool BDB = true>
+template <int BM, int BN, bool BNIN, int NP = 3, bool BDB = true, bool EXIT = false>
 __device__ __forceinline__ void conv_x3_s1_body(const X3Args& p) {
+    static_assert(!EXIT || BNIN, "the exit belongs to C2");
     static_assert(NP == 3 || NP == 2, "3 bf16 pieces (six products) or 2 fp16 pieces (three products)");
     constexpr int NACC = NP == 3 ? 1 : 2;
     constexpr int TM = BM / 64, TN = BN / 64;
@@ -447,6 +471,8 @@
     const int mt = tile_id / p.tiles_n;
     const int m0 = mt * BM, n0 = nt * BN;
     const int W = p.W, H = p.H;
+    if (p.zero_cnt != nullptr && blockIdx.x == 0)
+        for (int i = tid; i < p.n_zero; i += 256) p.zero_cnt[i] = 0;
     const int fr0 = m0 / W;
     const int g0 = BNIN ? m0 / p.rows_per_group : 0;
     const bool bn_two = BNIN && (m0 + (BM < p.M - m0 ? BM : p.M - m0) - 1) / p.rows_per_group > g0;
@@ -708,6 +734,10 @@
         }
     }
 
+    auto put = [](float* dst, float v) {
+        if constexpr (EXIT) __hip_atomic_store(dst, v, __ATOMIC_RELAXED, __HIP_MEMORY_SCOPE_AGENT);
+        else *dst = v;
+    };
 #pragma unroll
     for (int i = 0; i < TM; ++i)
 #pragma unroll
@@ -717,7 +747,7 @@
             for (int e = 0; e < 16; ++e) {
                 const int row = (e & 3) + 8 * (e >> 2) + 4 * h;
                 const int m = m0 + wm * (BM / 2) + i * 32 + row;
-                if (m < p.M) p.out[(long long)m * p.ldo + n] = val(i, j, e);
+                if (m < p.M) put(p.out + (long long)m * p.ldo + n, val(i, j, e));
             }
         }
     if (p.stats_ws != nullptr) {
@@ -755,8 +785,105 @@
                 const int n = n0 + wn * (BN / 2) + j * 32 + r;
                 float* w0 = p.stats_ws + (((long long)mt * 2 + 0) * p.Cout + n) * 2;
                 float* w1 = p.stats_ws + (((long long)mt * 2 + 1) * p.Cout + n) * 2;
-                w0[0] = o0[0] + o1[0]; w0[1] = o0[1] + o1[1];
-                w1[0] = o0[2] + o1[2]; w1[1] = o0[3] + o1[3];
+                put(w0, o0[0] + o1[0]); put(w0 + 1, o0[1] + o1[1]);
+                put(w1, o0[2] + o1[2]); put(w1 + 1, o0[3] + o1[3]);
+            }
+        }
+    }
+    if constexpr (EXIT) {
+        static_assert(BN == 64, "exit tables");
+        asm volatile("s_waitcnt vmcnt(0)" ::: "memory");
+        __syncthreads();
+        int* last = reinterpret_cast<int*>(smem);
+        const int R = p.rows_per_group;
+        const int g_hi = (m0 + (BM < p.M - m0 ? BM : p.M - m0) - 1) / R;
+        if (tid == 0) {
+            bool any = false;
+#pragma unroll
+            for (int gi = 0; gi < 2; ++gi) {
+                const int g = m0 / R + gi;
+                int is_last = 0;
+                if (g <= g_hi) {
+                    const MftTileSpan sp = mft_x3_group_tiles(g, p.M, R, BM);
+                    const int old = __hip_atomic_fetch_add(p.exit_cnt + (long long)g * p.tiles_n + nt, 1, __ATOMIC_RELAXED, __HIP_MEMORY_SCOPE_AGENT);
+                    is_last = old == sp.t1 - sp.t0;
+                }
+                last[gi] = is_last;
+                any |= is_last != 0;
+            }
+            if (any) {
+                __builtin_amdgcn_fence(__ATOMIC_ACQUIRE, "agent");
+                asm volatile("s_waitcnt vmcnt(0)" ::: "memory");
+            }
+        }
+        __syncthreads();
+        const int last0 = last[0], last1 = last[1];
+        if (last0 | last1) {
+            const int mx = p.bn_max_tiles;
+            MftTileW* wt = reinterpret_cast<MftTileW*>(smem + 16);
+            mft_f32x2* part = reinterpret_cast<mft_f32x2*>(wt + mx);
+            mft_f32x2* rpart = part + mx * BN;
+            float* tab = reinterpret_cast<float*>(rpart + mx * BN);
+#pragma unroll 1
+            for (int gi = 0; gi < 2; ++gi) {
+                if (!(gi == 0 ? last0 : last1)) continue;
+                const int g = m0 / R + gi;
+                const MftTileSpan sp = mft_x3_group_tiles(g, p.M, R, BM);
+                const int ntl = sp.t1 - sp.t0 + 1;
+                __syncthreads();
+                for (int i = tid; i < ntl; i += 256) wt[i] = mft_x3_tile_weights(sp.t0 + i, g, p.M, R, BM);
+                for (int i = tid; i < ntl * BN; i += 256) {
+                    const int tt = i / BN, c = i - tt * BN, t = sp.t0 + tt;
+                    const long long o = (((long long)t * 2 + mft_x3_tile_seg(t, g, R, BM)) * p.Cout + n0 + c) * 2;
+                    part[i] = *(const mft_f32x2*)(p.stats_ws + o);
+                    if (p.exit_rws) rpart[i] = *(const mft_f32x2*)(p.exit_rws + o);
+                }
+                __syncthreads();
+                if (tid < BN) {
+                    const int c = tid;
+                    float mu, rs, sc, sh;
+                    mft_x3_stats_chain([&](int t, int) { return part[(t - sp.t0) * BN + c]; }, [&](int t) { return wt[t - sp.t0]; }, g, p.M, R,
+                                       BM, p.bn_eps, mu, rs);
+                    mft_bn_fold(mu, rs, p.exit_gamma[n0 + c], p.exit_beta[n0 + c], sc, sh);
+                    tab[c] = sc; tab[BN + c] = sh;
+                    if (p.exit_rws) {
+                        mft_x3_stats_chain([&](int t, int) { return rpart[(t - sp.t0) * BN + c]; }, [&](int t) { return wt[t - sp.t0]; }, g,
+                                           p.M, R, BM, p.bn_eps, mu, rs);
+                        mft_bn_fold(mu, rs, p.exit_rgamma[n0 + c], p.exit_rbeta[n0 + c], sc, sh);
+                        tab[2 * BN + c] = sc; tab[3 * BN + c] = sh;
+                    }
+                }
+                __syncthreads();
+                const int r0 = g * R, r1 = r0 + R < p.M ? r0 + R : p.M;
+                const int total = (r1 - r0) * (BN / 4);
+                constexpr int EXIT_U = 8;
+                for (int i0 = tid; i0 < total; i0 += 256 * EXIT_U) {
+                    f32x4 v[EXIT_U], rv[EXIT_U];
+#pragma unroll
+                    for (int u = 0; u < EXIT_U; ++u) {
+                        const int i = i0 + u * 256;
+                        const int ic = i < total ? i : total - 1;
+                        const int rr = ic / (BN / 4), c = (ic - rr * (BN / 4)) * 4;
+                        const long long row = (long long)r0 + rr;
+                        v[u] = *(const f32x4*)(p.out + row * p.ldo + n0 + c);
+                        rv[u] = *(const f32x4*)(p.exit_res + row * p.exit_ldr + n0 + c);
+                    }
+#pragma unroll
+                    for (int u = 0; u < EXIT_U; ++u) {
+                        const int i = i0 + u * 256;
+                        if (i < total) {
+                            const int rr = i / (BN / 4), c = (i - rr * (BN / 4)) * 4;
+                            const long long row = (long long)r0 + rr;
+                            f32x4 o = mft_bn_affine4(v[u], *(const f32x4*)(tab + c), *(const f32x4*)(tab + BN + c));
+                            f32x4 r_ = rv[u];
+                            if (p.exit_rws) r_ = mft_bn_affine4(r_, *(const f32x4*)(tab + 2 * BN + c), *(const f32x4*)(tab + 3 * BN + c));
+                            o += r_;
+#pragma unroll
+                            for (int e = 0; e < 4; ++e) o[e] = fmaxf(o[e], 0.f);
+                            *(f32x4*)(p.exit_out + row * p.exit_ldo + n0 + c) = o;
+                        }
+                    }
+                }
             }
         }
     }
@@ -770,6 +897,11 @@
 template <int BM, int BN, int NP = 3, bool BDB = true>
 __global__ __launch_bounds__(256) __attribute__((amdgpu_waves_per_eu(3, 3))) void conv_x3_s1_bnin_kernel(X3Args p) {
     conv_x3_s1_body<BM, BN, true, NP, BDB>(p);
+}
+
+template <int BM, int BN, int NP = 3>
+__global__ __launch_bounds__(256) __attribute__((amdgpu_waves_per_eu(3, 3))) void conv_x3_s1_bnin_exit_kernel(X3Args p) {
+    conv_x3_s1_body<BM, BN, true, NP, true, true>(p);
 }
 
 __global__ void x3_stats_finalize_kernel(const float* __restrict__ ws, int C, int M, int R, int BM, float eps,
@@ -923,6 +1055,13 @@
     p.s1_rows = BM + 18;
     const size_t lds = x3_s1_lds(BM, BN, p.W, p.bn_ws ? p.Cin : 0, np);
     const dim3 grid((unsigned)(tiles_m * p.tiles_n));
+    if (p.exit_cnt != nullptr) {
+        const size_t need = 32 + (size_t)p.bn_max_tiles * (16 + 2 * BN * 8) + 4 * BN * sizeof(float);
+        if (!p.bn_ws || (np == 2 && !g_x3_bdb) || need > lds) return MFT_EINVAL;
+        if (np == 2) hipLaunchKernelGGL((conv_x3_s1_bnin_exit_kernel<BM, BN, 2>), grid, dim3(256), lds, s, p);
+        else hipLaunchKernelGGL((conv_x3_s1_bnin_exit_kernel<BM, BN, 3>), grid, dim3(256), lds, s, p);
+        return mft_launch_status();
+    }
     if (np == 2 && g_x3_bdb) {
         if (p.bn_ws) hipLaunchKernelGGL((conv_x3_s1_bnin_kernel<BM, BN, 2, true>), grid, dim3(256), lds, s, p);
         else hipLaunchKernelGGL((conv_x3_s1_kernel<BM, BN, 2, true>), grid, dim3(256), lds, s, p);
@@ -1003,16 +1142,28 @@
     return 0;
 }
 
+static void x3_no_extras(X3Args& p) {
+    p.exit_cnt = nullptr; p.exit_out = nullptr; p.exit_ldo = 0; p.exit_gamma = nullptr; p.exit_beta = nullptr; p.exit_res = nullptr;
+    p.exit_ldr = 0; p.exit_rws = nullptr; p.exit_rgamma = nullptr; p.exit_rbeta = nullptr; p.zero_cnt = nullptr; p.n_zero = 0;
+}
+
 static int x3_dispatch(const float* in, int ldi, const unsigned short* w3, long long plane_elems, float* out, int ldo,
                        int n_img, int H, int W, int Cin, int Cout, int KH, int KW, int stride, int pad, float* stats_ws,
                        int rows_per_group, void* stream,
                        const float* bn_ws = nullptr, const float* bn_gamma = nullptr, const float* bn_beta = nullptr,
-                       float bn_eps = 0.f, int np = 3) {
+                       float bn_eps = 0.f, int np = 3, const X3Args* extra = nullptr) {
     if (n_img <= 0 || Cin % 32 != 0 || Cout % 64 != 0 || ldi % 4 != 0 || (np != 3 && np != 2)) return MFT_EINVAL;
     if (np == 2 && (g_x3_tile > 1 || g_x3_db || g_x3_pp || g_x3_dbg || g_x3_hoist || g_x3_row_swz == 2 || g_x3_min_lds_kb ||
                     g_x3_patch))
         return MFT_EINVAL;
     X3Args p;
+    x3_no_extras(p);
+    if (extra != nullptr) {
+        p.exit_cnt = extra->exit_cnt; p.exit_out = extra->exit_out; p.exit_ldo = extra->exit_ldo;
+        p.exit_gamma = extra->exit_gamma; p.exit_beta = extra->exit_beta; p.exit_res = extra->exit_res; p.exit_ldr = extra->exit_ldr;
+        p.exit_rws = extra->exit_rws; p.exit_rgamma = extra->exit_rgamma; p.exit_rbeta = extra->exit_rbeta;
+        p.zero_cnt = extra->zero_cnt; p.n_zero = extra->n_zero;
+    }
     p.bn_ws = bn_ws; p.bn_gamma = bn_gamma; p.bn_beta = bn_beta; p.bn_eps = bn_eps;
     p.bn_max_tiles = bn_ws ? mft_x3_max_group_tiles(rows_per_group, 128) : 0;
     if (bn_ws != nullptr && (!bn_gamma || !bn_beta || rows_per_group < 128 || KH != 3 || KW != 3 || stride != 1 ||
@@ -1078,7 +1229,7 @@
         const bool s1 = g_x3_s1 && tile == 1 && KH == 3 && KW == 3 && stride == 1 && pad == 1 && !g_x3_db && !g_x3_pp && !g_x3_dbg &&
                         g_x3_hoist == 0 && g_x3_row_swz != 2 && g_x3_min_lds_kb == 0 &&
                         x3_s1_lds(128, 64, W, 0, np) <= 64 * 1024;
-        if (bn_ws != nullptr && !s1) return MFT_EINVAL;
+        if ((bn_ws != nullptr || p.exit_cnt != nullptr) && !s1) return MFT_EINVAL;
         const int rc = s1 ? launch_x3_s1<128, 64>(q, s, np)
                        : np == 2 ? launch_x3<128, 64, false>(q, s, 2)
                        : (tile == 2 && Cout % 128 == 0) ? launch_x3<128, 128, false>(q, s)
@@ -1152,6 +1303,67 @@
                       rstd, stream);
 }
 
+static int x3_pair_bnstats(int np, const float* in, int ldi, int n_img, int H, int W, int Cin, int Cout, int stride, int imgs_per_group,
+                           const unsigned short* w_c1, long long plane_c1, float* out_c1, int ldo_c1, float* ws_c1,
+                           const unsigned short* w_sc, long long plane_sc, float* out_sc, int ldo_sc, float* ws_sc, int* zero_cnt,
+                           int n_zero, void* stream) {
+    if (n_img <= 0 || imgs_per_group <= 0 || n_img % imgs_per_group != 0 || Cin % 32 != 0 || Cout % 64 != 0 || ldi % 4 != 0 ||
+        (np != 3 && np != 2) || stride < 2 || ldi < Cin || ldo_c1 < Cout || ldo_sc < Cout || H < 1 || W < 1 || !in || !w_c1 || !w_sc || !out_c1 || !out_sc || !ws_c1 || !ws_sc)
+        return MFT_EINVAL;
+    if (g_x3_tile > 1 || g_x3_db || g_x3_pp || g_x3_dbg || g_x3_hoist || g_x3_row_swz == 2 || g_x3_min_lds_kb || g_x3_patch)
+        return MFT_EINVAL;
+    const int OH = (H + 2 - 3) / stride + 1, OW = (W + 2 - 3) / stride + 1;
+    if (OH != (H - 1) / stride + 1 || OW != (W - 1) / stride + 1) return MFT_EINVAL;
+    const long long M = (long long)n_img * OH * OW, R = (long long)imgs_per_group * OH * OW;
+    const long long img_bytes = (long long)H * W * ldi * 4;
+    if (M > 0x7fffffffLL || R < 128 || img_bytes * n_img > 0x7fff0000LL || 3 * plane_c1 * 2 >= 0x7fff0000LL ||
+        plane_c1 < (long long)Cout * 9 * Cin || plane_sc < (long long)Cout * Cin)
+        return MFT_EINVAL;
+    X3PairArgs a;
+    for (int i = 0; i < 2; ++i) {
+        X3Args& p = a.q[i];
+        const int k = i == 0 ? 3 : 1;
+        p.in = in; p.ldi = ldi; p.in_bytes = (unsigned)(n_img * img_bytes);
+        p.w3 = i == 0 ? w_c1 : w_sc; p.plane = i == 0 ? plane_c1 : plane_sc; p.w_bytes = (unsigned)(np * p.plane * 2);
+        p.out = i == 0 ? out_c1 : out_sc; p.ldo = i == 0 ? ldo_c1 : ldo_sc;
+        p.H = H; p.W = W; p.Cin = Cin; p.OH = OH; p.OW = OW; p.Cout = Cout; p.KH = k; p.KW = k; p.stride = stride; p.pad = i == 0 ? 1 : 0;
+        p.Kpad = k * k * Cin;
+        p.M = (int)M;
+        p.tiles_n = Cout / 64;
+        p.xcd_swizzle = g_x3_xcd;
+        p.row_swz = g_x3_row_swz != 0;
+        p.stats_ws = i == 0 ? ws_c1 : ws_sc;
+        p.rows_per_group = (int)R;
+        p.s1_rows = 0;
+        p.bn_ws = nullptr; p.bn_gamma = nullptr; p.bn_beta = nullptr; p.bn_eps = 0.f; p.bn_max_tiles = 0;
+        x3_no_extras(p);
+    }
+    if (n_zero < 0 || (n_zero > 0 && !zero_cnt)) return MFT_EINVAL;
+    a.q[0].zero_cnt = n_zero > 0 ? zero_cnt : nullptr; a.q[0].n_zero = n_zero;
+    const int tiles = (int)((M + 127) / 128) * (Cout / 64);
+    a.split = tiles;
+    const size_t lds = (size_t)np * (128 + 64) * X3_RS * sizeof(unsigned short);
+    if (np == 2) hipLaunchKernelGGL((conv_x3_pair_kernel<128, 64, 2>), dim3((unsigned)(2 * tiles)), dim3(256), lds, (hipStream_t)stream, a);
+    else hipLaunchKernelGGL((conv_x3_pair_kernel<128, 64, 3>), dim3((unsigned)(2 * tiles)), dim3(256), lds, (hipStream_t)stream, a);
+    return mft_launch_status();
+}
+
+extern "C" int mft_conv2d_nhwc_x3_pair_bnstats(const float* in, int ldi, int n_img, int H, int W, int Cin, int Cout, int stride,
+                                               int imgs_per_group, const unsigned short* w_c1, long long plane_c1, float* out_c1,
+                                               int ldo_c1, float* ws_c1, const unsigned short* w_sc, long long plane_sc,
+                                               float* out_sc, int ldo_sc, float* ws_sc, int* zero_cnt, int n_zero, void* stream) {
+    return x3_pair_bnstats(3, in, ldi, n_img, H, W, Cin, Cout, stride, imgs_per_group, w_c1, plane_c1, out_c1, ldo_c1, ws_c1, w_sc, plane_sc,
+                           out_sc, ldo_sc, ws_sc, zero_cnt, n_zero, stream);
+}
+
+extern "C" int mft_conv2d_nhwc_h2_pair_bnstats(const float* in, int ldi, int n_img, int H, int W, int Cin, int Cout, int stride,
+                                               int imgs_per_group, const unsigned short* w_c1, long long plane_c1, float* out_c1,
+                                               int ldo_c1, float* ws_c1, const unsigned short* w_sc, long long plane_sc,
+                                               float* out_sc, int ldo_sc, float* ws_sc, int* zero_cnt, int n_zero, void* stream) {
+    return x3_pair_bnstats(2, in, ldi, n_img, H, W, Cin, Cout, stride, imgs_per_group, w_c1, plane_c1, out_c1, ldo_c1, ws_c1, w_sc, plane_sc,
+                           out_sc, ldo_sc, ws_sc, zero_cnt, n_zero, stream);
+}
+
 static int x3_bnin_bnstats(int np, const float* in, int ldi, const float* in_ws, const float* in_gamma,
                            const float* in_beta, const unsigned short* w3, long long plane_elems, float* out,
                            int ldo, int n_img, int H, int W, int Cin, int Cout, int imgs_per_group, float eps,
@@ -1183,3 +1395,67 @@
     return x3_bnin_bnstats(2, in, ldi, in_ws, in_gamma, in_beta, w2, plane_elems, out, ldo, n_img, H, W, Cin, Cout, imgs_per_group, eps,
                            stats_ws, mean, rstd, stream);
 }
+
+static int x3_bnstats_zero(int np, const float* in, int ldi, const unsigned short* w3, long long plane_elems, float* out, int ldo, int n_img,
+                           int H, int W, int Cin, int Cout, int KH, int KW, int stride, int pad, int imgs_per_group, float* stats_ws,
+                           int* zero_cnt, int n_zero, void* stream) {
+    if (imgs_per_group <= 0 || n_img % imgs_per_group != 0 || stats_ws == nullptr || zero_cnt == nullptr || n_zero < 1 || g_x3_tile == 3)
+        return MFT_EINVAL;
+    const int OH = (H + 2 * pad - KH) / stride + 1, OW = (W + 2 * pad - KW) / stride + 1;
+    X3Args ex;
+    x3_no_extras(ex);
+    ex.zero_cnt = zero_cnt; ex.n_zero = n_zero;
+    return x3_dispatch(in, ldi, w3, plane_elems, out, ldo, n_img, H, W, Cin, Cout, KH, KW, stride, pad, stats_ws, imgs_per_group * OH * OW,
+                       stream, nullptr, nullptr, nullptr, 0.f, np, &ex);
+}
+
+extern "C" int mft_conv2d_nhwc_x3_bnstats_zero(const float* in, int ldi, const unsigned short* w3, long long plane_elems, float* out, int ldo,
+                                               int n_img, int H, int W, int Cin, int Cout, int KH, int KW, int stride, int pad,
+                                               int imgs_per_group, float* stats_ws, int* zero_cnt, int n_zero, void* stream) {
+    return x3_bnstats_zero(3, in, ldi, w3, plane_elems, out, ldo, n_img, H, W, Cin, Cout, KH, KW, stride, pad, imgs_per_group, stats_ws, zero_cnt,
+                           n_zero, stream);
+}
+
+extern "C" int mft_conv2d_nhwc_h2_bnstats_zero(const float* in, int ldi, const unsigned short* w2, long long plane_elems, float* out, int ldo,
+                                               int n_img, int H, int W, int Cin, int Cout, int KH, int KW, int stride, int pad,
+                                               int imgs_per_group, float* stats_ws, int* zero_cnt, int n_zero, void* stream) {
+    return x3_bnstats_zero(2, in, ldi, w2, plane_elems, out, ldo, n_img, H, W, Cin, Cout, KH, KW, stride, pad, imgs_per_group, stats_ws, zero_cnt,
+                           n_zero, stream);
+}
+
+static int x3_bnin_bnstats_exit(int np, const float* in, int ldi, const float* in_ws, const float* in_gamma, const float* in_beta,
+                                const unsigned short* w3, long long plane_elems, float* out, int ldo, int n_img, int H, int W, int Cin,
+                                int Cout, int imgs_per_group, float eps, float* stats_ws, const float* gamma, const float* beta,
+                                const float* res, int ldr, const float* res_ws, const float* res_gamma, const float* res_beta, float* y,
+                                int ldy, int* cnt, void* stream) {
+    if (imgs_per_group <= 0 || n_img % imgs_per_group != 0 || stats_ws == nullptr || in_ws == nullptr || g_x3_tile > 1 || !gamma || !beta ||
+        !res || !y || !cnt || ldr < Cout || ldy < Cout || ldo < Cout || ldr % 4 != 0 || ldy % 4 != 0 || ldo % 4 != 0 ||
+        (res_ws && (!res_gamma || !res_beta)) || y == out || y == res)
+        return MFT_EINVAL;
+    X3Args ex;
+    x3_no_extras(ex);
+    ex.exit_cnt = cnt; ex.exit_out = y; ex.exit_ldo = ldy; ex.exit_gamma = gamma; ex.exit_beta = beta; ex.exit_res = res; ex.exit_ldr = ldr;
+    ex.exit_rws = res_ws; ex.exit_rgamma = res_gamma; ex.exit_rbeta = res_beta;
+    return x3_dispatch(in, ldi, w3, plane_elems, out, ldo, n_img, H, W, Cin, Cout, 3, 3, 1, 1, stats_ws, imgs_per_group * H * W, stream, in_ws,
+                       in_gamma, in_beta, eps, np, &ex);
+}
+
+extern "C" int mft_conv2d_nhwc_x3_bnin_bnstats_exit(const float* in, int ldi, const float* in_ws, const float* in_gamma, const float* in_beta,
+                                                    const unsigned short* w3, long long plane_elems, float* out, int ldo, int n_img, int H,
+                                                    int W, int Cin, int Cout, int imgs_per_group, float eps, float* stats_ws,
+                                                    const float* gamma, const float* beta, const float* res, int ldr, const float* res_ws,
+                                                    const float* res_gamma, const float* res_beta, float* y, int ldy, int* cnt,
+                                                    void* stream) {
+    return x3_bnin_bnstats_exit(3, in, ldi, in_ws, in_gamma, in_beta, w3, plane_elems, out, ldo, n_img, H, W, Cin, Cout, imgs_per_group, eps,
+                                stats_ws, gamma, beta, res, ldr, res_ws, res_gamma, res_beta, y, ldy, cnt, stream);
+}
+
+extern "C" int mft_conv2d_nhwc_h2_bnin_bnstats_exit(const float* in, int ldi, const float* in_ws, const float* in_gamma, const float* in_beta,
+                                                    const unsigned short* w2, long long plane_elems, float* out, int ldo, int n_img, int H,
+                                                    int W, int Cin, int Cout, int imgs_per_group, float eps, float* stats_ws,
+                                                    const float* gamma, const float* beta, const float* res, int ldr, const float* res_ws,
+                                                    const float* res_gamma, const float* res_beta, float* y, int ldy, int* cnt,
+                                                    void* stream) {
+    return x3_bnin_bnstats_exit(2, in, ldi, in_ws, in_gamma, in_beta, w2, plane_elems, out, ldo, n_img, H, W, Cin, Cout, imgs_per_group, eps,
+                                stats_ws, gamma, beta, res, ldr, res_ws, res_gamma, res_beta, y, ldy, cnt, stream);
+}
diff --git a/meta-fine-tuning_amd/functional.py b/meta-fine-tuning_amd/functional.py
--- a/meta-fine-tuning_amd/functional.py
+++ b/meta-fine-tuning_amd/functional.py
@@ -11,6 +11,9 @@
 FUSED_LAST_BLOCK = settings.current().fused_last_block
 X3_FUSED_STATS = settings.current().x3_fused_stats
 X3_FOLD_BN = settings.current().x3_fold_bn
+X3_PAIR_ENTRY = settings.current().x3_pair_entry
+X3_EXIT_IN_C2 = settings.current().x3_exit_in_c2
+X3_EXIT_MAX_ROWS = 256
 TRUNK_F16X2 = settings.current().trunk_f16x2
 TRAIN_X3 = settings.current().train_x3
 TRAIN_X3_MIN_ROWS = settings.current().train_x3_min_rows
@@ -88,6 +91,12 @@
             t = torch.empty(tuple(shape), device=self.device, dtype=dtype)
             self.bufs[key] = t
         return t
+
+    def zeros(self, name, shape, dtype=torch.float32):
+        key = (name, tuple(shape), dtype)
+        if key not in self.bufs:
+            self.bufs[key] = torch.zeros(tuple(shape), device=self.device, dtype=dtype)
+        return self.bufs[key]
 
     def existing(self, name, shape, dtype=torch.float32):
         key = (name, tuple(shape), dtype)
@@ -507,27 +516,53 @@
         return None if r is None else ws
 
     c1 = arena.get(tag + ".c1", (n, OH, OH, cout))
-    ws1 = partials(".C1", x, 3, stride, 1, c1, tag + ".bn1")
+    cnt = arena.zeros(tag + ".exitcnt", (groups * (cout // 64),), torch.int32) if X3_EXIT_IN_C2 and cout % 64 == 0 and rows <= X3_EXIT_MAX_ROWS else None
+    zeroed = False
+    sc = wss = None
+    ws1 = None
+    if X3_PAIR_ENTRY and cin != cout and stride > 1:
+        sc = arena.get(tag + ".sc", (n, OH, OH, cout))
+        ws1 = arena.get(tag + ".bn1.statws", (int(lib.mft_conv2d_x3_stats_ws_floats(n, H, H, cout, 3, 3, stride, 1)),))
+        wss = arena.get(tag + ".bns.statws", (int(lib.mft_conv2d_x3_stats_ws_floats(n, H, H, cout, 1, 1, stride, 0)),))
+        if ops.conv2d_x3_pair_bnstats(x, w3[p + ".C1"], w3[p + ".shortcut"], cout, stride, ipg, c1, ws1, sc, wss, zero=cnt) is None:
+            ws1 = wss = None
+        else:
+            zeroed = cnt is not None
+    if ws1 is None and cnt is not None:
+        ws1 = arena.get(tag + ".bn1.statws", (int(lib.mft_conv2d_x3_stats_ws_floats(n, H, H, cout, 3, 3, stride, 1)),))
+        if ops.conv2d_x3_bnstats_zero(x, w3[p + ".C1"], cout, 3, 3, stride, 1, ipg, c1, ws1, cnt) is None:
+            ws1 = None
+        else:
+            zeroed = True
+    if ws1 is None:
+        ws1 = partials(".C1", x, 3, stride, 1, c1, tag + ".bn1")
     if ws1 is None:
         return None
     c2 = arena.get(tag + ".c2", (n, OH, OH, cout))
     ws2 = arena.get(tag + ".bn2.statws", (int(lib.mft_conv2d_x3_stats_ws_floats(n, OH, OH, cout, 3, 3, 1, 1)),))
+    out = arena.get(tag + ".out", (n * OH * OH, cout))
+    gs = bs = None
+    if cin != cout:
+        gs, bs = W.bn[p + ".BNshortcut"]
+        if wss is None:
+            sc = arena.get(tag + ".sc", (n, OH, OH, cout))
+            wss = partials(".shortcut", x, 1, stride, 0, sc, tag + ".bns")
+        if wss is None:
+            raise RuntimeError("frozen block %s: shortcut outside the bf16x3 domain after C1 was inside it" % p)
+    res = sc.view(-1, cout) if cin != cout else x.view(-1, cin)
+    if zeroed and ops.conv2d_x3_bnin_bnstats_exit(c1, ws1, g1, b1, w3[p + ".C2"], cout, ipg, c2, ws2, g2, b2, res, out, cnt,
+                                                  res_ws=wss, res_gamma=gs, res_beta=bs) is not None:
+        return out.view(n, OH, OH, cout)
     if ops.conv2d_x3_bnin_bnstats(c1, ws1, g1, b1, w3[p + ".C2"], cout, ipg, c2, ws2) is None:
         r1 = ops.bn_apply_x3ws(c1.view(-1, cout), cout, rows, groups, ws1, g1, b1, arena.get(tag + ".r1", (n * OH * OH, cout)),
                                act=ops.ACT_RELU).view(n, OH, OH, cout)
         if ops.conv2d_x3_bnstats(r1, w3[p + ".C2"], cout, 3, 3, 1, 1, ipg, c2, ws2, None, None) is None:
             raise RuntimeError("frozen block %s: C2 outside the bf16x3 domain after C1 was inside it" % p)
-    out = arena.get(tag + ".out", (n * OH * OH, cout))
     if cin != cout:
-        gs, bs = W.bn[p + ".BNshortcut"]
-        sc = arena.get(tag + ".sc", (n, OH, OH, cout))
-        wss = partials(".shortcut", x, 1, stride, 0, sc, tag + ".bns")
-        if wss is None:
-            raise RuntimeError("frozen block %s: shortcut outside the bf16x3 domain after C1 was inside it" % p)
-        ops.bn_apply_x3ws(c2.view(-1, cout), cout, rows, groups, ws2, g2, b2, out, act=ops.ACT_RELU, res=sc.view(-1, cout),
-                          res_ws=wss, res_gamma=gs, res_beta=bs)
+        ops.bn_apply_x3ws(c2.view(-1, cout), cout, rows, groups, ws2, g2, b2, out, act=ops.ACT_RELU, res=res, res_ws=wss, res_gamma=gs,
+                          res_beta=bs)
     else:
-        ops.bn_apply_x3ws(c2.view(-1, cout), cout, rows, groups, ws2, g2, b2, out, act=ops.ACT_RELU, res=x.view(-1, cin))
+        ops.bn_apply_x3ws(c2.view(-1, cout), cout, rows, groups, ws2, g2, b2, out, act=ops.ACT_RELU, res=res)
     return out.view(n, OH, OH, cout)
 
 
diff --git a/meta-fine-tuning_amd/ops.py b/meta-fine-tuning_amd/ops.py
--- a/meta-fine-tuning_amd/ops.py
+++ b/meta-fine-tuning_amd/ops.py
@@ -254,6 +254,49 @@
         return None
     _lib.check(rc, name)
     return out, mean, rstd
+
+
+def conv2d_x3_pair_bnstats(x, w3_c1, w3_sc, Cout, stride, imgs_per_group, out_c1, ws_c1, out_sc, ws_sc, zero=None):
+    _f32c(x)
+    if int(w3_c1.shape[0]) != int(w3_sc.shape[0]):
+        return None
+    n, H, W, Cin = x.shape
+    fn, name = _x3_fn(w3_c1, "_pair_bnstats")
+    rc = fn(_p(x), Cin, n, H, W, Cin, Cout, stride, imgs_per_group, _p(w3_c1), w3_c1.shape[1] * w3_c1.shape[2], _p(out_c1), Cout,
+            _p(ws_c1), _p(w3_sc), w3_sc.shape[1] * w3_sc.shape[2], _p(out_sc), Cout, _p(ws_sc), _p(zero),
+            0 if zero is None else zero.numel(), _stream())
+    if rc == _lib.MFT_EINVAL:
+        return None
+    _lib.check(rc, name)
+    return out_c1, out_sc
+
+
+def conv2d_x3_bnstats_zero(x, w3, Cout, KH, KW, stride, pad, imgs_per_group, out, ws, zero):
+    _f32c(x)
+    assert zero.dtype == torch.int32 and zero.is_contiguous()
+    n, H, W, Cin = x.shape
+    fn, name = _x3_fn(w3, "_bnstats_zero")
+    rc = fn(_p(x), Cin, _p(w3), w3.shape[1] * w3.shape[2], _p(out), Cout, n, H, W, Cin, Cout, KH, KW, stride, pad, imgs_per_group, _p(ws),
+            _p(zero), zero.numel(), _stream())
+    if rc == _lib.MFT_EINVAL:
+        return None
+    _lib.check(rc, name)
+    return out
+
+
+def conv2d_x3_bnin_bnstats_exit(c_raw, in_ws, in_gamma, in_beta, w3, Cout, imgs_per_group, out, ws, gamma, beta, res, y, cnt,
+                                res_ws=None, res_gamma=None, res_beta=None, eps=BN_EPS):
+    _f32c(c_raw)
+    n, H, W, Cin = c_raw.shape
+    assert cnt.dtype == torch.int32 and cnt.numel() >= (n // imgs_per_group) * (Cout // 64)
+    fn, name = _x3_fn(w3, "_bnin_bnstats_exit")
+    rc = fn(_p(c_raw), Cin, _p(in_ws), _p(in_gamma), _p(in_beta), _p(w3), w3.shape[1] * w3.shape[2], _p(out), Cout, n, H, W, Cin, Cout,
+            imgs_per_group, eps, _p(ws), _p(gamma), _p(beta), _p(res), res.shape[-1], _p(res_ws), _p(res_gamma), _p(res_beta), _p(y),
+            y.shape[-1], _p(cnt), _stream())
+    if rc == _lib.MFT_EINVAL:
+        return None
+    _lib.check(rc, name)
+    return y
 
 
 def conv2d_x3_bnin_bnstats(c_raw, in_ws, in_gamma, in_beta, w3, Cout, imgs_per_group, out, ws, mean=None, rstd=None, eps=BN_EPS):
diff --git a/meta-fine-tuning_amd/settings.py b/meta-fine-tuning_amd/settings.py
--- a/meta-fine-tuning_amd/settings.py
+++ b/meta-fine-tuning_amd/settings.py
@@ -36,6 +36,8 @@
     ("fused_dgrad", "MFT_FUSED_DGRAD", _flag, False, "one-pass trunk.7.C2 weight gradient + Adam + data gradient (measured slower in the step)"),
     ("x3_fused_stats", "MFT_X3_FUSED_STATS", _flag, True, "BatchNorm statistics from the split-precision convolution epilogue"),
     ("x3_fold_bn", "MFT_X3_FOLD_BN", _flag, True, "frozen blocks without helper launches (per-tile partials merged by the consumers)"),
+    ("x3_pair_entry", "MFT_X3_PAIR_ENTRY", _flag, True, "frozen strided blocks: the 1x1 shortcut convolution rides in C1's grid (0: a launch of its own; bit-identical)"),
+    ("x3_exit_in_c2", "MFT_X3_EXIT_IN_C2", _flag, True, "frozen blocks: the block exit is finished inside C2's launch by the last workgroup per (group, N tile) (0: a launch of its own; bit-identical)"),
     ("trunk_f16x2", "MFT_TRUNK_F16X2", _flag, True, "frozen trunk.4-6 on two fp16 pieces per operand (0: three bf16 pieces)"),
     ("stem_pooled", "MFT_STEM_POOLED", _flag, True, "stem cache keeps per-window (max, min) instead of the full-resolution output"),
     ("stem_fused_fill", "MFT_STEM_FUSED_FILL", _flag, True, "stem cache filled by ONE launch (convolution + moments + window min/max; 0: three launches through a full-resolution buffer)"),
@@ -81,6 +83,8 @@
     fused_dgrad: bool = False
     x3_fused_stats: bool = True
     x3_fold_bn: bool = True
+    x3_pair_entry: bool = True
+    x3_exit_in_c2: bool = True
     trunk_f16x2: bool = True
     stem_pooled: bool = True
     stem_fused_fill: bool = True
@@ -144,7 +148,7 @@
 
 IMPORT_TIME = frozenset((
     "debug_skip_trunk", "adapt_graph", "adapt_batched_trunk", "fused_dgrad", "fused_last_block", "x3_fused_stats",
-    "x3_fold_bn", "trunk_f16x2", "train_x3", "train_x3_min_rows", "fused_pair_mlp", "pair_f16x2", "pair_rk_rows", "gemm_rk_rows", "pair_mlp_gb", "wgrad_batch",
+    "x3_fold_bn", "x3_pair_entry", "x3_exit_in_c2", "trunk_f16x2", "train_x3", "train_x3_min_rows", "fused_pair_mlp", "pair_f16x2", "pair_rk_rows", "gemm_rk_rows", "pair_mlp_gb", "wgrad_batch",
     "train_graph", "small_groups", "wf_xcd",
 ))
 assert IMPORT_TIME <= set(k[0] for k in KNOBS), IMPORT_TIME - set(k[0] for k in KNOBS)
```
